# xiyichen/morphablediffusion

Measured on AMD Instinct MI355X. Metric: multi-view denoising steps/sec (N=16 views, 256x256, CFG 2.0, DDIM-50 step), higher is better.
Workload: dtype f16; 1 GPU; synthetic sample (FaceScape-FLAME-sized mesh, 5023 vertices before voxel de-duplication): N=16 target views, 256x256 (latent 32x32), perspective cameras, full-width UNet (916.9M params, random init), CFG 2.0, one denoise_apply per step; views_per_gpu=16, batch_view_num=16, parallelism=single GPU

## Files before the change

include/mvd.h:

```cpp
#ifndef MVD_H
#define MVD_H
#include <stddef.h>
#include <stdint.h>

#ifdef __cplusplus
extern "C" {
#endif

typedef struct mvd_ctx mvd_ctx;

typedef struct {
  int image_size;
  int in_channels;
  int out_channels;
  int model_channels;
  int num_res_blocks;
  int channel_mult[4];
  int num_heads;
  int context_dim;
  int volume_dims[4];
  int attention_levels;
} mvd_unet_config;

typedef struct {
// ... 89 lines not shown
                      float* mse_per_sample, void* stream);
int mvd_op_image_metrics(const void* pred, int pred_dtype, int pred_layout, const void* target, int target_dtype, int target_layout,
                         const unsigned char* mask, int mask_mode, int V, int H, int W, double* out, void* stream);
int mvd_op_mesh_project(const float* verts, const float* K, const float* RT, int N, int Nv, float z_near, int32_t* xy, int32_t* key,
                        void* stream);
int mvd_op_mesh_raster(const int32_t* xy, const int32_t* key, const int32_t* faces, int N, int Nv, int Nf, int H, int W, int32_t* face_id,
                       int32_t* pix_key, int32_t* bad_faces, void* stream);
int mvd_op_mesh_vertex_colors(const void* images, int dtype, int layout, const int32_t* xy, const int32_t* key, const int32_t* faces,
                              const int32_t* face_id, const int32_t* pix_key, const float* verts, const float* normals,
                              const float* centres, int N, int Nv, int Nf, int H, int W, float power, int bias, int two_sided,
                              float fill_r, float fill_g, float fill_b, float* color, float* weight_sum, int32_t* n_seen, float* spread,
                              unsigned char* visible, void* stream);
int mvd_op_morph_pose(const float* betas, const float* pose, const float* j_template, const float* j_dirs, const int32_t* parents, int F,
                      int NB, int J, float* j_rest, float* rot, float* pose_feature, float* joints, float* A, void* stream);
int mvd_op_morph_skin(const float* basis, const float* v_template, const float* coef, const float* weights, const float* A,
                      const float* post, int F, int V, int L, int NB, int J, float* verts, void* stream);
int mvd_op_morph_landmarks(const float* verts, const int32_t* faces, const int32_t* lmk_face, const float* lmk_bary, int F, int V, int Nf,
                           int M, float* out, void* stream);
int mvd_train_conditioner_backward(mvd_ctx* ctx, const float* x_noisy, int64_t timestep, const float* v_embed, int n_views,
                                   int target_index, const float* dsrc0, const float* dsrc1, const float* dsrc2, const float* dsrc3,
                                   float* dbg_dvolume, float* dbg_dfused, float* dbg_dfeats, float* dbg_dtembed, void* stream);
int mvd_train_conditioner_backward_batch(mvd_ctx* ctx, int B, const int* slots, const float* x_noisy, const int64_t* timesteps,
                                         const float* v_embed, int n_views, const int* target_index, const float* dsrc0,
                                         const float* dsrc1, const float* dsrc2, const float* dsrc3, float* dbg_dvolume,
                                         float* dbg_dfused, float* dbg_dfeats, float* dbg_dtembed, void* stream);
int mvd_train_set_deterministic(mvd_ctx* ctx, int on);
int mvd_op_frustum_adjoint(mvd_ctx* ctx, const float* d_out, const int32_t* view_idx, int TN, int D, int S, int deterministic,
                           float* d_vol, void* stream);
int mvd_op_latent_adjoint(mvd_ctx* ctx, const float* d_vol, int deterministic, float* d_rows, int32_t* n_rows_out, void* stream);
int mvd_op_vertex_adjoint(mvd_ctx* ctx, const float* d_vf, const int32_t* view_idx, int n_views, int deterministic, float* d_feats,
                          void* stream);
int mvd_probe_adjoint_calls(mvd_ctx* ctx, int64_t* out);
int mvd_op_vertex_gather(mvd_ctx* ctx, const float* feats, const int32_t* view_idx, int n_views, float* vf_out, void* stream);
int mvd_op_latent_gather(mvd_ctx* ctx, const float* rows, float* vol_out, void* stream);
int mvd_op_frustum_gather(mvd_ctx* ctx, const float* vol, const int32_t* view_idx, int TN, int D, int S, float* out, void* stream);
int mvd_train_cond_backward(mvd_ctx* ctx, int cond_index, const float* x, const float* context, const float* d_out, int B, int H,
                            int W, int depth0, float* dx, float* dcontext, void* stream);
int mvd_train_get_grad(mvd_ctx* ctx, const char* name, float* out, size_t numel, void* stream);
int mvd_train_get_tensor(mvd_ctx* ctx, const char* name, float* out, size_t numel, void* stream);
int64_t mvd_train_bn_calls(mvd_ctx* ctx);
int mvd_train_adamw_step(mvd_ctx* ctx, float lr, float lr_aux, float beta1, float beta2, float eps, float weight_decay, int step,
                         float inv_scale, int finetune_unet, int* skipped_out, void* stream);
int mvd_train_grad_norm(mvd_ctx* ctx, float inv_scale, int finetune_unet, float* norm_out, void* stream);
int mvd_train_adamw_step_ex(mvd_ctx* ctx, float lr, float lr_aux, float beta1, float beta2, float eps, float weight_decay, int step,
                            float inv_scale, int finetune_unet, int* skipped_out, float max_grad_norm, float ema_decay,
                            float* grad_norm_out, void* stream);
int mvd_train_last_grad_norm(mvd_ctx* ctx, float* norm_out, void* stream);
int mvd_train_ema_swap(mvd_ctx* ctx, void* stream);
int mvd_train_repack(mvd_ctx* ctx);
int mvd_train_repack_async(mvd_ctx* ctx, void* stream);
int mvd_lora_attach(mvd_ctx* ctx, const char* const* keys, int n, int rank, float alpha);
int mvd_lora_arena_size(mvd_ctx* ctx, int64_t* numel);
int mvd_lora_target_count(mvd_ctx* ctx);
int mvd_lora_info(mvd_ctx* ctx, int i, char* name, size_t cap, int64_t* a_off, int64_t* b_off, int64_t* out, int64_t* in);
int mvd_lora_adopt_arena(mvd_ctx* ctx, int which, float* ptr, int64_t numel);
int mvd_lora_project(mvd_ctx* ctx, void* stream);
int mvd_lora_step(mvd_ctx* ctx, float lr, float beta1, float beta2, float eps, float weight_decay, int step, float inv_scale,
                  float max_grad_norm, int* skipped_out, float* grad_norm_out, void* stream);
int mvd_lora_set_scale(mvd_ctx* ctx, float scale, void* stream);
int mvd_lora_detach(mvd_ctx* ctx, int keep_merged);
int mvd_train_grad_bucket_count(mvd_ctx* ctx);
int mvd_train_grad_bucket(mvd_ctx* ctx, int k, int max_ranges, int64_t* offs, int64_t* lens, int* n_ranges);
int mvd_train_grad_bucket_wait(mvd_ctx* ctx, int k, void* stream);
int mvd_train_set_bucket_snapshot(mvd_ctx* ctx, float* arena);
int mvd_train_sync_gradients(mvd_ctx* ctx, int phase, void* comm_stream, void* stream);
int mvd_set_volume(mvd_ctx* ctx, const float* volume, void* stream);

int mvd_frustum_volumes(mvd_ctx* ctx, const float* t_embed, const float* v_embed, const int32_t* view_idx, int TN,
                        float* out0, float* out1, float* out2, float* out3, void* stream);
int mvd_frustum_volumes_batch(mvd_ctx* ctx, int B, const int* slots, const float* volumes, const float* t_embed, const float* v_rows,
                              const int32_t* view_idx, float* out0, float* out1, float* out2, float* out3, void* stream);

int mvd_denoise_views(mvd_ctx* ctx, const float* x_noisy, const float* x_input, const float* clip, int64_t timestep,
                      const float* t_embed, const float* v_embed, const int32_t* view_idx, int TN, float cfg_scale,
                      const float* noise, float sqrt_one_minus_at, float sqrt_at, float sqrt_aprev, float dir_coef,
                      float sigma, float* eps_out, float* x_prev, void* stream);
int mvd_denoise_views_batch(mvd_ctx* ctx, int B, const int* slots, const float* x_noisy, const float* x_input, const float* clip,
                            const int64_t* timesteps, const float* t_embed, const float* v_embed, const int32_t* view_idx, int TN,
                            float cfg_scale, const float* noise, float sqrt_one_minus_at, float sqrt_at, float sqrt_aprev,
                            float dir_coef, float sigma, float* eps_out, float* x_prev, void* stream);

int mvd_denoise_views_ms(mvd_ctx* ctx, int B, const int* slots, const float* x_noisy, const float* x_input, const float* clip,
                         const int64_t* timesteps, const float* t_embed, const float* v_embed, const int32_t* view_idx, int TN,
                         float cfg_scale, const float* noise, float s1m, float sqrt_at, float c_x, float c_d, float c_c, float c_n,
                         float* x0_hist, int first, float* eps_out, float* x_next, void* stream);

int mvd_op_cfg_ms(const float* eps_c, const float* eps_u, float scale, const float* x, const float* noise, float s1m, float sqrt_at,
                  float c_x, float c_d, float c_c, float c_n, float* x0_hist, int first, float* eps_out, float* x_next, size_t n,
                  void* stream);
int mvd_op_adamw_ex(float* p, const float* g, float* m, float* v, float* e, size_t n, float lr, float beta1, float beta2, float eps,
                    float wd, int step, float inv_scale, float max_grad_norm, float ema_decay, float* norm_out, void* stream);
int mvd_op_lora_project(const float* dW, const float* A, const float* B, int out, int in, int r, float scale, float* gA, float* gB,
                        void* stream);
int mvd_op_lora_merge(const float* W0, const float* A, const float* B, int out, int in, int r, float scale, float* W, void* stream);
int mvd_op_lora_project_grouped(const float* dW, const float* A, const float* B, int n, const int64_t* w_off, const int64_t* out,
                                const int64_t* in, const int64_t* a_off, const int64_t* b_off, int r, float scale, float* gA, float* gB,
                                void* stream);
int mvd_op_lora_merge_grouped(const float* W0, const float* A, const float* B, int n, const int64_t* w_off, const int64_t* w0_off,
                              const int64_t* out, const int64_t* in, const int64_t* a_off, const int64_t* b_off, int r, float scale,
                              float* W, void* stream);
int mvd_op_sparse_conv(const float* in, const int32_t* nbr, int n_out, int Cin, int Cout, const float* w, int layout, const float* scale,
                       const float* shift, int form, float* out, void* stream);
int mvd_op_bn_rows_relu(const float* x, int n, int C, const float* gamma, const float* beta, float eps, float momentum, float* y,
                        float* stats_out, float* rmean, float* rvar, void* stream);
int mvd_op_bn_rows_relu_bwd(const float* xraw, float* dy, int n, int C, const float* gamma, const float* beta, const float* stats,
                            int poison, float* dgamma, float* dbeta, void* stream);
int mvd_op_sparse_conv_bwd(const float* in, const int32_t* nbr, float* d_out, int n_in, int n_out, int Cin, int Cout, int strided,
                           int level0_subm, int deterministic, int form, const float* w, int layout, int poison, float* d_in, float* gw,
                           void* stream);
int mvd_op_conv(mvd_ctx* ctx, const float* x_nchw, int B, int Cin, int H, int W, const float* w, const float* bias,
                int Cout, int ksize, int stride, int upsample, const float* resid_nchw, float* out_nchw, int force_splitk,
                void* stream);
int mvd_op_linear(mvd_ctx* ctx, const float* a, int M, int K, const float* w, const float* bias, int N, int geglu,
                  const float* resid, int a_half, int force_splitk, float* out, void* stream);
int mvd_op_group_norm(mvd_ctx* ctx, const float* x_nchw, int B, int C, int HW, int groups, const float* gamma,
                      const float* beta, float eps, int act, float* out_nchw, void* stream);
int mvd_op_depth_attn(mvd_ctx* ctx, const float* qk, const float* context, const float* fill_row, int n_cond, int HW, int D, int Cc,
                      int heads, int ldx, int split, int nfill, int check_only, float* out, float* hi_out, void* stream);
int mvd_op_conv3d(mvd_ctx* ctx, const float* x_ncdhw, int B, int Cin, int D, int H, int W, const float* w,
                  const float* bias, int Cout, int stride, int transposed, const float* resid, float* out, void* stream);
int mvd_op_group_norm_bwd(mvd_ctx* ctx, const float* x, const float* dy, int B, int rows, int C, int groups, const float* gamma,
                          const float* beta, float eps, int act, float* dx, float* dgamma, float* dbeta, void* stream);
int mvd_op_layer_norm_bwd(mvd_ctx* ctx, const float* x, const float* dy, int rows, int C, const float* gamma, float* dx,
                          float* dgamma, float* dbeta, void* stream);
int mvd_op_conv_bwd(mvd_ctx* ctx, int kind, int ksize, int B, int Cin, int H, int W, int Cout, const float* x, int x_f16,
                    const float* w, const float* dy, int xp, int accum, int need_din, int poison, float* dx, float* dw, float* db,
                    void* stream);
int mvd_op_linear_bwd(mvd_ctx* ctx, int B, int rows, int K, int N, const float* x, int x_f16, const float* w, const float* bias,
                      const float* dy, int geglu, int dx_f16, int staged, int xp, int accum, int poison, float* dx, float* dw,
                      float* db, void* stream);
int mvd_op_conv3d_bwd(mvd_ctx* ctx, int kind, int B, int Cin, int D, int H, int W, int Cout, const float* x, int x_f16,
                      const float* w, const float* dy, int accum, int poison, float* dx, float* dw, float* db, void* stream);
int mvd_op_tgemm(mvd_ctx* ctx, int M, int N, int K, const float* a, int a_f16, int a_trans, long lda, const float* b, int b_f16,
                 int b_trans, long ldb, float* out, int ldc, int accum, int xp, int poison, void* stream);
int mvd_op_st_tail(mvd_ctx* ctx, int C, int rows, int T, const float* ao, const float* xin, const float* rowbias,
                   const float* w_ao, const float* b_ao, const float* ln_g, const float* ln_b, const float* w1, const float* b1,
                   const float* w2, const float* b2, const float* w_po, const float* b_po, const float* resid, float* out,
                   int flags, int iters, float* ms_out, void* stream);
int mvd_op_st_head(mvd_ctx* ctx, int rows, int xp, const float* n0, const float* w_pi, const float* b_pi, const float* ln_g,
                   const float* ln_b, const float* w_q, const float* w_k, const float* w_v, float* t0_out, float* qkv_out,
                   int iters, float* ms_out, void* stream);
int mvd_op_linear_ex(mvd_ctx* ctx, const float* a, int B, int rows, int K, const float* w, const float* bias, int N,
                     const float* rowbias, int rb_ld, float alpha, int act, int use_bias, int out_f16, int out_split, int ldc,
                     const float* resid, int resid_f16, int ldr, int a_half, int force_splitk, int xp, float* slabs,
                     size_t slabs_cap, int defer_epilogue, int* sk_used, int poison, void* out, void* stream);
int mvd_op_conv_ex(mvd_ctx* ctx, const float* x, int B, int H, int W, int Cin, const float* w, const float* bias, int Cout, int ksize,
                   int stride, int upsample, int up_fold, int tap_shift, const float* rowbias, int rb_ld, float alpha, int act,
                   int use_bias, int out_f16, int out_split, int ldc, const float* resid, int resid_f16, int ldr, int a_half,
                   int force_splitk, int xp, int conv3x_stream, float* slabs, size_t slabs_cap, int defer_epilogue, int* sk_used,
                   int poison, void* out, void* stream);
int mvd_op_conv3d_ex(mvd_ctx* ctx, const float* x, int B, int D, int H, int W, int Cin, const float* w, const float* bias, int Cout,
                     int stride, int transposed, int use_bias, const float* resid, int ldr, int in_place, int out_f16, int ldc,
                     int a_half, int force_splitk, int poison, void* out, void* stream);
int mvd_op_group_norm_ex(mvd_ctx* ctx, const float* x, int B, int rows, int C, int ld, int groups, const float* gamma,
                         const float* beta, float eps, int act, int form, const float* preadd, int pld, int split, int nslab,
                         size_t slab_stride, const float* bias2, const float* resid, int ldr, float* mat, int ldm, int ldo,
                         int poison, void* out, void* stream);
int mvd_op_layer_norm_slabs(mvd_ctx* ctx, const float* slabs, int nslab, size_t slab_stride, int rows, int C, const float* bias,
                            const float* rowbias, int rb_ld, int T, const float* resid, int ldr, const float* gamma,
                            const float* beta, float eps, int plain, int ld_raw, int poison, float* mat, void* raw, void* out,
                            void* stream);
int mvd_op_folded_group_norm(mvd_ctx* ctx, const float* x, int B, int rps, int K, const float* w, int N, int cpg,
                             const float* gamma, const float* beta, float eps, int poison, float* partials, float* scale,
                             float* shift, void* out, void* stream);
int mvd_op_softmax_rows(mvd_ctx* ctx, const float* scores, int rows, int cols, int out_f32, void* out, void* stream);
int mvd_op_rows_split(mvd_ctx* ctx, const float* x, int lda, int rows, int C, void* out, void* stream);
int mvd_op_attention_ex(mvd_ctx* ctx, const float* q, const float* k, const float* v, int B, int T, int heads, int d, int Tstride,
                        int ld_pad, int xcd, float* out, void* stream);
int mvd_op_attention_bwd_ex(mvd_ctx* ctx, const float* q, const float* k, const float* v, const float* d_out, int B, int T,
                            int heads, int d, float* dq, float* dk, float* dv, float* lse, float* delta, float* o, void* stream);
int mvd_op_train_depth_attn(const float* q, const float* k, const float* v, int R, int HW, int D, int hn, int hd, float* attn,
                            float* z, void* stream);
int mvd_op_train_depth_attn_bwd(const float* q, const float* k, const float* v, const float* attn, const float* dz, int R, int HW,
                                int D, int hn, int hd, float* dq, float* dk, float* dv, void* stream);
int mvd_op_train_im2col3(const float* x, int B, int H, int W, int C, float* col, void* stream);
int mvd_op_train_col2im3(const float* dcol, int B, int H, int W, int C, float* dx, void* stream);
int mvd_op_train_perm_w3(const float* src, int N, int C, int to_mat, float* dst, void* stream);
int mvd_bench_conv(mvd_ctx* ctx, int B, int C, int H, int W, int Cout, int iters, float* ms_out, void* stream);
int mvd_vae_decode(mvd_ctx* ctx, const float* z, int B, int h, int w, float* out, void* stream);
int mvd_vae_encode(mvd_ctx* ctx, const float* x, int B, int H, int W, float* moments, void* stream);
int mvd_clip_encode(mvd_ctx* ctx, const float* x, int B, int H, int W, float* out, void* stream);
int mvd_clip_embed_dim(mvd_ctx* ctx);
int mvd_probe_config(mvd_ctx* ctx, int mode, const char* family, int stride);
int mvd_probe_report(mvd_ctx* ctx, char* buf, size_t cap);
int mvd_bench_linear(mvd_ctx* ctx, int M, int K, int N, int flags, int iters, float* ms_out, void* stream);
int mvd_bench_group_norm(mvd_ctx* ctx, int B, int C, int HW, int groups, int flags, int iters, float* ms_out, void* stream);

#ifdef __cplusplus
}
#endif
#endif
```

morphablediffusion_amd/csrc/c_api_hooks.hip:

```cpp
#include <math.h>
#include <string.h>

#include <algorithm>
#include <string>
#include <vector>

#include "hooks.h"
#include "rowchain.h"

namespace {

__global__ void split_rows_to_f32_kernel(const half_t* in, int rows, int C, float* out) {
  for (size_t i = (size_t)blockIdx.x * blockDim.x + threadIdx.x; i < (size_t)rows * C; i += (size_t)gridDim.x * blockDim.x) {
    const size_t r = i / C, c = i % C;
    const half_t hi = in[r * 3 * C + c], lo = in[r * 3 * C + C + c], h2 = in[r * 3 * C + 2 * C + c];
    out[i] = (float)hi == (float)h2 ? (float)hi + (float)lo : __builtin_nanf("");
  }
}
__global__ void rows_f32_to_f16_ld_kernel(const float* in, size_t rows, int C, half_t* out, int ldo) {
  for (size_t i = (size_t)blockIdx.x * blockDim.x + threadIdx.x; i < rows * C; i += (size_t)gridDim.x * blockDim.x)
    out[(i / C) * ldo + i % C] = (half_t)in[i];
}
__global__ void rows_f32_ld_to_f16_ld_kernel(const float* in, int ldi, size_t rows, int C, half_t* out, int ldo) {
  for (size_t i = (size_t)blockIdx.x * blockDim.x + threadIdx.x; i < rows * C; i += (size_t)gridDim.x * blockDim.x)
// ... 484 lines not shown
  half_t* stream_w = ws_alloc<half_t>(c, rowhead_stream_halfs(xp));
  float* tmp = ws_alloc<float>(c, (size_t)3 * C);
  half_t* n0h = ws_alloc<half_t>(c, n * (xp ? 3 : 1));
  half_t* qkvh = ws_alloc<half_t>(c, 3 * n);
  WS_CHECK(stream_w && tmp && n0h && qkvh);
  RhWeights w;
  w.w_pi = w_pi; w.ln_g = ln_g; w.ln_b = ln_b; w.w_q = w_q; w.w_k = w_k; w.w_v = w_v;
  RET_IF(rowhead_pack(w, xp, tmp, stream_w, s));
  if (xp) RET_IF(launch_rows_f32_to_f16_split(n0, C, rows, C, n0h, s));
  else RET_IF(launch_f32_to_f16(n0, n0h, n, s));
  RowHead p;
  p.stream = stream_w; p.rows = rows; p.n0 = n0h; p.ld_n0 = xp ? 3 * C : C; p.b_pi = b_pi; p.t0 = t0_out; p.ld_t0 = C; p.qkv = qkvh; p.ld_qkv = 3 * C;
  RET_IF(launch_rowhead(p, xp, s));
  if (iters > 0) {
    float ms = 0.f;
    RET_IF(hook_time(s, iters, [&] { return launch_rowhead(p, xp, s); }, &ms));
    if (ms_out) *ms_out = ms;
  }
  hook_f16_to_f32(qkvh, qkv_out, 3 * n, s);
  HIP_CHECK_RET(hipGetLastError());
  return 0;
}

namespace {
struct ExEpi {
  const float *bias, *rowbias, *resid;
  int rb_ld, act, use_bias, out_f16, out_split, ldc, resid_f16, ldr, force_splitk;
  float alpha;
  float* slabs;
  size_t slabs_cap;
  int defer_epilogue;
  int* sk_used;
  void* out;
};
int ex_epi_check(const char* who, const ExEpi& e, int N, bool rb_unaligned_ok = false) {
  const std::string w(who);
  if (!e.out) return mvd_fail((w + ": null result").c_str());
  if (N <= 0 || (N & 3)) return mvd_fail((w + ": N must be a positive multiple of 4").c_str());
  if (e.act != ACT_NONE && e.act != ACT_SILU) return mvd_fail((w + ": act is 0 (none) or 1 (SiLU)").c_str());
  if (!(e.alpha == e.alpha) || e.alpha - e.alpha != 0.0f) return mvd_fail((w + ": alpha must be finite").c_str());
  if (e.use_bias && !e.bias) return mvd_fail((w + ": use_bias without a bias").c_str());
  if (e.rowbias && (e.rb_ld < N || (!rb_unaligned_ok && (e.rb_ld & 3)))) return mvd_fail((w + ": rb_ld must be a multiple of 4, >= N").c_str());
  if (e.resid && (e.ldr < N || (e.ldr & 3))) return mvd_fail((w + ": ldr must be a multiple of 4, >= N").c_str());
  if (e.out_split && !e.out_f16) return mvd_fail((w + ": out_split is a form of the fp16 result").c_str());
  if ((e.ldc & 3) || e.ldc < (e.out_split ? 3 : 1) * N) return mvd_fail((w + ": ldc must be a multiple of 4, >= N (3 N with out_split)").c_str());
  if (e.force_splitk < 0) return mvd_fail((w + ": force_splitk >= 0").c_str());
  if (e.slabs && !e.sk_used) return mvd_fail((w + ": a slab buffer needs sk_used").c_str());
  if (e.slabs && ((uintptr_t)e.slabs & 15)) return mvd_fail((w + ": the slab buffer must be 16-byte aligned").c_str());
  if ((uintptr_t)e.out & 15) return mvd_fail((w + ": the result must be 16-byte aligned").c_str());
  return 0;
}
int ex_epi_fill(mvd_ctx* c, const ExEpi& e, size_t out_rows, int N, GemmArgs& g, hipStream_t s) {
  g.out = e.out; g.out_f32 = e.out_f16 ? 0 : 1; g.ldc = e.ldc; g.out_split = e.out_split ? N : 0;
  g.rowbias = e.rowbias; g.rb_ld = e.rb_ld; g.alpha = e.alpha; g.act = e.act; g.use_bias = e.use_bias != 0;
  g.force_splitk = e.force_splitk;
  if (e.resid) {
    g.resid = e.resid; g.resid_f32 = 1; g.ldr = e.ldr;
    if (e.resid_f16) {
      const half_t* rh;
      RET_IF(hook_f16(c, e.resid, out_rows * e.ldr, &rh, s));
      g.resid = rh; g.resid_f32 = 0;
    }
  }
  if (e.slabs) {
    g.slabs = e.slabs; g.slabs_cap = e.slabs_cap; g.sk_used = e.sk_used; g.defer_epilogue = e.defer_epilogue != 0;
  }
  return 0;
}
}

int mvd_op_linear_ex(mvd_ctx* c, const float* a, int B, int rows, int K, const float* w, const float* bias, int N, const float* rowbias,
                     int rb_ld, float alpha, int act, int use_bias, int out_f16, int out_split, int ldc, const float* resid,
                     int resid_f16, int ldr, int a_half, int force_splitk, int xp, float* slabs, size_t slabs_cap, int defer_epilogue,
                     int* sk_used, int poison, void* out, void* stream) {
  RET_IF(hook_begin(c));
  if (!a || !w) return mvd_fail("op_linear_ex: null operand");
  if (B <= 0 || rows <= 0 || rows % B || K <= 0 || (K & 7)) return mvd_fail("op_linear_ex: rows % B == 0 and K % 8 == 0 expected");
  const ExEpi e{bias, rowbias, resid, rb_ld, act, use_bias, out_f16, out_split, ldc, resid_f16, ldr, force_splitk, alpha,
                slabs, slabs_cap, defer_epilogue, sk_used, out};
  RET_IF(ex_epi_check("op_linear_ex", e, N, true));
  hipStream_t s = S(stream);
  WsScope ws_scope(c);
  const int Kp = xp ? 3 * K : K;
  ConvW cw;
  RET_IF(hook_pack_fwd(c, w, N, K, 1, 0, 0, xp, &cw, s));
  cw.bias = const_cast<float*>(bias);
  GemmArgs g;
  g.a = a; g.a_f32 = 1; g.lda = K; g.w = &cw;
  if (xp || a_half) {
    half_t* ah = ws_alloc<half_t>(c, (size_t)rows * Kp);
    WS_CHECK(ah);
    if (xp) RET_IF(launch_rows_f32_to_f16_split(a, K, rows, K, ah, s));
    else RET_IF(launch_f32_to_f16(a, ah, (size_t)rows * K, s));
    g.a = ah; g.a_f32 = 0; g.lda = Kp;
  }
  RET_IF(ex_epi_fill(c, e, (size_t)rows, N, g, s));
  if (sk_used) *sk_used = 1;
  if (poison) RET_IF(hook_poison(c, s));
  return hook_sync("op_linear_ex", s, run_linear(c, g, B, rows, s));
}

int mvd_op_conv_ex(mvd_ctx* c, const float* x, int B, int H, int W, int Cin, const float* w, const float* bias, int Cout, int ksize,
                   int stride, int upsample, int up_fold, int tap_shift, const float* rowbias, int rb_ld, float alpha, int act,
                   int use_bias, int out_f16, int out_split, int ldc, const float* resid, int resid_f16, int ldr, int a_half,
                   int force_splitk, int xp, int conv3x_stream, float* slabs, size_t slabs_cap, int defer_epilogue, int* sk_used,
                   int poison, void* out, void* stream) {
  RET_IF(hook_begin(c));
  if (!x || !w) return mvd_fail("op_conv_ex: null operand");
  if (B <= 0 || H <= 0 || W <= 0 || Cin <= 0 || (Cin & 7)) return mvd_fail("op_conv_ex: Cin % 8 == 0 expected");
  if ((ksize != 1 && ksize != 3) || (stride != 1 && stride != 2) || (upsample != 0 && upsample != 1))
    return mvd_fail("op_conv_ex: 1x1 or 3x3, stride 1 or 2, upsample 0 or 1");
  if (tap_shift != 0 && (tap_shift != 1 || ksize != 3 || stride != 2 || upsample || (H & 1) || (W & 1)))
    return mvd_fail("op_conv_ex: tap_shift = 1 is the 3x3 stride-2 Downsample of even H and W");
  if (up_fold && (!upsample || ksize != 3 || stride != 1 || xp || slabs))
    return mvd_fail("op_conv_ex: the parity-folded form is a 3x3 stride-1 upsample conv without xp or a slab buffer");
  const ExEpi e{bias, rowbias, resid, rb_ld, act, use_bias, out_f16, out_split, ldc, resid_f16, ldr, force_splitk, alpha,
                slabs, slabs_cap, defer_epilogue, sk_used, out};
  RET_IF(ex_epi_check("op_conv_ex", e, Cout));
  hipStream_t s = S(stream);
  WsScope ws_scope(c);
  const int taps = ksize * ksize, Cp = xp ? 3 * Cin : Cin;
  const int Ho = ((H << upsample) - 1) / stride + 1, Wo = ((W << upsample) - 1) / stride + 1;
  const size_t rows_in = (size_t)B * H * W, rows_out = (size_t)B * Ho * Wo;
  ConvW cw;
  RET_IF(hook_pack_fwd(c, w, Cout, Cin, taps, 0, 0, xp, &cw, s));
  cw.bias = const_cast<float*>(bias);
  GemmArgs g;
  g.a = x; g.a_f32 = 1; g.lda = Cin; g.w = &cw; g.tap_shift = tap_shift;
  if (xp || a_half) {
    half_t* xh = ws_alloc<half_t>(c, rows_in * Cp);
    WS_CHECK(xh);
    if (xp) RET_IF(launch_rows_f32_to_f16_split(x, Cin, (long)rows_in, Cin, xh, s));
    else RET_IF(launch_f32_to_f16(x, xh, rows_in * Cin, s));
    g.a = xh; g.a_f32 = 0; g.lda = Cp;
  }
  const int bnx = Cout % 160 == 0 ? 160 : (Cout % 128 == 0 ? 128 : 0);
  if (conv3x_stream && taps == 9 && bnx && Cp % 64 == 0 && !g.a_f32) {
    cw.wx = ws_alloc<half_t>(c, conv3x_stream_halfs(Cout, Cp, bnx));
    WS_CHECK(cw.wx);
    RET_IF(conv3x_pack(cw.w, Cout, Cp, bnx, cw.wx, s));
    cw.wx_bn = bnx;
  }
  if (up_fold) {
    cw.w_up = ws_alloc<half_t>(c, (size_t)16 * Cout * Cin);
    WS_CHECK(cw.w_up);
    RET_IF(launch_pack_upconv_weight(w, Cout, Cin, cw.w_up, s));
  }
  RET_IF(ex_epi_fill(c, e, rows_out, Cout, g, s));
  if (sk_used) *sk_used = 1;
  if (poison) RET_IF(hook_poison(c, s));
  return hook_sync("op_conv_ex", s, up_fold ? run_upconv2d(c, g, B, H, W, s) : run_conv2d(c, g, B, H, W, stride, upsample, s));
}

int mvd_op_conv3d_ex(mvd_ctx* c, const float* x, int B, int D, int H, int W, int Cin, const float* w, const float* bias, int Cout,
                     int stride, int transposed, int use_bias, const float* resid, int ldr, int in_place, int out_f16, int ldc,
                     int a_half, int force_splitk, int poison, void* out, void* stream) {
  RET_IF(hook_begin(c));
  if (!x || !w || !out) return mvd_fail("op_conv3d_ex: null operand");
  if (B <= 0 || D <= 0 || H <= 0 || W <= 0 || Cin <= 0 || (Cin & 7)) return mvd_fail("op_conv3d_ex: Cin % 8 == 0 expected");
  if (Cout <= 0 || (Cout & 3)) return mvd_fail("op_conv3d_ex: Cout must be a positive multiple of 4");
  if ((transposed != 0 && transposed != 1) || (stride != 1 && stride != 2) || (transposed && stride != 1))
    return mvd_fail("op_conv3d_ex: stride 1 or 2, or transposed (with stride 1)");
  if (use_bias && !bias) return mvd_fail("op_conv3d_ex: use_bias without a bias");
  if (resid && (ldr < Cout || (ldr & 3))) return mvd_fail("op_conv3d_ex: ldr must be a multiple of 4, >= Cout");
  if (in_place && !resid) return mvd_fail("op_conv3d_ex: in_place needs a residual");
  if ((ldc & 3) || ldc < Cout) return mvd_fail("op_conv3d_ex: ldc must be a multiple of 4, >= Cout");
  if (force_splitk < 0) return mvd_fail("op_conv3d_ex: force_splitk >= 0");
  if ((uintptr_t)out & 15) return mvd_fail("op_conv3d_ex: the result must be 16-byte aligned");
  const int Do = transposed ? 2 * D : (D - 1) / stride + 1, Ho = transposed ? 2 * H : (H - 1) / stride + 1,
            Wo = transposed ? 2 * W : (W - 1) / stride + 1;
  const size_t rows_in = (size_t)B * D * H * W, rows_out = (size_t)B * Do * Ho * Wo;
  if (rows_out > (size_t)1 << 24 || rows_out * (size_t)ldc > (size_t)1 << 30 || rows_in * (size_t)Cin > (size_t)1 << 30)
    return mvd_fail("op_conv3d_ex: at most 2^24 output rows and 2^30 elements per image");
  hipStream_t s = S(stream);
  WsScope ws_scope(c);
  ConvW cw;
  RET_IF(hook_pack_fwd(c, w, Cout, Cin, 27, transposed, 0, 0, &cw, s));
  cw.bias = const_cast<float*>(bias);
  GemmArgs g;
  g.a = x; g.a_f32 = 1; g.lda = Cin; g.w = &cw; g.out = out; g.out_f32 = out_f16 ? 0 : 1; g.ldc = ldc;
  g.use_bias = use_bias != 0; g.force_splitk = force_splitk;
  if (a_half) {
    const half_t* xh;
    RET_IF(hook_f16(c, x, rows_in * Cin, &xh, s));
    g.a = xh; g.a_f32 = 0;
  }
  if (resid) {
    g.resid = resid; g.resid_f32 = 1; g.ldr = ldr;
    if (in_place) {
      if (out_f16) {
        hipLaunchKernelGGL(rows_f32_ld_to_f16_ld_kernel, dim3(hook_blocks(rows_out * Cout)), dim3(256), 0, s, resid, ldr, rows_out, Cout,
                           (half_t*)out, ldc);
        HIP_CHECK_RET(hipGetLastError());
      } else {
        HIP_CHECK_RET(hipMemcpy2DAsync(out, (size_t)ldc * 4, resid, (size_t)ldr * 4, (size_t)Cout * 4, rows_out, hipMemcpyDeviceToDevice, s));
      }
      g.resid = out; g.resid_f32 = out_f16 ? 0 : 1; g.ldr = ldc;
    }
  }
  if (poison) RET_IF(hook_poison(c, s));
  return hook_sync("op_conv3d_ex", s, transposed ? run_convT3d(c, g, B, D, H, W, s) : run_conv3d(c, g, B, D, H, W, stride, s));
}

int mvd_op_group_norm_ex(mvd_ctx* c, const float* x, int B, int rows, int C, int ld, int groups, const float* gamma, const float* beta,
                         float eps, int act, int form, const float* preadd, int pld, int split, int nslab, size_t slab_stride,
                         const float* bias2, const float* resid, int ldr, float* mat, int ldm, int ldo, int poison, void* out,
                         void* stream) {
  RET_IF(hook_begin(c));
  if (!x || !gamma || !beta || !out) return mvd_fail("op_group_norm_ex: null operand");
  if (B <= 0 || rows <= 0 || C <= 0 || groups <= 0 || C % groups || ld < C) return mvd_fail("op_group_norm_ex: C % groups == 0 and ld >= C expected");
  if (act < ACT_NONE || act > ACT_RELU || (form != 0 && form != 1) || split < 0 || split > 2) return mvd_fail("op_group_norm_ex: act 0..2, form 0..1, split 0..2");
  if (ldo < (split == 1 ? 3 : (split == 2 ? 2 : 1)) * C) return mvd_fail("op_group_norm_ex: ldo >= C halfs (3 C with split = 1, 2 C with split = 2)");
  if (nslab < 1 || (nslab > 1 && slab_stride < (size_t)B * rows * ld)) return mvd_fail("op_group_norm_ex: slabs overlap");
  if (preadd && pld < C) return mvd_fail("op_group_norm_ex: pld >= C expected");
  if ((resid && ldr < C) || (mat && ldm < C)) return mvd_fail("op_group_norm_ex: ldr, ldm >= C expected");
  const bool one_pass = !mvd_env().gn_two_pass && gn_group_eligible(ld, rows, C, groups, preadd ? pld : 0, ldo);
  if ((form == 1 || !one_pass) && (nslab > 1 || bias2 || resid || mat || split == 2))
    return mvd_fail("op_group_norm_ex: slabs, bias2, resid, mat and the fp32 result need the single-pass form");
  hipStream_t s = S(stream);
  WsScope ws_scope(c);
  NormW n;
  n.g = const_cast<float*>(gamma); n.b = const_cast<float*>(beta); n.C = C;
  half_t* o = (half_t*)out;
  if (form == 0) {
    if (poison) RET_IF(hook_poison(c, s));
    return hook_sync("op_group_norm_ex", s,
                   run_group_norm(c, x, ld, B, rows, n, groups, eps, act, preadd, o, ldo, s, pld, split, nslab, slab_stride, bias2, resid,
                                  ldr, mat, ldm));
  }
  if (C > 2560 || groups > 32 || (C & 3) || (ld & 3) || (ldo & 3) || (preadd && (pld & 3)))
    return mvd_fail("op_group_norm_ex: the two-pass form takes C <= 2560, groups <= 32 and C, ld, ldo, pld % 4 == 0");
  float* partial = ws_alloc<float>(c, (size_t)B * gn_max_slabs() * groups * 2);
  WS_CHECK(partial);
  if (poison) RET_IF(hook_poison(c, s));
  int nsl = 0;
  int rc = launch_gn_stats(x, ld, B, rows, C, groups, preadd, pld, partial, &nsl, s);
  if (!rc) rc = launch_gn_apply(x, ld, B, rows, C, groups, preadd, pld, partial, nsl, gamma, beta, eps, act, o, ldo, s, split);
  return hook_sync("op_group_norm_ex", s, rc);
}

int mvd_op_layer_norm_slabs(mvd_ctx* c, const float* slabs, int nslab, size_t slab_stride, int rows, int C, const float* bias,
                            const float* rowbias, int rb_ld, int T, const float* resid, int ldr, const float* gamma, const float* beta,
                            float eps, int plain, int ld_raw, int poison, float* mat, void* raw, void* out, void* stream) {
  RET_IF(hook_begin(c));
  if (!slabs || !gamma || !beta || !out) return mvd_fail("op_layer_norm_slabs: null operand");
  if (rows <= 0 || C <= 0 || nslab < 1 || T < 1) return mvd_fail("op_layer_norm_slabs: bad argument");
  if (raw && ld_raw < C) return mvd_fail("op_layer_norm_slabs: ld_raw >= C expected");
  hipStream_t s = S(stream);
  if (plain) {
    if (nslab != 1 || bias || rowbias || resid || mat) return mvd_fail("op_layer_norm_slabs: the plain LayerNorm takes one slab and writes no mat");
    if (poison) RET_IF(hook_poison(c, s));
    return hook_sync("op_layer_norm_slabs", s, launch_layernorm(slabs, rows, C, gamma, beta, eps, (half_t*)out, s, (half_t*)raw, ld_raw));
  }
  if (!mat) return mvd_fail("op_layer_norm_slabs: mat is required");
  if (nslab > 1 && slab_stride < (size_t)rows * C) return mvd_fail("op_layer_norm_slabs: slabs overlap");
  if ((rowbias && rb_ld < C) || (resid && ldr < C)) return mvd_fail("op_layer_norm_slabs: rb_ld, ldr >= C expected");
  if (poison) RET_IF(hook_poison(c, s));
  return hook_sync("op_layer_norm_slabs", s,
                 launch_layernorm_slabs(slabs, nslab, slab_stride, rows, C, bias, rowbias, rb_ld, T, resid, ldr, mat, gamma, beta, eps,
                                        (half_t*)out, s, (half_t*)raw, ld_raw));
}

int mvd_op_folded_group_norm(mvd_ctx* c, const float* x, int B, int rps, int K, const float* w, int N, int cpg, const float* gamma,
                             const float* beta, float eps, int poison, float* partials, float* scale, float* shift, void* out,
                             void* stream) {
  RET_IF(hook_begin(c));
  if (!x || !w || !gamma || !beta || !partials || !scale || !shift || !out) return mvd_fail("op_folded_group_norm: null operand");
  if (B <= 0 || rps <= 0 || K <= 0 || (K & 7) || N <= 0 || (N & 3)) return mvd_fail("op_folded_group_norm: K % 8 == 0 and N % 4 == 0 expected");
  if (rps % 256 || (cpg != 8 && cpg != 16 && cpg != 32) || (long)B * rps < 512)
    return mvd_fail("op_folded_group_norm: rps % 256 == 0, 8 / 16 / 32 channels per group and at least 512 rows expected");
  if (N % cpg || N / cpg > 32) return mvd_fail("op_folded_group_norm: at most 32 whole groups expected");
  hipStream_t s = S(stream);
  WsScope ws_scope(c);
  const int rows = B * rps, G = N / cpg, ntile = rps / 256;
  ConvW cw;
  RET_IF(hook_pack_fwd(c, w, N, K, 1, 0, 0, 0, &cw, s));
  const half_t* xh;
  RET_IF(hook_f16(c, x, (size_t)rows * K, &xh, s));
  if (poison) RET_IF(hook_poison(c, s));
  GemmArgs g;
  g.a = xh; g.lda = K; g.w = &cw; g.use_bias = false; g.gn_partial = partials; g.gn_cpg = cpg; g.force_splitk = 1;
  int rc = run_linear(c, g, B, rows, s);
  if (!rc) rc = launch_gn_finalize(partials, B, ntile, rps, N, G, gamma, beta, eps, scale, shift, N, s);
  if (!rc) {
    g = GemmArgs();
    g.a = xh; g.lda = K; g.w = &cw; g.use_bias = false; g.out = out; g.out_f32 = 0; g.ldc = N;
    g.rowscale = scale; g.rs_ld = N; g.rowbias = shift; g.rb_ld = N; g.act = ACT_RELU; g.force_splitk = 1;
    rc = run_linear(c, g, B, rows, s);
  }
  return hook_sync("op_folded_group_norm", s, rc);
}

int mvd_op_softmax_rows(mvd_ctx* c, const float* scores, int rows, int cols, int out_f32, void* out, void* stream) {
  RET_IF(hook_begin(c));
  if (!scores || !out || rows <= 0 || cols <= 0) return mvd_fail("op_softmax_rows: bad argument");
  hipStream_t s = S(stream);
  return hook_sync("op_softmax_rows", s,
                 out_f32 ? launch_softmax_rows_f32(scores, rows, cols, (float*)out, s) : launch_softmax_rows(scores, rows, cols, (half_t*)out, s));
}

int mvd_op_rows_split(mvd_ctx* c, const float* x, int lda, int rows, int C, void* out, void* stream) {
  RET_IF(hook_begin(c));
  if (!x || !out || rows <= 0 || C <= 0 || lda < C) return mvd_fail("op_rows_split: bad argument");
  hipStream_t s = S(stream);
  return hook_sync("op_rows_split", s, launch_rows_f32_to_f16_split(x, lda, rows, C, (half_t*)out, s));
}


namespace {
int attn_ex_check(const char* who, const void* q, const void* k, const void* v, int B, int T, int heads, int d) {
  const std::string w(who);
  if (!q || !k || !v) return mvd_fail((w + ": null operand").c_str());
  if (B < 1 || T < 1 || heads < 1) return mvd_fail((w + ": B, T, heads >= 1 expected").c_str());
  if (d != 8 && d != 16 && d != 32 && d != 40 && d != 64 && d != 80 && d != 160) return mvd_fail((w + ": unsupported head dim").c_str());
  return 0;
}
hipError_t hook_unpack_qkv(const float* dqkv, size_t rows, int C, float* dq, float* dk, float* dv, hipStream_t s) {
  float* outs[3] = {dq, dk, dv};
  for (int i = 0; i < 3; ++i) {
    const hipError_t e = hipMemcpy2DAsync(outs[i], (size_t)C * 4, dqkv + (size_t)i * C, (size_t)3 * C * 4, (size_t)C * 4, rows, hipMemcpyDeviceToDevice, s);
    if (e != hipSuccess) return e;
  }
  return hipSuccess;
}
}

int mvd_op_attention_ex(mvd_ctx* c, const float* q, const float* k, const float* v, int B, int T, int heads, int d, int Tstride,
                        int ld_pad, int xcd, float* out, void* stream) {
  RET_IF(hook_begin(c));
  RET_IF(attn_ex_check("op_attention_ex", q, k, v, B, T, heads, d));
  if (!out) return mvd_fail("op_attention_ex: null operand");
  if (Tstride < 0 || (Tstride != 0 && Tstride < T)) return mvd_fail("op_attention_ex: Tstride >= T (or 0) expected");
  if (ld_pad < 0 || ld_pad % 8) return mvd_fail("op_attention_ex: ld_pad must be a multiple of 8");
  if (xcd < -1 || xcd > 1) return mvd_fail("op_attention_ex: xcd is -1, 0 or 1");
  hipStream_t s = S(stream);
  WsScope ws_scope(c);
  const int C = heads * d, ld = 3 * C + ld_pad, Ts = Tstride ? Tstride : T;
  const size_t rows = (size_t)B * Ts + 1;
  half_t* qkv = ws_alloc<half_t>(c, rows * ld);
  half_t* o = ws_alloc<half_t>(c, rows * C);
  WS_CHECK(qkv && o);
  HIP_CHECK_RET(hipMemsetAsync(qkv, 0xFF, rows * ld * sizeof(half_t), s));
  HIP_CHECK_RET(hipMemsetAsync(o, 0xFF, rows * C * sizeof(half_t), s));
  hipLaunchKernelGGL(pack_qkv_image_kernel, dim3(hook_blocks((size_t)B * T * C)), dim3(256), 0, s, q, k, v, B, T, C, Ts, ld, qkv);
  int rc = launch_attention(qkv, ld, qkv + 2 * C, ld, o, C, B, T, heads, d, s, Ts, xcd);
  if (!rc) {
    hook_f16_to_f32(o, out, rows * C, s);
    if (hipGetLastError() != hipSuccess) rc = mvd_fail("op_attention_ex: launch failed");
  }
  return hook_sync("op_attention_ex", s, rc);
}

int mvd_op_attention_bwd_ex(mvd_ctx* c, const float* q, const float* k, const float* v, const float* d_out, int B, int T, int heads,
                            int d, float* dq, float* dk, float* dv, float* lse, float* delta, float* o_out, void* stream) {
// ... 74 lines not shown
```

morphablediffusion_amd/csrc/common.h:

```cpp
#pragma once
#include <hip/hip_runtime.h>
#include <hip/hip_fp16.h>
#include <stdint.h>

#include "env.h"

#ifdef MVD_BF16
typedef __bf16 half_t;
#define MVD_MFMA_32x32x16 __builtin_amdgcn_mfma_f32_32x32x16_bf16
#define MVD_MFMA_16x16x32 __builtin_amdgcn_mfma_f32_16x16x32_bf16
#define MVD_DTYPE_NAME "bf16"
#else
typedef _Float16 half_t;
#define MVD_MFMA_32x32x16 __builtin_amdgcn_mfma_f32_32x32x16_f16
#define MVD_MFMA_16x16x32 __builtin_amdgcn_mfma_f32_16x16x32_f16
#define MVD_DTYPE_NAME "f16"
#endif
typedef half_t h8 __attribute__((ext_vector_type(8)));
typedef half_t h4 __attribute__((ext_vector_type(4)));
typedef half_t h2 __attribute__((ext_vector_type(2)));
typedef float f32x16 __attribute__((ext_vector_type(16)));
typedef float f32x4 __attribute__((ext_vector_type(4)));

#define MVD_MAX_TAPS 27

enum { ACT_NONE = 0, ACT_SILU = 1, ACT_RELU = 2 };

inline bool xcd_prefers_cols(int tiles_m, int groups_n, double a_bytes, double w_bytes) {
  const int nwg = tiles_m * groups_n, q = (nwg + 7) / 8;
  if (nwg < 16) return false;
  auto span = [](int q_, int inner, int outer) {
    const double n = q_ % inner == 0 ? q_ / inner : (q_ - 1) / (double)inner + 1.0;
    return n < outer ? n : (double)outer;
  };
  const double at = a_bytes / tiles_m, wt = w_bytes / groups_n;
  const double row = at * span(q, groups_n, tiles_m) + wt * (q < groups_n ? q : groups_n);
  const double col = wt * span(q, tiles_m, groups_n) + at * (q < tiles_m ? q : tiles_m);
  return col < 0.8 * row;
}

struct IGemm {
  const void* a;
  int a_f32;
  int lda;
  int Cin;
  int cin_alg;
  int B, Z, Y, X;
  int IZ, IY, IX;
  int sz, sy, sx;
  int ups;
  int PZ, PY, PX;
  int ntaps;
  int tap[MVD_MAX_TAPS];
  const half_t* w;
  int N;
  void* out;
  int out_f32;
  int ldc;
  int out_linear;
  int OZ, OY, OX, ozm, ozo, oym, oyo, oxm, oxo;
  const float* bias;
  const float* rowbias;
  int rb_ld;
  const float* rowscale;
  int rs_ld;
  float* gn_partial;
  int gn_cpg;
  const void* resid;
  int resid_f32;
  int ldr;
  int out_split;
  int geglu;
  float alpha;
  int act;
  int nch;
  int xcd_cols;
  int npar;
  int par_ntaps[8];
  int par_tap[8][8];
  int par_oz[8], par_oy[8], par_ox[8];
  int par_walk;
  const half_t* wx;
  int wx_bn;
  int bn;
  int bm;
  int splitk;
  float* partial;
};

struct MvdStream {
  hipStream_t s;
};

#define HIP_CHECK_RET(expr)                                        \
  do {                                                             \
    hipError_t _e = (expr);                                        \
    if (_e != hipSuccess) return mvd_fail(hipGetErrorString(_e));  \
  } while (0)

int mvd_fail(const char* msg);
const char* mvd_error_text();

#define MVD_MAX_DEVICES 64
static inline int mvd_current_device() {
  int d = 0;
  if (hipGetDevice(&d) != hipSuccess || d < 0 || d >= MVD_MAX_DEVICES) d = 0;
  return d;
}
static inline int cdiv(int a, int b) { return (a + b - 1) / b; }
static inline int igemm_tap(int dz, int dy, int dx, int slab) { return (dz + 1) | ((dy + 1) << 2) | ((dx + 1) << 4) | (slab << 8); }

int launch_igemm(const IGemm& g, hipStream_t s);
int igemm_pick_bn(int N, int geglu);
int launch_splitk_reduce(const IGemm& g, hipStream_t s);
bool conv3_halo_eligible(const IGemm& g);
int conv3_halo_tiles(const IGemm& g, int bn);
int launch_conv3_halo(const IGemm& g, hipStream_t s);
int igemm_pick_splitk(int M, int N, int ksteps, int bn);
bool conv3x_eligible(const IGemm& g, int bn);
size_t conv3x_stream_halfs(int N, int Cin, int bn);
int conv3x_pack(const half_t* w, int N, int Cin, int bn, half_t* stream, hipStream_t s);
int launch_conv3x(const IGemm& g, const half_t* stream, int bn, hipStream_t s);
bool gemm_dma_eligible(const IGemm& g);
bool gemm_dma_is_plain(const IGemm& g);
void gemm_dma_plan(int M, int N, int ksteps, int bn, int geglu, int* nch_out, int* splitk_out);
int launch_target_encoder(const float* x, const float* pre, int n_views, const half_t* const* w, const float* const* bias,
                          const int* cin, const float* const* gamma, const float* const* beta, float* feats, hipStream_t s);
void gemm_dma_plan_us(int M, int N, int ksteps, int geglu, int out_b, int res_b, int* bn_io, int* nch_out, int* splitk_out,
                      int* bm_out = nullptr);
int launch_gemm_dma(const IGemm& g, hipStream_t s);

int launch_gn_stats(const float* x, int ld, int B, int rows_per_sample, int C, int G, const float* preadd, int pld,
                    float* partial, int* nslabs_out, hipStream_t s);
int launch_gn_apply(const float* x, int ld, int B, int rows_per_sample, int C, int G, const float* preadd, int pld,
                    const float* partial, int nslabs, const float* gamma, const float* beta, float eps, int act,
                    half_t* out, int ldo, hipStream_t s, int split = 0);
int gn_max_slabs();
int launch_gn_finalize(const float* partial, int B, int nslabs, int rows_per_sample, int C, int G, const float* gamma,
                       const float* beta, float eps, float* scale, float* shift, int ld, hipStream_t s);
bool gn_group_eligible(int ld, int rows, int C, int G, int pld, int ldo);
int launch_gn_group(const float* x, int ld, int B, int rows, int C, int G, const float* preadd, int pld, const float* gamma,
                    const float* beta, float eps, int act, half_t* out, int ldo, hipStream_t s, int split = 0,
                    int nslab = 1, size_t slab_stride = 0, const float* bias2 = nullptr, const float* resid = nullptr, int ldr = 0,
                    float* mat = nullptr, int ldm = 0);
int launch_layernorm(const float* x, int rows, int C, const float* gamma, const float* beta, float eps,
                     half_t* out, hipStream_t s, half_t* raw = nullptr, int ld_raw = 0);
bool layernorm_slabs_takes(int C);
int launch_layernorm_slabs(const float* slabs, int nslab, size_t slab_stride, int rows, int C, const float* bias, const float* rowbias,
                           int rb_ld, int T, const float* resid, int ldr, float* mat, const float* gamma, const float* beta, float eps,
                           half_t* out, hipStream_t s, half_t* raw = nullptr, int ld_raw = 0);
int launch_layernorm_f32(const float* x, long ldx, int rows, int C, const float* gamma, const float* beta, float eps,
                         float* out, hipStream_t s);
int launch_attention(const half_t* qk, int ldqk, const half_t* v, int ldv, half_t* out, int ldo, int B, int T, int heads,
                     int d, hipStream_t s, int Tstride = 0, int xcd = -1);
int launch_clip_patches(const float* img, int B, int H, int W, int S, int P, int Kp, half_t* out, hipStream_t s);
int launch_clip_tokens(const float* pe, const float* cls, const float* pos, int B, int T, int Tp, int C, float* x,
                       hipStream_t s);
int launch_scale_copy(const float* src, size_t n, float k, float* dst, hipStream_t s);
int launch_softmax_rows(const float* s, long rows, int cols, half_t* p, hipStream_t st);
int launch_softmax_rows_f32(const float* s, long rows, int cols, float* p, hipStream_t st);
int launch_depth_attn(const float* qk, const half_t* ctxn, half_t* z, int n_cond, int HW, int D, int Cc, int heads,
                      hipStream_t s, int split = 0, int nfill = 0, const half_t* fill_row = nullptr, int ldx = 0);
int depth_attn_check(int D, int Cc, int heads, int ldx, int nfill);
int launch_small_linear(const float* a, int lda, int rows, int K, const half_t* w, const float* bias, int N,
                        int act_in, float* out, int ldo, int accumulate, hipStream_t s);
int launch_timestep_embedding(const int64_t* t, int B, int dim, float* out, hipStream_t s);
int launch_nchw_to_nhwc(const float* in, int B, int C, int HW, float* out, int ldo, int cpad, hipStream_t s);
int launch_nhwc_to_nchw(const float* in, int ld, int B, int C, int HW, float* out, hipStream_t s);
int launch_pack_weight(const float* src, int N, int Cin, int taps, int transposed, int geglu, half_t* dst,
                       hipStream_t s, int cin_src = -1, int xp = 0);
int launch_rows_f32_to_f16_split(const float* in, int lda, long rows, int C, half_t* out, hipStream_t s);
int launch_permute_geglu_bias(const float* src, int N, float* dst, hipStream_t s);
int launch_f32_to_f16(const float* in, half_t* out, size_t n, hipStream_t s);
int launch_rows_f32_to_f16(const float* in, int lda, long rows, int C, half_t* out, hipStream_t s);
int launch_pack_upconv_weight(const float* src, int N, int Cin, half_t* dst, hipStream_t s);
int launch_fill_rows_f16(half_t* out, int ld, int rows, const half_t* vec, int n, hipStream_t s);
int launch_fold_qk(const float* wq, const float* wk, int heads, int hd, int Cc, int I, float scale, half_t* out,
                   hipStream_t s, float* out32 = nullptr);
int launch_fold_ov(const float* wo, const float* wv, int heads, int hd, int Cc, int I, half_t* out, hipStream_t s,
                   float* out32 = nullptr);
int launch_fold_mm(const float* a, int lda, const float* b, int ldb, int M, int N, int K, half_t* out16, int ldc, float* out32,
                   hipStream_t s);
int launch_relu_beta_tile(const float* beta, int Cc, int heads, half_t* out, hipStream_t s, int split = 0);
int launch_cfg_ddim(const float* eps_c, const float* eps_u, float scale, const float* x, const float* noise,
                    float sqrt_one_minus_at, float sqrt_at, float sqrt_aprev, float dir_coef, float sigma,
                    float* eps_out, float* x_prev, size_t n, hipStream_t s);
struct DpmCoef {
  float s1m, sqrt_at, c_x, c_d, c_c, c_n;
};
int launch_cfg_dpm(const float* eps_c, const float* eps_u, float scale, const float* x, const float* noise, DpmCoef k,
                   float* x0_hist, int use_hist, float* eps_out, float* x_next, size_t n, hipStream_t s);
struct ViewCam {
  float P[12];
  float Pinv[12];
  float Kinv[9];
  float near_, far_;
};
int launch_vertex_gather(const float* feats, const ViewCam* cams, const int* view_idx, int n_views, const float* verts, int Nv, int V,
                         float vol_len, int fsize, int persp, float* out, hipStream_t s);
int launch_unproject_views(const float* feats, const ViewCam* cams, int N, int V, float vol_len, int S, int persp, half_t* out,
                           hipStream_t s);
int launch_rows_f16_to_nchw(const half_t* in, long rows, int C, float* out, hipStream_t s);
int launch_accumulate_f32(float* dst, const float* src, size_t n, hipStream_t s);
int launch_fuse_views(const float* vf, int n_views, int Nv, int total_views, const float* w, const float* b,
                      float* out, int accumulate, hipStream_t s);
int launch_sparse_conv(const float* in, const int* nbr, int n_out, int Cin, int Cout, const float* w, const float* wp,
                       const float* scale, const float* shift, float* out, hipStream_t s, int mask_nonrep = 0);
bool sparse_mfma_takes(int Cin, int Cout);
int launch_sparse_w_frag(const float* w, int Cl_in, int Cl_out, int transposed, int flip, float* dst, hipStream_t s);
int launch_sparse_w_pack(const float* src, int Cin, int Cout, int layout, float* dst, hipStream_t s);
int launch_bn_fold(const float* gamma, const float* beta, const float* mean, const float* var, float eps, int C, float* scale,
                   float* shift, hipStream_t s);
int launch_bn_rows_relu(const float* x, float* y, int n, int C, const float* gamma, const float* beta, float eps, float* stats_out,
                        hipStream_t s, float* rmean = nullptr, float* rvar = nullptr, float momentum = 0.f);
int launch_mse(const float* a, const float* b, size_t n, float* out, hipStream_t s);
size_t train_loss_scratch_bytes(int B, int HW);
int train_loss_check(const char* who, int B, int HW, int C, int loss_type, float huber_delta);
int launch_train_loss(const float* pred, const float* target, int B, int HW, int C, const float* w, const float* m, int loss_type,
                      float huber_delta, float loss_scale, float* dpred, float* loss_out, float* loss_ps, float* mse_ps, void* scratch,
                      hipStream_t s);
size_t image_metrics_scratch_bytes(int V, int H, int W);
int image_metrics_check(const char* who, const void* pred, int pred_dtype, int pred_layout, const void* target, int target_dtype,
                        int target_layout, const unsigned char* mask, int mask_mode, int V, int H, int W, const double* out);
int launch_image_metrics(const void* pred, int pred_dtype, int pred_layout, const void* target, int target_dtype, int target_layout,
                         const unsigned char* mask, int mask_mode, int V, int H, int W, double* out, void* scratch, hipStream_t s);
int mesh_project_check(const char* who, const float* verts, const float* K, const float* RT, int N, int Nv, float z_near, const int* xy,
                       const int* key);
int launch_mesh_project(const float* verts, const float* K, const float* RT, int N, int Nv, float z_near, int* xy, int* key, hipStream_t s);
int mesh_raster_check(const char* who, const int* xy, const int* key, const int* faces, int N, int Nv, int Nf, int H, int W,
                      const int* face_id, const int* pix_key, const int* bad_faces);
size_t mesh_raster_scratch_bytes(int N, int H, int W);
int launch_mesh_raster(const int* xy, const int* key, const int* faces, int N, int Nv, int Nf, int H, int W, int* face_id, int* pix_key,
                       int* bad_faces, void* scratch, hipStream_t s);
int mesh_vertex_colors_check(const char* who, const void* images, int dtype, int layout, const int* xy, const int* key, const int* faces,
                             const int* face_id, const int* pix_key, const float* verts, const float* normals, const float* centres, int N,
                             int Nv, int Nf, int H, int W, float power, const float* color, const float* weight_sum, const int* n_seen,
                             const float* spread);
int launch_mesh_vertex_colors(const void* images, int dtype, int layout, const int* xy, const int* key, const int* faces, const int* face_id,
                              const int* pix_key, const float* verts, const float* normals, const float* centres, int N, int Nv, int Nf,
                              int H, int W, float power, int bias, int two_sided, float fill_r, float fill_g, float fill_b, float* color,
                              float* weight_sum, int* n_seen, float* spread, unsigned char* visible, hipStream_t s);
constexpr int MORPH_MAX_JOINTS = 64;
int morph_pose_check(const char* who, const float* betas, const float* pose, const float* j_template, const float* j_dirs,
                     const int* parents, int F, int NB, int J, const float* j_rest, const float* rot, const float* pose_feature,
                     const float* joints, const float* A);
int launch_morph_pose(const float* betas, const float* pose, const float* j_template, const float* j_dirs, const int* parents, int F,
                      int NB, int J, float* j_rest, float* rot, float* pose_feature, float* joints, float* A, hipStream_t s);
int morph_skin_check(const char* who, const float* basis, const float* v_template, const float* coef, const float* weights,
                     const float* A, int F, int V, int L, int NB, int J, const float* verts);
int launch_morph_skin(const float* basis, const float* v_template, const float* coef, const float* weights, const float* A,
                      const float* post, int F, int V, int L, int J, float* verts, hipStream_t s);
int morph_landmarks_check(const char* who, const float* verts, const int* faces, const int* lmk_face, const float* lmk_bary, int F, int V,
                          int Nf, int M, const float* out);
int launch_morph_landmarks(const float* verts, const int* faces, const int* lmk_face, const float* lmk_bary, int F, int V, int Nf, int M,
                           float* out, hipStream_t s);
int launch_latent_gather(const float* feats, const int* grid, int gd, int gh, int gw, const float* min_xyz,
                         const int* out_sh, float voxel, int V, float vol_len, float* out, hipStream_t s);
int launch_sparse_densify(const float* feats, const int* grid, long nvox, int C, float* out, hipStream_t s);
int launch_frustum_gather(const float* vol, const ViewCam* cams, const int* view_idx, int TN, int D, int S, int V,
                          float vol_len, int persp, half_t* out, hipStream_t s);
int launch_bits_checksum(const void* p, size_t bytes, unsigned long long* out, hipStream_t s);
int launch_add_rows(float* dst, const float* a, const float* b, size_t n, hipStream_t s);
int launch_add_image_rows(const float* in, int ldi, const float* img, int C, int nb, int HW, float* out, int ldo, hipStream_t s);
int launch_upsample2_f16(const float* in, int ldi, int B, int H, int W, int C, half_t* out, hipStream_t s);
int launch_conv_in_f32(const float* x, int ldx, const float* w, int cin_src, const float* bias, int N, int B, int H, int W, float* out,
                       int ldo, hipStream_t s);
int launch_out_conv_f32(const float* a, int C, const float* w, const float* bias, int N, int B, int H, int W, float* out, int ldo,
                        hipStream_t s);
int launch_probe_null(hipStream_t s);
int bwd_tcast(const void* src, int src_f32, long ld, int R, int C, half_t* dst, int Rp, hipStream_t s, int split = 0, half_t* rows16 = nullptr,
              int Cp = 0);
int bwd_im2colT(const void* src, int src_f32, long ld, int B, int H, int W, int C, int stride, int ups, half_t* dst, int Rp, hipStream_t s);
int bwd_cast_rows(const float* src, long ld, long rows, int C, int Cp, half_t* dst, hipStream_t s, int split = 0);
int bwd_pack_dgrad(const half_t* w, int taps, int N, int ldw, int Cl, int Np, half_t* wT, hipStream_t s, int flip = 1);
int bwd_group_norm(const float* x, long ld, const float* pre, int pld, const float* dy, long ldy, int B, int rows, int C, int G,
// ... 97 lines not shown
```

morphablediffusion_amd/csrc/engine.h:

```cpp
#pragma once
#include <functional>
#include <map>
#include <string>
#include <vector>

#include "../../include/mvd.h"
#include "common.h"
#include "rowchain.h"

struct RawTensor {
  float* d = nullptr;
  std::vector<int64_t> shape;
  size_t numel = 0;
};

struct ConvW {
  int xp = 0;
  int cin_l = 0;
  half_t* w = nullptr;
  half_t* wx = nullptr;
  int wx_bn = 0;
  half_t* w_up = nullptr;
  int res_out = 0;
  float* w32 = nullptr;
// ... 385 lines not shown
  int Bv, n_ctx, depth0;
  const float* emb_all;
  const float* context;
  const float* a2_all;
  const Ctx5* src;
  const half_t* src16[4];
  const half_t* cn_pre[16] = {nullptr};
  int cn_ld[16] = {0};
  bool ctx_side = false;
  bool train = false;
};
struct Carry;
int unet_embeddings(mvd_ctx* c, const int64_t* t, const float* context, int Bv, hipStream_t s, float** e0_out, float** e1_out,
                    float** e2_out, float** ea_out, float** a2_out);
int engine_unet_block(mvd_ctx* c, const char* path, const float* x_nhwc, int B, int C, int H, int W, const int64_t* t,
                      const float* context, const float* vol_ndhwc, int D, int n_ctx, float* out_nhwc, int* Cout, int* Hout,
                      hipStream_t s);
int unet_do_res(Fwd& f, const ResW& r, View in, View out, int H, int W, ResSaved* sv = nullptr, Carry* in_carry = nullptr,
                Carry* out_carry = nullptr);
int unet_do_st(Fwd& f, const STW& t, View in, View out, int H, int W, STSaved* sv = nullptr, Carry* in_carry = nullptr,
               Carry* out_carry = nullptr);
int unet_do_cond(Fwd& f, const CondW& d, View in, View out, int H, int W, int level, int cond_idx = -1);
int unet_do_op(Fwd& f, const UOp& op, View in, View out, int& H, int& W, StageRec* rec = nullptr, Carry* in_carry = nullptr,
               Carry* out_carry = nullptr);
int engine_repack(mvd_ctx* c, hipStream_t after = nullptr, bool have_stream = false);
int engine_train_setup(mvd_ctx* c);
void engine_build_rotate(mvd_ctx* c);
int engine_build_join(mvd_ctx* c);
bool engine_hot_key(const std::string& k);
int engine_build_dgrad(mvd_ctx* c);
int engine_build_dgrad_cond(mvd_ctx* c);
float* engine_grad(mvd_ctx* c, const std::string& key);
const float* engine_master(mvd_ctx* c, const std::string& key);
int engine_dmalloc(mvd_ctx* c, void** p, size_t bytes);
int engine_train_conditioner_backward(mvd_ctx* c, const float* x_noisy_nchw, int64_t timestep, const float* v_embed, int n_views,
                                      int target_idx, float* const dsrc[4], float* dbg_dvolume, float* dbg_dfused, float* dbg_dfeats,
                                      float* dbg_dtembed, hipStream_t s);
int engine_train_conditioner_backward_batch(mvd_ctx* c, int B, const int* slots, const float* x_noisy_all, const int64_t* timesteps,
                                            const float* v_embed_all, int n_views, const int* target_idx, float* const dsrc[4],
                                            float* dbg_dvolume, float* dbg_dfused, float* dbg_dfeats, float* dbg_dtembed, hipStream_t s);
struct TrainLossOpts {
  const float* sample_w;
  const float* pixel_w;
  int loss_type;
  float huber_delta;
  float* loss_per_sample;
  float* mse_per_sample;
};
int engine_train_cond_backward(mvd_ctx* c, int cond_idx, const float* x, const float* ctx_vol, const float* dout, int B, int H, int W,
                               int level, int depth0, float* dx, float* dctx, hipStream_t s);
int engine_train_step(mvd_ctx* c, const float* x_nhwc, int x_ld, const int64_t* t, const float* context, int B, int depth0,
                      const Ctx5 src[4], const float* target_nhwc, float loss_scale, int recompute, float* pred_nhwc, float* loss_out,
                      float* const dsrc[4], hipStream_t s, const TrainLossOpts* lo = nullptr);
int engine_set_cameras(mvd_ctx* c, const float* K, const float* RT, int N, hipStream_t s);
int engine_set_mesh(mvd_ctx* c, const float* vertices, const int32_t* coord, const int32_t* out_sh, const float* bounds,
                    int Nv, hipStream_t s);
int engine_select_sample(mvd_ctx* c, int slot);
int engine_set_samples(mvd_ctx* c, int B, const int* slots, const float* const* vertices, const int32_t* const* coord,
                       const int32_t* const* out_sh, const float* const* bounds, const int* Nv, const float* const* K,
                       const float* const* RT, int N, hipStream_t s);
int engine_rulebook_build(const int32_t* coord, const int32_t* out_sh, int Nv, int force_hash, int32_t* n_sites, int64_t* lens);
int engine_rulebook_table(int which, int32_t* out);
void mesh_free(MeshTables& m);
int engine_vertex_features(mvd_ctx* c, const float* x_noisy, const float* t_embed, const float* v_embed,
                           const int32_t* view_idx_dev, int n_local, int add_bias, float* fused_out, hipStream_t s,
                           float* vf_out = nullptr);
int engine_target_encoder(mvd_ctx* c, const float* x_noisy, const float* t_embed, const float* v_embed, int n_local, float* feats,
                          hipStream_t s, float* pre_own = nullptr);
bool engine_encoder_is_fused(const mvd_ctx* c);
struct EncBufs {
  float *cur[4], *r1[3];
  half_t *a1[3], *a2[3], *af;
};
int engine_encoder_layers(mvd_ctx* c, const ConvW* const w[8], bool xp, const void* x0, int n, const float* pre, const EncBufs& b,
                          float* feats, hipStream_t s);
struct SparseSaved {
  const float* in[9];
  float *raw[9], *post[9], *stats[9];
  const int* nbr[9];
  int n_out[9], n_in[9];
};
int engine_sparse_net(mvd_ctx* c, const float* fused, hipStream_t s, bool bn_batch_stats, const float** rows_out,
                      SparseSaved* sv = nullptr);
struct FrustumGeom {
  int D[4], S[4];
  size_t vox[4];
};
FrustumGeom frustum_geom(const mvd_ctx* c);
struct FrustumBufs {
  float *xd[4], *xf[4];
  float* tmp[3];
  half_t *a1[3], *a2[3], *au[3];
  half_t* x0h = nullptr;
};
int engine_frustum_layers(mvd_ctx* c, int TN, const half_t* gath, const float* pre, const FrustumBufs& b, hipStream_t s,
                          const std::function<int()>* film = nullptr);
int engine_fuse_vertex_features(mvd_ctx* c, const float* vf_all, int n_views, float* fused_out, hipStream_t s);
int engine_volume_from_fused(mvd_ctx* c, const float* fused, hipStream_t s, bool bn_batch_stats = false);
struct FrustumOut {
  half_t* lvl0_half = nullptr;
  float* lvl[4];
};
int engine_frustum(mvd_ctx* c, const float* t_embed, const float* v_embed, const int32_t* view_idx_dev, int TN,
                   FrustumOut* out, hipStream_t s, bool half0 = false);
int engine_frustum_multi(mvd_ctx* c, int B, const int* slots, const float* t_embed, const float* v_embed,
                         const int32_t* view_idx_dev, int TN, FrustumOut* out, hipStream_t s, bool half0);
int engine_frustum_batch(mvd_ctx* c, int B, const int* slots, const float* volumes, const float* t_embed, const float* v_rows,
                         const int32_t* view_idx_dev, FrustumOut* out, hipStream_t s);
int engine_spatial_time_volume(mvd_ctx* c, const float* x_noisy, const float* t_embed, const float* v_embed, int n_views,
                               float* volume_out, hipStream_t s);
int engine_stage_unproject(mvd_ctx* c, const float* feats_nchw, int n_views, float* out, hipStream_t s);
size_t engine_spatial_arena_bytes(const mvd_ctx* c);

struct GemmArgs {
  const void* a = nullptr;
  int a_f32 = 0, lda = 0;
  const ConvW* w = nullptr;
  void* out = nullptr;
  int out_f32 = 1, ldc = 0;
  const float* rowbias = nullptr;
  int rb_ld = 0;
  float alpha = 1.0f;
  int tap_shift = 0;
  const float* rowscale = nullptr;
  int rs_ld = 0;
  float* gn_partial = nullptr;
  int gn_cpg = 0;
  const void* resid = nullptr;
  int resid_f32 = 1, ldr = 0;
  int geglu = 0;
  int act = 0;
  bool use_bias = true;
  int force_splitk = 0;
  int out_split = 0;
  float* slabs = nullptr;
  size_t slabs_cap = 0;
  int* sk_used = nullptr;
  bool defer_epilogue = false;
};
struct Carry {
  float* slabs = nullptr;
  size_t cap = 0;
  float* aux = nullptr;
  size_t aux_cap = 0;
  int sk = 1;
  size_t stride = 0;
  const float* bias = nullptr;
  const float* resid = nullptr;
  int ldr = 0;
};
int run_linear(mvd_ctx* c, const GemmArgs& ga, int B, int rows, hipStream_t s);
int run_conv2d(mvd_ctx* c, const GemmArgs& ga, int B, int H, int W, int stride, int ups, hipStream_t s);
int run_upconv2d(mvd_ctx* c, const GemmArgs& ga, int B, int H, int W, hipStream_t s);
int run_conv3d(mvd_ctx* c, const GemmArgs& ga, int B, int D, int H, int W, int stride, hipStream_t s);
int run_convT3d(mvd_ctx* c, const GemmArgs& ga, int B, int D, int H, int W, hipStream_t s);
int run_group_norm(mvd_ctx* c, const float* x, int ld, int B, int rows_per_sample, const NormW& n, int groups, float eps,
                   int act, const float* preadd, half_t* out, int ldo, hipStream_t s, int preadd_ld = 0, int split = 0,
                   int nslab = 1, size_t slab_stride = 0, const float* bias2 = nullptr, const float* resid = nullptr, int ldr = 0,
                   float* mat = nullptr, int ldm = 0);
enum { WS_CHAIN = 0, WS_BLOCK = 1, WS_TEMP = 2 };
struct WsScope {
  Workspace& w;
  const size_t mark;
  const int kind;
  explicit WsScope(mvd_ctx* c, int kind_ = WS_CHAIN) : w(c->ws), mark(c->ws.off), kind(kind_) {}
  ~WsScope() {
    if (!w.hold || (kind == WS_TEMP && w.hold >= 2) || (kind == WS_BLOCK && w.hold == 3)) w.off = mark;
  }
  WsScope(const WsScope&) = delete;
  WsScope& operator=(const WsScope&) = delete;
};
struct SideJoin {
  hipStream_t main;
  hipStream_t side = nullptr;
  hipEvent_t ev = nullptr;
  explicit SideJoin(hipStream_t m) : main(m) {}
  ~SideJoin() {
    if (!side) return;
    hipEventRecord(ev, side);
    hipStreamWaitEvent(main, ev, 0);
  }
};
struct ProbeScope {
  mvd_ctx* c;
  hipStream_t s;
  size_t slot = (size_t)-1;
  ProbeScope(mvd_ctx* c_, hipStream_t s_, const char* family, double flops, double bytes) : c(c_), s(s_) {
    if (!c->probe_mode) return;
    if (c->probe_mode == 2 && c->probe_only != family) return;
    mvd_ctx::ProbeFam& f = c->probe_fam[family];
    ++f.launches;
    f.flops += flops;
    f.bytes += bytes;
    if (c->probe_mode == 2 && c->probe_stride > 1) {
      unsigned h = ++c->probe_counter * 2654435761u;
      h ^= h >> 15;
      if (h % (unsigned)c->probe_stride) return;
    }
    if (c->probe_used + 2 > c->probe_ev.size())
      for (int i = 0; i < 2; ++i) {
        hipEvent_t ev;
        if (hipEventCreate(&ev) != hipSuccess) return;
        c->probe_ev.push_back(ev);
      }
    slot = c->probe_used;
    c->probe_used += 2;
    ++f.sampled;
    f.s_flops += flops;
    f.s_bytes += bytes;
    f.ev.push_back(slot);
    hipEventRecord(c->probe_ev[slot], s);
  }
  ~ProbeScope() {
    if (slot == (size_t)-1) return;
    hipEventRecord(c->probe_ev[slot + 1], s);
    if (c->probe_mode == 1 && (slot & 14) == 0) {
      if (c->probe_used + 2 > c->probe_ev.size())
        for (int i = 0; i < 2; ++i) {
          hipEvent_t ev;
          if (hipEventCreate(&ev) != hipSuccess) return;
          c->probe_ev.push_back(ev);
        }
      const size_t e = c->probe_used;
      c->probe_used += 2;
      c->probe_empty.push_back(e);
      hipEventRecord(c->probe_ev[e], s);
      hipEventRecord(c->probe_ev[e + 1], s);
    }
    if (c->probe_mode == 1 && (slot & 14) == 8) {
      if (c->probe_used + 2 > c->probe_ev.size())
        for (int i = 0; i < 2; ++i) {
          hipEvent_t ev;
          if (hipEventCreate(&ev) != hipSuccess) return;
          c->probe_ev.push_back(ev);
        }
      const size_t e = c->probe_used;
      c->probe_used += 2;
      c->probe_null.push_back(e);
      hipEventRecord(c->probe_ev[e], s);
      launch_probe_null(s);
      hipEventRecord(c->probe_ev[e + 1], s);
    }
  }
  ProbeScope(const ProbeScope&) = delete;
  ProbeScope& operator=(const ProbeScope&) = delete;
};
int engine_side_init(mvd_ctx* c);
template <typename T>
inline T* ws_alloc(mvd_ctx* c, size_t n) {
  return (T*)c->ws.alloc(n * sizeof(T));
}
#define WS_CHECK(p) \
  if (!(p)) return mvd_fail("workspace exhausted: create the context with a larger workspace_bytes")
#define RET_IF(x)          \
  do {                     \
    int _r = (x);          \
    if (_r) return _r;     \
  } while (0)
```

morphablediffusion_amd/csrc/engine_unet.hip:

```cpp
#include <string.h>

#include <algorithm>

#include "engine.h"

namespace {

void igemm_init(IGemm& g) {
  memset(&g, 0, sizeof(g));
  g.alpha = 1.0f;
  g.sz = g.sy = g.sx = 1;
  g.out_linear = 1;
  g.Z = g.Y = g.X = g.B = 1;
  g.IZ = g.IY = g.IX = 1;
  g.PZ = g.PY = g.PX = 1;
  for (int i = 0; i < MVD_MAX_TAPS; ++i) g.tap[i] = igemm_tap(0, 0, 0, i);
}

void igemm_fill(IGemm& g, const GemmArgs& ga) {
  g.a = ga.a;
  g.a_f32 = ga.a_f32;
  g.lda = ga.lda;
  g.Cin = ga.w->Cin;
  g.cin_alg = ga.w->xp ? ga.w->cin_l : ga.w->Cin;
  g.w = ga.w->w;
  g.wx = ga.w->wx;
  g.wx_bn = ga.w->wx_bn;
  g.N = ga.w->N;
  g.out = ga.out;
  g.out_f32 = ga.out_f32;
  g.ldc = ga.ldc;
  g.bias = ga.use_bias ? ga.w->bias : nullptr;
  g.rowbias = ga.rowbias;
  g.rb_ld = ga.rb_ld;
  g.alpha = ga.alpha;
  g.rowscale = ga.rowscale;
  g.rs_ld = ga.rs_ld;
  g.gn_partial = ga.gn_partial;
  g.gn_cpg = ga.gn_cpg;
  g.resid = ga.resid;
  g.resid_f32 = ga.resid_f32;
  g.ldr = ga.ldr;
  g.geglu = ga.geglu;
  g.act = ga.act;
  g.out_split = ga.out_split;
}

int pick_chunk_split(int tiles, int ncc, double step_us, int M, int N, double* us) {
  int sk = 1;
  *us = 1e30;
  for (int s2 = 1; s2 <= 8 && s2 <= ncc; ++s2) {
    const int rounds = cdiv(tiles * s2, 256), steps = cdiv(ncc, s2) * 9;
    double t = rounds * (steps * step_us + 8.0);
    if (s2 > 1) t += 3.0 + (s2 + 1) * (double)M * N * 4.0 / 3.5e6;
    if (t < *us) {
      *us = t;
      sk = s2;
    }
  }
  return sk;
}

bool place_partials(mvd_ctx* c, IGemm& g, int M, int sk, const GemmArgs* defer, bool form_ok) {
  g.splitk = sk;
  g.partial = nullptr;
  bool deferred = false;
  if (sk > 1) {
    if (defer && defer->slabs && defer->sk_used && sk <= mvd_env().defer_max && (size_t)sk * M * g.N <= defer->slabs_cap &&
        (!g.resid || (defer->defer_epilogue && g.resid_f32)) && form_ok) {
      g.partial = defer->slabs;
      deferred = true;
    } else {
      g.partial = ws_alloc<float>(c, (size_t)sk * M * g.N);
      if (!g.partial) g.splitk = 1;
    }
  }
  if (defer && defer->sk_used) *defer->sk_used = deferred ? sk : 1;
  return deferred;
}

int reduce_partials(mvd_ctx* c, IGemm& g, int M, hipStream_t s) {
  ProbeScope ps(c, s, "splitk_reduce_kernel", 0.0, (double)M * g.N * 4.0 * (g.splitk + 1));
  return launch_splitk_reduce(g, s);
}

int go_conv3x(mvd_ctx* c, IGemm& g, int M, int force_splitk, hipStream_t s, const GemmArgs* defer) {
  const int ncc = g.Cin / 64;
  const int tiles = (g.X == 8 ? cdiv(g.B, 4) : g.B * (g.Y / 16) * (g.X / 16)) * (g.N / g.wx_bn);
  double us;
  int sk = pick_chunk_split(tiles, ncc, g.wx_bn == 160 ? 0.75 : 0.62, M, g.N, &us);
  if (force_splitk > 0) sk = force_splitk < ncc ? force_splitk : ncc;
  if (sk > 1) sk = cdiv(ncc, cdiv(ncc, sk));
  g.bn = g.wx_bn;
  WsScope ws_scope(c, WS_TEMP);
  const bool deferred = place_partials(c, g, M, sk, defer, true);
  const double kalg = (double)(g.cin_alg ? g.cin_alg : g.Cin);
  const double flops = 2.0 * M * g.N * kalg * 9.0;
  double bytes = (double)M * kalg * 2 + 9.0 * g.N * kalg * 2 + (g.splitk > 1 ? 0.0 : (double)M * g.N * 4);
  if (g.resid && g.splitk <= 1) bytes += (double)M * g.N * 4;
  int r;
  {
    ProbeScope ps(c, s, g.wx_bn == 160 ? "conv3x_kernel<5>" : "conv3x_kernel<4>", flops, bytes);
    r = launch_conv3x(g, g.wx, g.wx_bn, s);
  }
  if (!r && g.splitk > 1 && !deferred) r = reduce_partials(c, g, M, s);
  return r;
}

int go_parity_batch(mvd_ctx* c, IGemm& g, int M, hipStream_t s) {
  if (!gemm_dma_eligible(g)) return mvd_fail("igemm_go: parity batch needs the LDS-DMA kernel");
  int kmax = 0;
  for (int p = 0; p < g.npar; ++p) kmax = g.par_ntaps[p] > kmax ? g.par_ntaps[p] : kmax;
  int nch = 1, sk2 = 1;
  gemm_dma_plan(M * g.npar, g.N, kmax * cdiv(g.Cin, 64), g.bn, 1, &nch, &sk2);
  g.nch = nch;
  g.splitk = 1;
  g.partial = nullptr;
  const int pwalk_min = mvd_env().par_walk_min;
  if (pwalk_min > 0 && cdiv(M, 256) * cdiv(g.N, g.bn) >= pwalk_min) {
    g.par_walk = 1;
    g.nch = 1;
  }
  double fl = 0.0;
  for (int p = 0; p < g.npar; ++p) fl += 2.0 * M * g.N * (double)(g.cin_alg ? g.cin_alg : g.Cin) * g.par_ntaps[p];
  const double by = (double)g.B * g.PZ * g.PY * g.PX * g.Cin * 2 + (double)g.npar * kmax * g.N * g.Cin * 2 +
                    (double)M * g.npar * g.N * (g.out_f32 ? 4 : 2) + (g.resid ? (double)M * g.npar * g.N * (g.resid_f32 ? 4 : 2) : 0.0);
  char fam[64];
  snprintf(fam, sizeof fam, "gemm_dma_kernel<%d,0>", g.bn);
  ProbeScope ps(c, s, fam, fl, by);
  return launch_gemm_dma(g, s);
}

int plan_halo(IGemm& g, int M, int force_splitk) {
  const MvdEnv& env = mvd_env();
  const int ncc = g.Cin / 64;
  double best = 1e30;
  int best_bn = 128, best_sk = 1;
  for (int bn = 128; bn <= 160; bn += 32) {
    double us;
    const int s2 = pick_chunk_split(conv3_halo_tiles(g, bn), ncc, bn == 160 ? 1.3 : 1.0, M, g.N, &us);
    if (us < best) {
      best = us;
      best_bn = bn;
      best_sk = s2;
    }
  }
  g.bn = best_bn;
  int sk = force_splitk > 0 ? (force_splitk < ncc ? force_splitk : ncc) : best_sk;
  if (env.halo_bn) g.bn = env.halo_bn;
  if (env.halo_sk) sk = env.halo_sk;
  if (sk > ncc) sk = ncc;
  if (sk > 1) sk = cdiv(ncc, cdiv(ncc, sk));
  return sk;
}

int plan_dense(IGemm& g, int M, int force_splitk) {
  const MvdEnv& env = mvd_env();
  int nch = 1, sk2 = 1;
  const int ksteps = g.ntaps * cdiv(g.Cin, 64);
  const bool plain_gemm = !g.gn_partial && !g.rowscale && g.ntaps == 1;
  if (plain_gemm && !env.old_plan) {
    int bn = 0, bm = 256;
    gemm_dma_plan_us(M, g.N, ksteps, g.geglu, g.out_f32 ? 4 : (g.out_split ? 6 : 2), g.resid ? (g.resid_f32 ? 4 : 2) : 0, &bn,
                     &nch, &sk2, gemm_dma_is_plain(g) ? &bm : nullptr);
    g.bn = bn;
    g.bm = bm;
  } else {
    gemm_dma_plan(M, g.N, ksteps, g.bn, g.geglu, &nch, &sk2);
  }
  if (g.gn_partial || g.rowscale) {
    if (g.bn == 160) g.bn = 128;
    const int tiles = cdiv(M, 256) * cdiv(g.N, g.bn);
    nch = cdiv(tiles, 256);
    if (nch > 64) nch = 64;
    force_splitk = 1;
  }
  int sk = g.geglu ? 1 : (force_splitk > 0 ? force_splitk : sk2);
  if (env.dense_bn && !g.geglu && !g.gn_partial && !g.rowscale) {
    g.bn = env.dense_bn;
    g.bm = (env.dense_bm == 128 && gemm_dma_is_plain(g)) ? 128 : 256;
    gemm_dma_plan(M, g.N, ksteps, g.bn, g.geglu, &nch, &sk2);
    if (g.bm == 128) {
      nch = 1;
      sk2 = 1;
    }
    if (force_splitk <= 0) sk = sk2;
  }
  if (env.dense_sk && !g.geglu && force_splitk <= 0) sk = env.dense_sk;
  if (sk > ksteps) sk = ksteps;
  if (sk > 1) sk = cdiv(ksteps, cdiv(ksteps, sk));
  g.nch = sk > 1 ? 1 : nch;
  if (env.plan_debug) fprintf(stderr, "[plan] M=%d N=%d ksteps=%d -> bm=%d bn=%d nch=%d sk=%d\n", M, g.N, ksteps, g.bm ? g.bm : 256, g.bn, g.nch, sk);
  return sk;
}

int plan_gather(IGemm& g, int M, int force_splitk) {
  const int ksteps = g.ntaps * cdiv(g.Cin, 64);
  int sk = force_splitk > 0 ? force_splitk : igemm_pick_splitk(M, g.N, ksteps, g.bn);
  if (sk > ksteps) sk = ksteps;
  if (sk > 1) sk = cdiv(ksteps, cdiv(ksteps, sk));
  return sk;
}

enum IGemmKernel { K_GATHER = 0, K_HALO = 1, K_DENSE = 2 };

int launch_planned(mvd_ctx* c, IGemm& g, int M, int sk, IGemmKernel kernel, hipStream_t s, const GemmArgs* defer) {
  WsScope ws_scope(c, WS_TEMP);
  const bool deferred =
      place_partials(c, g, M, sk, defer, !g.geglu && g.act == 0 && g.alpha == 1.0f && g.out_linear && g.out_f32 && !g.out_split);
  const bool timing = mvd_env().layer_timing;
  static hipEvent_t ev0 = nullptr, ev1 = nullptr;
  if (timing) {
    if (!ev0) {
      hipEventCreate(&ev0);
      hipEventCreate(&ev1);
    }
    hipEventRecord(ev0, s);
  }
  int r;
  const double flops = 2.0 * M * g.N * (double)(g.cin_alg ? g.cin_alg : g.Cin) * g.ntaps;
  const double in_rows = (double)g.B * g.PZ * g.PY * g.PX;
  const double out_cols = g.geglu ? g.N / 2 : g.N;
  const double kalg = (double)(g.cin_alg ? g.cin_alg : g.Cin);
  double bytes = in_rows * kalg * (g.a_f32 ? 4 : 2) + (double)g.ntaps * g.N * kalg * 2 +
                 (g.gn_partial ? 0.0 : (double)M * out_cols * (g.out_f32 ? 4 : 2));
  if (g.resid) bytes += (double)M * g.N * (g.resid_f32 ? 4 : 2);
  char fam[64];
  if (kernel == K_HALO) {
    snprintf(fam, sizeof fam, "conv3_dma_kernel<%d,%d,%d>", g.bn == 160 ? 160 : 128, g.X % 16 == 0 ? 16 : 8, g.X % 16 == 0 ? 16 : 8);
    ProbeScope ps(c, s, fam, flops, g.splitk > 1 ? bytes - (double)M * out_cols * (g.out_f32 ? 4 : 2) : bytes);
    r = launch_conv3_halo(g, s);
  } else if (kernel == K_DENSE) {
    if (g.bm == 128) snprintf(fam, sizeof fam, "gemm_dma_kernel<128x%d>", g.bn);
    else snprintf(fam, sizeof fam, "gemm_dma_kernel<%d,%d>", g.bn, g.gn_partial ? 1 : (g.rowscale ? 2 : 0));
    ProbeScope ps(c, s, fam, flops, bytes);
    r = launch_gemm_dma(g, s);
  } else {
    const int bn = g.bn ? g.bn : igemm_pick_bn(g.N, g.geglu);
    snprintf(fam, sizeof fam, "igemm_kernel<%d,%d>", g.a_f32, bn);
    ProbeScope ps(c, s, fam, flops, bytes);
    r = launch_igemm(g, s);
  }
  if (!r && g.splitk > 1 && !deferred) r = reduce_partials(c, g, M, s);
  if (timing) {
    hipEventRecord(ev1, s);
    hipEventSynchronize(ev1);
    float ms = 0.f;
    hipEventElapsedTime(&ms, ev0, ev1);
    const double fl = 2.0 * M * g.N * g.Cin * g.ntaps;
    fprintf(stderr, "[gemm] M=%d N=%d Cin=%d taps=%d f32=%d halo=%d bn=%d sk=%d geglu=%d  %.1f us  %.0f TF\n", M, g.N, g.Cin,
            g.ntaps, g.a_f32, (int)kernel, g.bn, g.splitk, g.geglu, ms * 1e3, fl / (ms * 1e-3) * 1e-12);
  }
  return r;
}

int igemm_go(mvd_ctx* c, IGemm& g, int force_splitk, hipStream_t s, const GemmArgs* defer = nullptr) {
  const MvdEnv& env = mvd_env();
  const int M = g.B * g.Z * g.Y * g.X;
  g.bn = igemm_pick_bn(g.N, g.geglu);
  if (g.a_f32 && g.bn == 160 && env.igemm_f32_bn128) g.bn = 128;
  if (env.conv3x && c->use_halo && g.wx && conv3x_eligible(g, g.wx_bn)) return go_conv3x(c, g, M, force_splitk, s, defer);
  if (g.npar > 0) return go_parity_batch(c, g, M, s);
  const bool halo = c->use_halo && conv3_halo_eligible(g);
  const bool dense = env.gemm_dma && !halo && M >= env.dense_min_m && (g.ntaps == 1 || M <= 16384) && gemm_dma_eligible(g);
  if (g.gn_partial && !dense) return mvd_fail("igemm_go: the statistics-only pass needs the LDS-DMA kernel");
  if (halo) return launch_planned(c, g, M, plan_halo(g, M, force_splitk), K_HALO, s, defer);
  if (dense) return launch_planned(c, g, M, plan_dense(g, M, force_splitk), K_DENSE, s, defer);
  return launch_planned(c, g, M, plan_gather(g, M, force_splitk), K_GATHER, s, defer);
}

}

int run_linear(mvd_ctx* c, const GemmArgs& ga, int B, int rows, hipStream_t s) {
  IGemm g;
  igemm_init(g);
  igemm_fill(g, ga);
  g.B = B;
  g.X = rows / B;
  g.IX = g.X;
  g.PX = g.X;
  g.ntaps = 1;
  return igemm_go(c, g, ga.force_splitk, s, &ga);
}

int run_conv2d(mvd_ctx* c, const GemmArgs& ga, int B, int H, int W, int stride, int ups, hipStream_t s) {
  IGemm g;
  igemm_init(g);
  igemm_fill(g, ga);
  g.B = B;
  g.PY = H;
  g.PX = W;
  g.ups = ups;
  g.IY = H << ups;
  g.IX = W << ups;
  g.sy = g.sx = stride;
  g.Y = (g.IY - 1) / stride + 1;
  g.X = (g.IX - 1) / stride + 1;
  if (ga.w->taps == 9) {
    g.ntaps = 9;
    for (int t = 0; t < 9; ++t) g.tap[t] = igemm_tap(0, t / 3 - 1 + ga.tap_shift, t % 3 - 1 + ga.tap_shift, t);
  } else if (ga.w->taps == 1) {
    g.ntaps = 1;
  } else {
    return mvd_fail("run_conv2d: kernel must be 1x1 or 3x3");
  }
  return igemm_go(c, g, ga.force_splitk, s, &ga);
}

int run_upconv2d(mvd_ctx* c, const GemmArgs& ga_in, int B, int H, int W, hipStream_t s) {
  if (!ga_in.w->w_up) return mvd_fail("run_upconv2d: weights were not folded");
  WsScope ws_scope(c, WS_TEMP);
  GemmArgs ga = ga_in;
  ConvW cw = *ga_in.w;
  cw.w = cw.w_up;
  cw.taps = 16;
  ga.w = &cw;
  if (ga.a_f32) {
    half_t* ah = ws_alloc<half_t>(c, (size_t)B * H * W * cw.Cin);
    WS_CHECK(ah);
    RET_IF(launch_rows_f32_to_f16((const float*)ga.a, ga.lda, (long)B * H * W, cw.Cin, ah, s));
    ga.a = ah;
    ga.a_f32 = 0;
    ga.lda = cw.Cin;
  }
  IGemm gb;
  igemm_init(gb);
  igemm_fill(gb, ga);
  gb.B = B;
  gb.Y = gb.PY = gb.IY = H;
  gb.X = gb.PX = gb.IX = W;
  gb.out_linear = 0;
  gb.OZ = 1;
  gb.OY = 2 * H;
  gb.OX = 2 * W;
  gb.ozm = 1;
  gb.oym = gb.oxm = 2;
  const bool batched = mvd_env().parity_batch && ga.force_splitk <= 1 && gemm_dma_eligible(gb);
  for (int par = 0; par < 4; ++par) {
    const int py = par >> 1, px = par & 1;
    int taps[4];
    for (int a = 0; a < 2; ++a)
      for (int b = 0; b < 2; ++b)
        taps[a * 2 + b] = igemm_tap(0, py == 0 ? a - 1 : a, px == 0 ? b - 1 : b, par * 4 + a * 2 + b);
    if (batched) {
      gb.par_ntaps[par] = 4;
      for (int i = 0; i < 4; ++i) gb.par_tap[par][i] = taps[i];
      gb.par_oz[par] = 0;
      gb.par_oy[par] = py;
      gb.par_ox[par] = px;
      continue;
    }
    IGemm g = gb;
    g.ntaps = 4;
    for (int i = 0; i < 4; ++i) g.tap[i] = taps[i];
    g.oyo = py;
    g.oxo = px;
    RET_IF(igemm_go(c, g, ga.force_splitk, s));
  }
  if (batched) {
    gb.npar = 4;
    gb.ntaps = 4;
    gb.bn = igemm_pick_bn(gb.N, 0);
    RET_IF(igemm_go(c, gb, 0, s));
  }
  return 0;
}

int run_conv3d(mvd_ctx* c, const GemmArgs& ga, int B, int D, int H, int W, int stride, hipStream_t s) {
  IGemm g;
  igemm_init(g);
  igemm_fill(g, ga);
  g.B = B;
  g.PZ = g.IZ = D;
  g.PY = g.IY = H;
  g.PX = g.IX = W;
  g.sz = g.sy = g.sx = stride;
  g.Z = (D - 1) / stride + 1;
  g.Y = (H - 1) / stride + 1;
  g.X = (W - 1) / stride + 1;
  if (ga.w->taps == 27) {
    g.ntaps = 27;
    for (int t = 0; t < 27; ++t) g.tap[t] = igemm_tap(t / 9 - 1, (t / 3) % 3 - 1, t % 3 - 1, t);
  } else if (ga.w->taps == 1) {
    g.ntaps = 1;
  } else {
    return mvd_fail("run_conv3d: kernel must be 1 or 27 taps");
  }
  return igemm_go(c, g, ga.force_splitk, s);
}

int run_convT3d(mvd_ctx* c, const GemmArgs& ga, int B, int D, int H, int W, hipStream_t s) {
  if (ga.w->taps != 27) return mvd_fail("run_convT3d: expects a 3x3x3 kernel");
  IGemm gb;
  igemm_init(gb);
  igemm_fill(gb, ga);
  gb.B = B;
  gb.Z = gb.PZ = gb.IZ = D;
  gb.Y = gb.PY = gb.IY = H;
  gb.X = gb.PX = gb.IX = W;
  gb.out_linear = 0;
  gb.OZ = 2 * D;
  gb.OY = 2 * H;
  gb.OX = 2 * W;
  gb.ozm = gb.oym = gb.oxm = 2;
  const bool batched = mvd_env().parity_batch && !ga.a_f32 && ga.force_splitk <= 1 && B * D * H * W >= 512 && gemm_dma_eligible(gb);
  for (int par = 0; par < 8; ++par) {
    const int pz = par >> 2, py = (par >> 1) & 1, px = par & 1;
    const int kz[2] = {pz ? 0 : 1, 2}, dzv[2] = {pz ? 1 : 0, 0}, nz = pz ? 2 : 1;
    const int ky[2] = {py ? 0 : 1, 2}, dyv[2] = {py ? 1 : 0, 0}, ny = py ? 2 : 1;
    const int kx[2] = {px ? 0 : 1, 2}, dxv[2] = {px ? 1 : 0, 0}, nx = px ? 2 : 1;
    int taps[8], t = 0;
    for (int a = 0; a < nz; ++a)
      for (int b = 0; b < ny; ++b)
        for (int e = 0; e < nx; ++e) taps[t++] = igemm_tap(dzv[a], dyv[b], dxv[e], (kz[a] * 3 + ky[b]) * 3 + kx[e]);
    if (batched) {
      gb.par_ntaps[par] = t;
      for (int i = 0; i < t; ++i) gb.par_tap[par][i] = taps[i];
      gb.par_oz[par] = pz;
      gb.par_oy[par] = py;
      gb.par_ox[par] = px;
      continue;
    }
    IGemm g = gb;
    for (int i = 0; i < t; ++i) g.tap[i] = taps[i];
    g.ntaps = t;
    g.ozo = pz;
    g.oyo = py;
    g.oxo = px;
    RET_IF(igemm_go(c, g, ga.force_splitk, s));
  }
  if (batched) {
    gb.npar = 8;
    gb.ntaps = 8;
    gb.bn = igemm_pick_bn(gb.N, 0);
    RET_IF(igemm_go(c, gb, 0, s));
  }
  return 0;
}

int run_group_norm(mvd_ctx* c, const float* x, int ld, int B, int rows_per_sample, const NormW& n, int groups, float eps,
                   int act, const float* preadd, half_t* out, int ldo, hipStream_t s, int preadd_ld, int split, int nslab,
                   size_t slab_stride, const float* bias2, const float* resid, int ldr, float* mat, int ldm) {
  ProbeScope ps(c, s, "group_norm", 0.0, (double)B * rows_per_sample * n.C * 6.0);
  if (!mvd_env().gn_two_pass && gn_group_eligible(ld, rows_per_sample, n.C, groups, preadd ? (preadd_ld ? preadd_ld : n.C) : 0, ldo))
    return launch_gn_group(x, ld, B, rows_per_sample, n.C, groups, preadd, preadd_ld ? preadd_ld : n.C, n.g, n.b, eps, act, out,
                           ldo, s, split, nslab, slab_stride, bias2, resid, ldr, mat, ldm);
  if (nslab > 1 || resid || mat) return mvd_fail("run_group_norm: slab input needs the single-pass form");
  WsScope ws_scope(c, WS_TEMP);
  float* partial = ws_alloc<float>(c, (size_t)B * gn_max_slabs() * groups * 2);
  WS_CHECK(partial);
  int nslabs = 0;
  RET_IF(launch_gn_stats(x, ld, B, rows_per_sample, n.C, groups, preadd, preadd_ld, partial, &nslabs, s));
  RET_IF(launch_gn_apply(x, ld, B, rows_per_sample, n.C, groups, preadd, preadd_ld, partial, nslabs, n.g, n.b, eps, act, out,
                         ldo, s, split));
  return 0;
}

namespace {

}

int unet_do_res(Fwd& f, const ResW& r, View in, View out, int H, int W, ResSaved* sv, Carry* in_carry, Carry* out_carry) {
  mvd_ctx* c = f.c;
  WsScope ws_scope(c, WS_BLOCK);
  const int rows = f.Bv * H * W;
  const int w1 = r.c1.xp ? 3 : 1, w2 = r.c2.xp ? 3 : 1;
  half_t* a1 = ws_alloc<half_t>(c, (size_t)rows * r.cin * w1);
  float* h1 = ws_alloc<float>(c, (size_t)rows * r.cout);
  half_t* a2 = ws_alloc<half_t>(c, (size_t)rows * r.cout * w2);
  WS_CHECK(a1 && h1 && a2);
  const bool skip_side = r.has_skip && mvd_env().skip_side && !f.train && !sv;
  const bool sk_in_carry = r.has_skip && out_carry && out_carry->aux && out_carry->aux_cap >= (size_t)rows * r.cout;
  float* skbuf = nullptr;
  auto launch_skip = [&](hipStream_t ss, bool no_split) -> int {
    GemmArgs gs;
    gs.a = in.p; gs.a_f32 = 1; gs.lda = in.ld; gs.w = &r.skip; gs.out = skbuf; gs.ldc = r.cout;
    if (no_split) gs.force_splitk = 1;
    if (r.skip.xp) {
      half_t* as = ws_alloc<half_t>(c, (size_t)rows * 3 * r.cin);
      WS_CHECK(as);
      RET_IF(launch_rows_f32_to_f16_split(in.p, in.ld, rows, r.cin, as, ss));
      gs.a = as; gs.a_f32 = 0; gs.lda = 3 * r.cin;
    }
    return run_linear(c, gs, f.Bv, rows, ss);
  };
  auto fork_skip = [&]() -> int {
    if (!c->side2) {
      HIP_CHECK_RET(hipStreamCreateWithFlags(&c->side2, hipStreamNonBlocking));
      HIP_CHECK_RET(hipEventCreateWithFlags(&c->ev_s2_fork, hipEventDisableTiming));
      HIP_CHECK_RET(hipEventCreateWithFlags(&c->ev_s2_join, hipEventDisableTiming));
    }
    HIP_CHECK_RET(hipEventRecord(c->ev_s2_fork, f.s));
    HIP_CHECK_RET(hipStreamWaitEvent(c->side2, c->ev_s2_fork, 0));
    RET_IF(launch_skip(c->side2, true));
    HIP_CHECK_RET(hipEventRecord(c->ev_s2_join, c->side2));
    return 0;
  };
  if (r.has_skip) {
    skbuf = sk_in_carry ? out_carry->aux : ws_alloc<float>(c, (size_t)rows * r.cout);
    WS_CHECK(skbuf);
  }
  const bool in_slabs = in_carry && in_carry->sk > 1;
  if (skip_side && !in_slabs) RET_IF(fork_skip());
  if (in_slabs)
    RET_IF(run_group_norm(c, in_carry->slabs, r.cin, f.Bv, H * W, r.n1, 32, 1e-5f, ACT_SILU, nullptr, a1, r.cin * w1, f.s, 0, r.c1.xp,
                          in_carry->sk, in_carry->stride, in_carry->bias, in_carry->resid, in_carry->ldr, in.p, in.ld));
  else
    RET_IF(run_group_norm(c, in.p, in.ld, f.Bv, H * W, r.n1, 32, 1e-5f, ACT_SILU, nullptr, a1, r.cin * w1, f.s, 0, r.c1.xp));
  if (skip_side && in_slabs) RET_IF(fork_skip());
  GemmArgs g1;
  g1.a = a1; g1.lda = r.cin * w1; g1.w = &r.c1; g1.out = h1; g1.ldc = r.cout;
  g1.rowbias = f.emb_all + r.emb_off; g1.rb_ld = c->emb_total;
  int sk1 = 1;
  const size_t slab_elems = (size_t)rows * r.cout;
  if (mvd_env().defer_reduce && !f.train && gn_group_eligible(r.cout, H * W, r.cout, 32, c->emb_total, r.cout * w2)) {
    const size_t nsl = rows > 8192 ? 4 : 16;
    g1.slabs = ws_alloc<float>(c, nsl * slab_elems);
    g1.slabs_cap = g1.slabs ? nsl * slab_elems : 0;
    g1.sk_used = &sk1;
  }
  RET_IF(run_conv2d(c, g1, f.Bv, H, W, 1, 0, f.s));
  if (sk1 > 1)
    RET_IF(run_group_norm(c, g1.slabs, r.cout, f.Bv, H * W, r.n2, 32, 1e-5f, ACT_SILU, g1.rowbias, a2, r.cout * w2, f.s, g1.rb_ld,
                          r.c2.xp, sk1, slab_elems, r.c1.bias));
  else
    RET_IF(run_group_norm(c, h1, r.cout, f.Bv, H * W, r.n2, 32, 1e-5f, ACT_SILU, nullptr, a2, r.cout * w2, f.s, 0, r.c2.xp));
  const float* resid = in.p;
  int ldr = in.ld;
  bool skip_outlives_scope = true;
  if (r.has_skip) {
    skip_outlives_scope = sk_in_carry;
    if (skip_side) HIP_CHECK_RET(hipStreamWaitEvent(f.s, c->ev_s2_join, 0));
    else RET_IF(launch_skip(f.s, false));
    resid = skbuf;
    ldr = r.cout;
  }
  GemmArgs g2;
  g2.a = a2; g2.lda = r.cout * w2; g2.w = &r.c2; g2.out = out.p; g2.ldc = out.ld; g2.resid = resid; g2.ldr = ldr;
  int sk2 = 1;
  if (out_carry && out_carry->slabs && skip_outlives_scope) {
    g2.slabs = out_carry->slabs; g2.slabs_cap = out_carry->cap; g2.sk_used = &sk2; g2.defer_epilogue = true;
// ... 848 lines not shown
```

morphablediffusion_amd/csrc/engine_weights.hip:

```cpp
#include <algorithm>
#include <math.h>
#include <string.h>

#include "engine.h"

int engine_dmalloc(mvd_ctx* c, void** p, size_t bytes) {
  if (bytes == 0) bytes = 16;
  if (c->repacking) {
    if (c->repack_cursor >= c->sec_end || c->owned_bytes[c->repack_cursor] != bytes)
      return mvd_fail("engine_repack: allocation sequence differs from the first build");
    *p = c->owned[c->repack_cursor++];
    return 0;
  }
  HIP_CHECK_RET(hipMalloc(p, bytes));
  c->owned.push_back(*p);
  c->owned_bytes.push_back(bytes);
  return 0;
}

void engine_build_rotate(mvd_ctx* c) {
  if (c->bs_multi) c->bs = c->bstreams[(c->bs_rr++) & 3];
}
int engine_build_join(mvd_ctx* c) {
  if (!c->bs_multi) return 0;
// ... 58 lines not shown
  o->cin_l = Cl;
  o->taps = taps;
  o->key = wkey;
  o->bkey = bkey;
  RET_IF(dmalloc(c, (void**)&o->w, (size_t)taps * N * Cin * sizeof(half_t)));
  RET_IF(launch_pack_weight(r->d, N, Cin, taps, transposed ? 1 : 0, geglu ? 1 : 0, o->w, c->bs, cin_src, xp ? 1 : 0));
  if (!bkey.empty()) {
    if (geglu) {
      RawTensor* b;
      RET_IF(get_raw(c, bkey, &b));
      RET_IF(dmalloc(c, (void**)&o->bias, (size_t)N * sizeof(float)));
      RET_IF(launch_permute_geglu_bias(b->d, N, o->bias, c->bs));
    } else {
      RET_IF(copy_f32(c, bkey, &o->bias));
    }
  }
  return 0;
}

int pack_lin(mvd_ctx* c, const std::string& wkey, const std::string& bkey, LinW* o) {
  engine_build_rotate(c);
  RawTensor* r;
  RET_IF(get_raw(c, wkey, &r));
  o->N = (int)r->shape[0];
  o->K = (int)(r->numel / r->shape[0]);
  o->key = wkey.size() > 7 ? wkey.substr(0, wkey.size() - 7) : wkey;
  RET_IF(dmalloc(c, (void**)&o->w, r->numel * sizeof(half_t)));
  RET_IF(launch_f32_to_f16(r->d, o->w, r->numel, c->bs));
  if (!bkey.empty()) RET_IF(copy_f32(c, bkey, &o->bias));
  return 0;
}

int build_res(mvd_ctx* c, const std::string& p, int cin, int cout, ResW* r) {
  r->key = p;
  r->cin = cin;
  r->cout = cout;
  RET_IF(load_norm(c, p + ".in_layers.0", &r->n1));
  RET_IF(pack_conv(c, p + ".in_layers.2.weight", p + ".in_layers.2.bias", false, false, &r->c1));
  RET_IF(load_norm(c, p + ".out_layers.0", &r->n2));
  RET_IF(pack_conv(c, p + ".out_layers.3.weight", p + ".out_layers.3.bias", false, false, &r->c2));
  r->has_skip = c->raw.count(p + ".skip_connection.weight") > 0;
  if (r->has_skip) RET_IF(pack_conv(c, p + ".skip_connection.weight", p + ".skip_connection.bias", false, false, &r->skip));
  else if (cin != cout) return mvd_fail("ResBlock changes width but has no skip_connection weight");
  return 0;
}

int build_st(mvd_ctx* c, const std::string& p, int C, STW* s) {
  s->key = p;
  s->C = C;
  s->heads = c->u.num_heads;
  const std::string t = p + ".transformer_blocks.0";
  RET_IF(load_norm(c, p + ".norm", &s->norm));
  RET_IF(pack_conv(c, p + ".proj_in.weight", p + ".proj_in.bias", false, false, &s->proj_in));
  RET_IF(pack_conv(c, p + ".proj_out.weight", p + ".proj_out.bias", false, false, &s->proj_out));
  RET_IF(load_norm(c, t + ".norm1", &s->ln1));
  RET_IF(load_norm(c, t + ".norm3", &s->ln3));
  RawTensor *q, *k, *v;
  RET_IF(get_raw(c, t + ".attn1.to_q.weight", &q));
  RET_IF(get_raw(c, t + ".attn1.to_k.weight", &k));
  RET_IF(get_raw(c, t + ".attn1.to_v.weight", &v));
  s->qkv.N = 3 * C;
  s->qkv.Cin = C;
  s->qkv.cin_l = C;
  s->qkv.taps = 1;
  RET_IF(dmalloc(c, (void**)&s->qkv.w, (size_t)3 * C * C * sizeof(half_t)));
  RET_IF(launch_f32_to_f16(q->d, s->qkv.w, (size_t)C * C, c->bs));
  RET_IF(launch_f32_to_f16(k->d, s->qkv.w + (size_t)C * C, (size_t)C * C, c->bs));
  RET_IF(launch_f32_to_f16(v->d, s->qkv.w + (size_t)2 * C * C, (size_t)C * C, c->bs));
  RET_IF(pack_conv(c, t + ".attn1.to_out.0.weight", t + ".attn1.to_out.0.bias", false, false, &s->attn_out));
  RET_IF(pack_conv(c, t + ".ff.net.0.proj.weight", t + ".ff.net.0.proj.bias", false, true, &s->ff1));
  RET_IF(pack_conv(c, t + ".ff.net.2.weight", t + ".ff.net.2.bias", false, false, &s->ff2));
  return 0;
}

int build_cond(mvd_ctx* c, const std::string& p, int dim, int Cc, CondW* d) {
  const int heads = 4, hd = Cc / 2, I = 2 * Cc;
  d->key = p;
  d->dim = dim;
  d->Cc = Cc;
  d->I = I;
  RET_IF(pack_conv(c, p + ".proj_in.0.weight", p + ".proj_in.0.bias", false, false, &d->proj_in));
  RET_IF(load_norm(c, p + ".proj_in.1", &d->gn_in));
  RET_IF(pack_conv(c, p + ".proj_context.0.weight", "", false, false, &d->proj_ctx));
  RET_IF(load_norm(c, p + ".proj_context.1", &d->gn_ctx));
  RawTensor *wq, *wk, *wv, *wo;
  RET_IF(get_raw(c, p + ".depth_attn.to_q.weight", &wq));
  RET_IF(get_raw(c, p + ".depth_attn.to_k.weight", &wk));
  RET_IF(get_raw(c, p + ".depth_attn.to_v.weight", &wv));
  RET_IF(get_raw(c, p + ".depth_attn.to_out.weight", &wo));
  d->wqk.N = heads * Cc;
  d->wqk.Cin = I;
  d->wqk.taps = 1;
  RET_IF(dmalloc(c, (void**)&d->wqk.w, (size_t)heads * Cc * I * sizeof(half_t)));
  RET_IF(launch_fold_qk(wq->d, wk->d, heads, hd, Cc, I, 1.0f / sqrtf((float)hd), d->wqk.w, c->bs));
  d->wov.N = I;
  d->wov.Cin = heads * Cc;
  d->wov.taps = 1;
  RET_IF(dmalloc(c, (void**)&d->wov.w, (size_t)heads * Cc * I * sizeof(half_t)));
  RET_IF(launch_fold_ov(wo->d, wv->d, heads, hd, Cc, I, d->wov.w, c->bs));
  RET_IF(load_norm(c, p + ".proj_out.0", &d->gn_o1));
  RET_IF(pack_conv(c, p + ".proj_out.2.weight", "", false, false, &d->conv1));
  RET_IF(load_norm(c, p + ".proj_out.3", &d->gn_o2));
  RET_IF(pack_conv(c, p + ".proj_out.5.weight", "", false, false, &d->conv2));
  RET_IF(dmalloc(c, (void**)&d->relu_beta, (size_t)heads * Cc * sizeof(half_t)));
  RET_IF(launch_relu_beta_tile(d->gn_ctx.b, Cc, heads, d->relu_beta, c->bs));
  return 0;
}

int build_sparse_layer(mvd_ctx* c, const std::string& p, const std::string& blk, int slot, bool strided, SparseLayerW* L) {
  RawTensor *w, *g, *b, *rm, *rv;
  const std::string wk = p + blk + "." + std::to_string(slot) + ".weight";
  const std::string bn = p + blk + "." + std::to_string(slot + 1);
  RET_IF(get_raw(c, wk, &w));
  RET_IF(get_raw(c, bn + ".weight", &g));
  RET_IF(get_raw(c, bn + ".bias", &b));
  RET_IF(get_raw(c, bn + ".running_mean", &rm));
  RET_IF(get_raw(c, bn + ".running_var", &rv));
  if (w->shape.size() != 5) return mvd_fail("sparse conv weight: rank 5 expected");
  const int64_t* sh5 = w->shape.data();
  int layout = -1, cout = 0, cin = 0;
  if (sh5[2] == 3 && sh5[3] == 3 && sh5[4] == 3 && sh5[0] != 3) { layout = 0; cout = (int)sh5[0]; cin = (int)sh5[1]; }
  else if (sh5[1] == 3 && sh5[2] == 3 && sh5[3] == 3 && sh5[0] != 3) { layout = 1; cout = (int)sh5[0]; cin = (int)sh5[4]; }
  else if (sh5[0] == 3 && sh5[1] == 3 && sh5[2] == 3) { layout = 2; cin = (int)sh5[3]; cout = (int)sh5[4]; }
  else return mvd_fail("sparse conv weight: not a 3x3x3 kernel in a known layout");
  if ((int)g->numel != cout) return mvd_fail("sparse conv weight: channel count does not match its BatchNorm");
  L->cin = cin;
  L->cout = cout;
  L->strided = strided;
  L->wkey = wk;
  L->bnkey = bn;
  L->layout = layout;
  RET_IF(dmalloc(c, (void**)&L->w, w->numel * 4));
  RET_IF(dmalloc(c, (void**)&L->scale, cout * 4));
  RET_IF(dmalloc(c, (void**)&L->shift, cout * 4));
  RET_IF(launch_sparse_w_pack(w->d, cin, cout, layout, L->w, c->bs));
  if (sparse_mfma_takes(cin, cout) && !mvd_env_call::sparse_valu()) {
    RET_IF(dmalloc(c, (void**)&L->wp, w->numel * 4));
    RET_IF(launch_sparse_w_frag(L->w, cin, cout, 0, 0, L->wp, c->bs));
    if (c->train_mode) {
      RET_IF(dmalloc(c, (void**)&L->wd, w->numel * 4));
      RET_IF(launch_sparse_w_frag(L->w, cout, cin, 1, strided ? 0 : 1, L->wd, c->bs));
    }
  }
  RET_IF(launch_bn_fold(g->d, b->d, rm->d, rv->d, 1e-3f, cout, L->scale, L->shift, c->bs));
  RET_IF(copy_f32(c, bn + ".weight", &L->gamma));
  RET_IF(copy_f32(c, bn + ".bias", &L->beta));
  if (c->train_mode) {
    L->rmean = rm->d;
    L->rvar = rv->d;
  }
  return 0;
}

int build_frustum_block(mvd_ctx* c, const std::string& p, const char* norm_name, bool transposed, int stride,
                        FrustumBlockW* f) {
  RET_IF(pack_lin(c, p + "t_conv.weight", p + "t_conv.bias", &f->t_conv));
  RET_IF(pack_lin(c, p + "v_conv.weight", p + "v_conv.bias", &f->v_conv));
  RET_IF(load_norm(c, p + norm_name, &f->gn));
  RET_IF(pack_conv(c, p + "conv.weight", p + "conv.bias", transposed, false, &f->conv));
  f->cin = f->conv.Cin;
  f->cout = f->conv.N;
  f->stride = stride;
  return 0;
}

}

int build_vae_res(mvd_ctx* c, const std::string& p, VaeResW* r) {
  RawTensor* w1;
  RET_IF(get_raw(c, p + ".conv1.weight", &w1));
  r->cout = (int)w1->shape[0];
  r->cin = (int)w1->shape[1];
  RET_IF(load_norm(c, p + ".norm1", &r->n1));
  RET_IF(pack_conv(c, p + ".conv1.weight", p + ".conv1.bias", false, false, &r->c1, 0, c->vae_exact));
  RET_IF(load_norm(c, p + ".norm2", &r->n2));
  RET_IF(pack_conv(c, p + ".conv2.weight", p + ".conv2.bias", false, false, &r->c2, 0, c->vae_exact));
  r->has_skip = c->raw.count(p + ".nin_shortcut.weight") > 0;
  if (r->has_skip) RET_IF(pack_conv(c, p + ".nin_shortcut.weight", p + ".nin_shortcut.bias", false, false, &r->skip, 0, c->vae_exact));
  else if (r->cin != r->cout) return mvd_fail("VAE ResnetBlock changes width but has no nin_shortcut (conv_shortcut is not used by the reference config)");
  return 0;
}

__global__ void vae_fold_v_bias_kernel(const float* __restrict__ wp, const float* __restrict__ bv, const float* __restrict__ bp,
                                       int C, float* __restrict__ out) {
  const int i = blockIdx.x * blockDim.x + threadIdx.x;
  if (i >= C) return;
  double acc = bp[i];
  for (int j = 0; j < C; ++j) acc += (double)wp[(long)i * C + j] * (double)bv[j];
  out[i] = (float)acc;
}

int build_vae_attn(mvd_ctx* c, const std::string& p, VaeAttnW* a) {
  RET_IF(load_norm(c, p + ".norm", &a->norm));
  RET_IF(pack_conv(c, p + ".q.weight", p + ".q.bias", false, false, &a->q, 0, c->vae_exact));
  RET_IF(pack_conv(c, p + ".k.weight", p + ".k.bias", false, false, &a->k, 0, c->vae_exact));
  RET_IF(pack_conv(c, p + ".v.weight", "", false, false, &a->v, 0, c->vae_exact));
  RET_IF(pack_conv(c, p + ".proj_out.weight", "", false, false, &a->proj, 0, c->vae_exact));
  RawTensor *wp, *bv, *bp;
  RET_IF(get_raw(c, p + ".proj_out.weight", &wp));
  RET_IF(get_raw(c, p + ".v.bias", &bv));
  RET_IF(get_raw(c, p + ".proj_out.bias", &bp));
  const int C = (int)bp->numel;
  RET_IF(dmalloc(c, (void**)&a->proj.bias, C * sizeof(float)));
  hipLaunchKernelGGL(vae_fold_v_bias_kernel, dim3(cdiv(C, 128)), dim3(128), 0, 0, wp->d, bv->d, bp->d, C, a->proj.bias);
  HIP_CHECK_RET(hipGetLastError());
  return 0;
}

int pack_rows(mvd_ctx* c, const float* src, int N, int Cin, int cin_src, ConvW* o) {
  engine_build_rotate(c);
  o->N = N;
  o->Cin = Cin;
  o->taps = 1;
  RET_IF(dmalloc(c, (void**)&o->w, (size_t)N * Cin * sizeof(half_t)));
  return launch_pack_weight(src, N, Cin, 1, 0, 0, o->w, c->bs, cin_src);
}

int build_clip(mvd_ctx* c) {
  const std::string P = "clip_image_encoder.model.visual.";
  ClipW& k = c->clip;
  RawTensor *c1, *pos, *pj;
  RET_IF(get_raw(c, P + "conv1.weight", &c1));
  RET_IF(get_raw(c, P + "positional_embedding", &pos));
  RET_IF(get_raw(c, P + "proj", &pj));
  if (c1->shape.size() != 4 || c1->shape[1] != 3 || c1->shape[2] != c1->shape[3] || pos->shape.size() != 2 ||
      pj->shape.size() != 2)
    return mvd_fail("CLIP: unexpected conv1 / positional_embedding / proj shapes");
  k.width = (int)c1->shape[0];
  k.patch = (int)c1->shape[2];
  k.T = (int)pos->shape[0];
  k.embed = (int)pj->shape[1];
  int grid = 1;
  while (grid * grid < k.T - 1) ++grid;
  if (grid * grid != k.T - 1 || (int)pos->shape[1] != k.width || (int)pj->shape[0] != k.width)
    return mvd_fail("CLIP: positional_embedding must hold 1 + grid^2 tokens of `width` channels");
  k.image = grid * k.patch;
  k.heads = k.width / 64;
  if (k.width % 64 || k.width > 1536) return mvd_fail("CLIP: width must be a multiple of 64, at most 1536");
  k.Tp = (k.T + 7) & ~7;
  const int K = 3 * k.patch * k.patch;
  k.Kp = (K + 7) & ~7;
  RET_IF(pack_rows(c, c1->d, k.width, k.Kp, K, &k.conv1));
  RET_IF(copy_f32(c, P + "class_embedding", &k.cls));
  RET_IF(copy_f32(c, P + "positional_embedding", &k.pos));
  RET_IF(load_norm(c, P + "ln_pre", &k.ln_pre));
  RET_IF(load_norm(c, P + "ln_post", &k.ln_post));
  {
    ConvW t;
    RET_IF(pack_conv(c, P + "proj", "", true, false, &t));
    k.proj.w = t.w;
    k.proj.N = k.embed;
    k.proj.K = k.width;
  }
  k.layers = 0;
  while (c->raw.count(P + "transformer.resblocks." + std::to_string(k.layers) + ".attn.in_proj_weight")) ++k.layers;
  if (k.layers < 1) return mvd_fail("CLIP: no transformer.resblocks uploaded");
  const int w = k.width;
  k.blk.assign(k.layers, ClipLayerW());
  for (int i = 0; i < k.layers; ++i) {
    const std::string L = P + "transformer.resblocks." + std::to_string(i);
    ClipLayerW& b = k.blk[i];
    RawTensor *iw, *ib, *ow, *ob, *fb;
    RET_IF(get_raw(c, L + ".attn.in_proj_weight", &iw));
    RET_IF(get_raw(c, L + ".attn.in_proj_bias", &ib));
    RET_IF(get_raw(c, L + ".attn.out_proj.weight", &ow));
    RET_IF(get_raw(c, L + ".attn.out_proj.bias", &ob));
    RET_IF(get_raw(c, L + ".mlp.c_fc.bias", &fb));
    if ((long)iw->numel != 3L * w * w || (long)ib->numel != 3L * w) return mvd_fail("CLIP: in_proj shape");
    RET_IF(load_norm(c, L + ".ln_1", &b.ln1));
    RET_IF(load_norm(c, L + ".ln_2", &b.ln2));
    RET_IF(pack_rows(c, iw->d, 3 * w, w, w, &b.qkv));
    RET_IF(dmalloc(c, (void**)&b.qkv.bias, (size_t)3 * w * sizeof(float)));
    HIP_CHECK_RET(hipMemcpyAsync(b.qkv.bias, ib->d, (size_t)2 * w * sizeof(float), hipMemcpyDeviceToDevice, 0));
    HIP_CHECK_RET(hipMemset(b.qkv.bias + 2 * w, 0, (size_t)w * sizeof(float)));
    RET_IF(pack_conv(c, L + ".attn.out_proj.weight", "", false, false, &b.out));
    RET_IF(dmalloc(c, (void**)&b.out.bias, (size_t)w * sizeof(float)));
    hipLaunchKernelGGL(vae_fold_v_bias_kernel, dim3(cdiv(w, 128)), dim3(128), 0, 0, ow->d, ib->d + 2 * w, ob->d, w, b.out.bias);
    HIP_CHECK_RET(hipGetLastError());
    RET_IF(pack_conv(c, L + ".mlp.c_fc.weight", "", false, false, &b.fc));
    RET_IF(dmalloc(c, (void**)&b.fc.bias, fb->numel * sizeof(float)));
    RET_IF(launch_scale_copy(fb->d, fb->numel, 1.702f, b.fc.bias, 0));
    RET_IF(pack_conv(c, L + ".mlp.c_proj.weight", L + ".mlp.c_proj.bias", false, false, &b.proj));
  }
  k.present = true;
  return 0;
}

int build_vae_encoder(mvd_ctx* c) {
  const std::string V = "first_stage_model.", E = V + "encoder.";
  VaeEncW& v = c->vae_enc;
  RawTensor *ci, *q;
  RET_IF(get_raw(c, E + "conv_in.weight", &ci));
  RET_IF(get_raw(c, V + "quant_conv.weight", &q));
  v.in_ch = (int)ci->shape[1];
  v.mom = (int)q->shape[0];
  if (v.in_ch > 8 || (v.mom & 3) || (q->shape[1] & 7)) return mvd_fail("VAE encoder: in_channels <= 8, moments % 4 == 0 expected");
  RET_IF(pack_conv(c, E + "conv_in.weight", E + "conv_in.bias", false, false, &v.conv_in, 8, c->vae_exact));
  v.nlev = 0;
  while (c->raw.count(E + "down." + std::to_string(v.nlev) + ".block.0.conv1.weight")) ++v.nlev;
  if (v.nlev < 1) return mvd_fail("VAE encoder: no down blocks uploaded");
  v.down.assign(v.nlev, {});
  v.down_conv.assign(v.nlev, ConvW());
  for (int l = 0; l < v.nlev; ++l) {
    const std::string L = E + "down." + std::to_string(l);
    for (int i = 0; c->raw.count(L + ".block." + std::to_string(i) + ".conv1.weight"); ++i) {
      VaeResW r;
      RET_IF(build_vae_res(c, L + ".block." + std::to_string(i), &r));
      v.down[l].push_back(r);
    }
    if (l < v.nlev - 1) RET_IF(pack_conv(c, L + ".downsample.conv.weight", L + ".downsample.conv.bias", false, false, &v.down_conv[l], 0, c->vae_exact));
  }
  RET_IF(build_vae_res(c, E + "mid.block_1", &v.mid1));
  RET_IF(build_vae_attn(c, E + "mid.attn_1", &v.attn));
  RET_IF(build_vae_res(c, E + "mid.block_2", &v.mid2));
  RET_IF(load_norm(c, E + "norm_out", &v.norm_out));
// ... 334 lines not shown
    }
    if (level != 3) {
      std::vector<UOp> ops;
      RET_IF(add_conv("input_blocks." + std::to_string(bi) + ".0.op", OP_DOWN, ch, ch, ops));
      c->in_blocks.push_back(ops);
      chans.push_back(ch);
      ++bi;
      ds *= 2;
    }
  }
  RET_IF(add_res("middle_block.0", ch, ch, c->mid_block));
  c->res.back().res = u.image_size / ds;
  RET_IF(add_st("middle_block.1", ch, c->mid_block));
  RET_IF(add_res("middle_block.2", ch, ch, c->mid_block));
  c->res.back().res = u.image_size / ds;
  bi = 0;
  for (int level = 3; level >= 0; --level) {
    const int mult = u.channel_mult[level];
    for (int i = 0; i <= u.num_res_blocks; ++i) {
      const int ich = chans.back();
      chans.pop_back();
      std::vector<UOp> ops;
      const std::string b = "output_blocks." + std::to_string(bi);
      RET_IF(add_res(b + ".0", ch + ich, mc * mult, ops));
      c->res.back().res = u.image_size / ds;
      ch = mc * mult;
      int j = 1;
      if (u.attention_levels & ds) {
        RET_IF(add_st(b + "." + std::to_string(j), ch, ops));
        ++j;
      }
      if (level && i == u.num_res_blocks) {
        RET_IF(add_conv(b + "." + std::to_string(j) + ".conv", OP_UP, ch, ch, ops));
        ds /= 2;
        c->convs.back().res_out = u.image_size / ds;
      }
      c->out_blocks.push_back(ops);
      ++bi;
    }
  }
  RET_IF(load_norm(c, U + "out.0", &c->out_norm));
  RET_IF(pack_conv(c, U + "out.2.weight", U + "out.2.bias", false, false, &c->out_conv));
  if (c->out_conv.taps == 9 && c->out_conv.N <= 4 && mc % 32 == 0 && mc <= 512) {
    RET_IF(copy_f32(c, U + "out.2.weight", &c->out_conv.w32));
    c->out_conv.cin_src = mc;
  }
  c->emb_all.N = c->emb_total;
  c->emb_all.K = temb;
  RET_IF(dmalloc(c, (void**)&c->emb_all.w, (size_t)c->emb_total * temb * sizeof(half_t)));
  RET_IF(dmalloc(c, (void**)&c->emb_all.bias, (size_t)c->emb_total * sizeof(float)));
  {
    int off = 0;
    for (auto& pz : emb_pieces) {
      RawTensor *w, *b;
      RET_IF(get_raw(c, pz.key + ".weight", &w));
      RET_IF(get_raw(c, pz.key + ".bias", &b));
      RET_IF(launch_f32_to_f16(w->d, c->emb_all.w + (size_t)off * temb, w->numel, c->bs));
      HIP_CHECK_RET(hipMemcpyAsync(c->emb_all.bias + off, b->d, pz.cout * sizeof(float), hipMemcpyDeviceToDevice, c->bs));
      off += pz.cout;
    }
  }
  c->a2_all.N = c->a2_total;
  c->a2_all.Cin = u.context_dim;
  c->a2_all.taps = 1;
  RET_IF(dmalloc(c, (void**)&c->a2_all.w, (size_t)c->a2_total * u.context_dim * sizeof(half_t)));
  RET_IF(dmalloc(c, (void**)&c->a2_all.bias, (size_t)c->a2_total * sizeof(float)));
  {
    size_t off = 0;
    for (auto& k : a2v_keys) {
      RawTensor *wv, *wo, *bo;
      RET_IF(get_raw(c, k + ".to_v.weight", &wv));
      RET_IF(get_raw(c, k + ".to_out.0.weight", &wo));
      RET_IF(get_raw(c, k + ".to_out.0.bias", &bo));
      const int C = (int)bo->numel;
      RET_IF(launch_fold_ov(wo->d, wv->d, 1, C, u.context_dim, C, c->a2_all.w + off * u.context_dim, c->bs));
      HIP_CHECK_RET(hipMemcpyAsync(c->a2_all.bias + off, bo->d, C * sizeof(float), hipMemcpyDeviceToDevice, c->bs));
      off += C;
    }
  }
  {
    const int c2 = mc * u.channel_mult[2], c1 = mc * u.channel_mult[1], c0 = mc * u.channel_mult[0];
    const int* d = u.volume_dims;
    const int dims[10] = {c2, c2, c2, c2, c1, c1, c1, c0, c0, c0};
    const int ccs[10] = {d[3], d[2], d[2], d[1], d[1], d[1], d[0], d[0], d[0], d[0]};
    const int lvl[10] = {3, 2, 2, 1, 1, 1, 0, 0, 0, 0};
    c->conds.resize(10);
    RET_IF(build_cond(c, U + "middle_conditions", dims[0], ccs[0], &c->conds[0]));
    for (int k = 0; k < 9; ++k)
      RET_IF(build_cond(c, U + "output_conditions." + std::to_string(k), dims[k + 1], ccs[k + 1], &c->conds[k + 1]));
    for (int k = 0; k < 10; ++k) c->conds[k].res = u.image_size >> lvl[k];
    RET_IF(engine_build_join(c));
    c->ctx_groups.clear();
    for (int L = 0; L < 4; ++L) {
      mvd_ctx::CtxGroup gp;
      gp.level = L;
      for (int k = 0; k < 10; ++k)
        if (lvl[k] == L && gp.nblk < 4 && !c->conds[k].proj_ctx.xp && (gp.nblk == 0 || c->conds[k].Cc == gp.Cc)) {
          gp.Cc = c->conds[k].Cc;
          gp.cond[gp.nblk++] = k;
        }
      if (gp.nblk < 2) continue;
      const int Cc = gp.Cc, N = gp.nblk * Cc;
      gp.w.N = N; gp.w.Cin = Cc; gp.w.taps = 1;
      gp.gn.C = N;
      RET_IF(dmalloc(c, (void**)&gp.w.w, (size_t)N * Cc * sizeof(half_t)));
      RET_IF(dmalloc(c, (void**)&gp.gn.g, (size_t)N * sizeof(float)));
      RET_IF(dmalloc(c, (void**)&gp.gn.b, (size_t)N * sizeof(float)));
      for (int j = 0; j < gp.nblk; ++j) {
        const CondW& d = c->conds[gp.cond[j]];
        if (d.proj_ctx.N != Cc || d.proj_ctx.Cin != Cc) return mvd_fail("build_unet_section: unexpected proj_context shape");
        HIP_CHECK_RET(hipMemcpyAsync(gp.w.w + (size_t)j * Cc * Cc, d.proj_ctx.w, (size_t)Cc * Cc * sizeof(half_t), hipMemcpyDeviceToDevice, c->bs));
        HIP_CHECK_RET(hipMemcpyAsync(gp.gn.g + (size_t)j * Cc, d.gn_ctx.g, (size_t)Cc * sizeof(float), hipMemcpyDeviceToDevice, c->bs));
        HIP_CHECK_RET(hipMemcpyAsync(gp.gn.b + (size_t)j * Cc, d.gn_ctx.b, (size_t)Cc * sizeof(float), hipMemcpyDeviceToDevice, c->bs));
      }
      c->ctx_groups.push_back(gp);
    }
  }
  return 0;
}

int build_step_section(mvd_ctx* c) {
  RET_IF(pack_lin(c, "time_embed.0.weight", "time_embed.0.bias", &c->step_te0));
  RET_IF(pack_lin(c, "time_embed.2.weight", "time_embed.2.bias", &c->step_te2));
  return 0;
}

int build_condnet_section(mvd_ctx* c) {
  const std::string S = "spatial_volume.";
  RET_IF(pack_conv(c, S + "target_encoder.init_conv.weight", S + "target_encoder.init_conv.bias", false, false,
                   &c->enc_init, 8));
  for (int i = 0; i < 3; ++i) {
    const std::string p = S + "target_encoder.out_conv" + std::to_string(i) + ".";
    EncBlockW& e = c->enc_blocks[i];
    RET_IF(pack_lin(c, p + "time_embed.weight", p + "time_embed.bias", &e.t));
    RET_IF(pack_lin(c, p + "view_embed.weight", p + "view_embed.bias", &e.v));
    RET_IF(load_norm(c, p + "conv.0", &e.n1));
    RET_IF(pack_conv(c, p + "conv.2.weight", p + "conv.2.bias", false, false, &e.c1));
    RET_IF(load_norm(c, p + "conv.3", &e.n2));
    RET_IF(pack_conv(c, p + "conv.5.weight", p + "conv.5.bias", false, false, &e.c2));
  }
  RET_IF(load_norm(c, S + "target_encoder.final_out.0", &c->enc_final_norm));
  RET_IF(pack_conv(c, S + "target_encoder.final_out.2.weight", S + "target_encoder.final_out.2.bias", false, false,
                   &c->enc_final));
  RET_IF(copy_f32(c, S + "smpl_feature_extractor.conv0.weight", &c->fuse_w));
  RET_IF(copy_f32(c, S + "smpl_feature_extractor.conv0.bias", &c->fuse_b));
  {
    const char* blk[9] = {"conv0", "conv0", "down0", "conv1", "conv1", "down1", "conv2", "conv2", "conv2"};
    const int slot[9] = {0, 3, 0, 0, 3, 0, 0, 3, 6};
    for (int i = 0; i < 9; ++i)
      RET_IF(build_sparse_layer(c, S + "xyzc_net.", blk[i], slot[i], blk[i][0] == 'd', &c->sparse[i]));
  }
  const std::string F = S + "frustum_volume_feats.";
  RET_IF(pack_conv(c, F + "conv0.weight", F + "conv0.bias", false, false, &c->fr_conv0));
  for (int i = 0; i < 6; ++i)
    RET_IF(build_frustum_block(c, F + "conv" + std::to_string(i + 1) + ".", "bn", false, (i % 2 == 0) ? 2 : 1,
                               &c->fr_blocks[i]));
  for (int i = 0; i < 3; ++i)
    RET_IF(build_frustum_block(c, F + "up" + std::to_string(i) + ".", "norm", true, 2, &c->fr_up[i]));
  {
    auto stack = [&](const std::vector<std::string>& prefixes, const char* wn, LinW* out, int K) -> int {
      int total = 0;
      std::vector<RawTensor*> ws, bs;
      for (auto& p : prefixes) {
        RawTensor *wt, *bt;
        RET_IF(get_raw(c, p + wn + ".weight", &wt));
        RET_IF(get_raw(c, p + wn + ".bias", &bt));
        ws.push_back(wt);
        bs.push_back(bt);
        total += (int)wt->shape[0];
      }
      out->N = total;
      out->K = K;
      RET_IF(dmalloc(c, (void**)&out->w, (size_t)total * K * sizeof(half_t)));
      RET_IF(dmalloc(c, (void**)&out->bias, (size_t)total * sizeof(float)));
      size_t off = 0;
      for (size_t i = 0; i < ws.size(); ++i) {
        RET_IF(launch_f32_to_f16(ws[i]->d, out->w + off * K, ws[i]->numel, c->bs));
        HIP_CHECK_RET(hipMemcpyAsync(out->bias + off, bs[i]->d, bs[i]->numel * sizeof(float), hipMemcpyDeviceToDevice, c->bs));
        off += ws[i]->shape[0];
      }
      return 0;
    };
    std::vector<std::string> fp, ep;
    int off = 0;
    for (int i = 0; i < 9; ++i) {
      fp.push_back(i < 6 ? F + "conv" + std::to_string(i + 1) + "." : F + "up" + std::to_string(i - 6) + ".");
      c->film_off[i] = off;
      off += i < 6 ? c->fr_blocks[i].cin : c->fr_up[i - 6].cin;
    }
    c->film_total = off;
    RET_IF(stack(fp, "t_conv", &c->film_t, c->v.time_dim));
    RET_IF(stack(fp, "v_conv", &c->film_v, c->v.view_dim));
    for (int i = 0; i < 3; ++i) ep.push_back(S + "target_encoder.out_conv" + std::to_string(i) + ".");
    RET_IF(stack(ep, "time_embed", &c->enc_t, c->v.time_dim));
    RET_IF(stack(ep, "view_embed", &c->enc_v, c->v.view_dim));
    c->has_spatial = false;
    if (c->use_spatial_volume) {
      const std::string T = S + "spatial_volume_feats.";
      RET_IF(pack_conv(c, T + "init_conv.weight", T + "init_conv.bias", false, false, &c->sp_init));
      if (c->sp_init.Cin != 16 * c->v.num_views || c->sp_init.N != c->spatial_dims[0])
        return mvd_fail("spatial_volume_feats.init_conv: expected [spatial_dims[0], 16 * num_views, 3, 3, 3]");
      const char* names[13] = {"conv0", "conv1", "conv2_0", "conv2_1", "conv3", "conv4_0", "conv4_1", "conv5", "conv6_0", "conv6_1",
                               "conv7", "conv8", "conv9"};
      std::vector<std::string> sp;
      int soff = 0;
      for (int i = 0; i < 13; ++i) {
        const std::string p = T + names[i] + ".";
        SpatialBlockW& b = i < 10 ? c->sp_blocks[i] : c->sp_up[i - 10];
        RET_IF(load_norm(c, p + (i < 10 ? "bn" : "norm"), &b.gn));
        RET_IF(pack_conv(c, p + "conv.weight", p + "conv.bias", i >= 10, false, &b.conv));
        b.cin = b.conv.Cin;
        b.cout = b.conv.N;
        if (b.conv.taps != 27 || b.gn.C != b.cin) return mvd_fail("spatial_volume_feats: a block's conv / norm has an unexpected shape");
        sp.push_back(p);
        c->sp_film_off[i] = soff;
        soff += b.cin;
      }
      c->sp_film_total = soff;
      RET_IF(stack(sp, "t_conv", &c->sp_film_t, c->v.time_dim));
      {
        const int* d = c->spatial_dims;
        const int want[13][2] = {{d[0], d[0]}, {d[0], d[1]}, {d[1], d[1]}, {d[1], d[1]}, {d[1], d[2]}, {d[2], d[2]}, {d[2], d[2]},
                                 {d[2], d[3]}, {d[3], d[3]}, {d[3], d[3]}, {d[3], d[2]}, {d[2], d[1]}, {d[1], d[0]}};
        for (int i = 0; i < 13; ++i) {
          const SpatialBlockW& b = i < 10 ? c->sp_blocks[i] : c->sp_up[i - 10];
          if (b.cin != want[i][0] || b.cout != want[i][1]) return mvd_fail("spatial_volume_feats: channel widths do not match spatial_dims");
        }
      }
      c->has_spatial = true;
    }
  }
  return 0;
}

int build_hot_sections(mvd_ctx* c) {
  if (c->has_unet) {
    RET_IF(build_unet_section(c));
    RET_IF(apply_xp_policy(c));
    RET_IF(engine_build_join(c));
    RET_IF(build_conv3x_streams(c));
    RET_IF(build_rowchain_streams(c));
    RET_IF(build_ffp(c));
    if (c->train_mode) RET_IF(engine_build_dgrad(c));
  }
  if (c->has_step) RET_IF(build_step_section(c));
  if (c->has_cond) {
    RET_IF(build_condnet_section(c));
    RET_IF(engine_build_join(c));
    if (c->train_mode) RET_IF(engine_build_dgrad_cond(c));
  }
  return 0;
}

}

int engine_finalize(mvd_ctx* c) {
  const std::string U = "model.diffusion_model.";
  HIP_CHECK_RET(hipSetDevice(c->device));
  const bool has_unet = c->raw.count(U + "time_embed.0.weight") > 0;
  const bool has_cond = c->raw.count("spatial_volume.target_encoder.init_conv.weight") > 0;
  const bool has_step = c->raw.count("time_embed.0.weight") > 0;
  const bool has_vae = c->raw.count("first_stage_model.decoder.conv_in.weight") > 0;
  const bool has_vae_enc = c->raw.count("first_stage_model.encoder.conv_in.weight") > 0;
  const bool has_clip = c->raw.count("clip_image_encoder.model.visual.conv1.weight") > 0;
  if (!has_unet && !has_cond && !has_vae && !has_vae_enc && !has_clip)
    return mvd_fail("finalize: no UNet, spatial_volume, first-stage or CLIP weights were uploaded");
  if (has_clip) RET_IF(build_clip(c));
  if (has_vae) RET_IF(build_vae(c));
  if (has_vae_enc) RET_IF(build_vae_encoder(c));
  c->has_unet = has_unet;
  c->has_step = has_step;
  c->has_cond = has_cond;
  if (c->train_mode) RET_IF(engine_train_setup(c));
  for (auto& cc : c->cond_const) cc.valid = false;
  c->sec_begin = c->owned.size();
  RET_IF(build_hot_sections(c));
  c->sec_end = c->owned.size();
  HIP_CHECK_RET(hipDeviceSynchronize());
  for (auto it = c->raw.begin(); it != c->raw.end();) {
    if (c->train_mode && engine_hot_key(it->first)) {
      ++it;
      continue;
    }
    hipFree(it->second.d);
    it = c->raw.erase(it);
  }
  if (c->has_unet) RET_IF(engine_side_init(c));
  if (c->has_spatial && !c->sp_ws.base) {
    const size_t bytes = engine_spatial_arena_bytes(c);
    if (hipMalloc((void**)&c->sp_ws.base, bytes) != hipSuccess) return mvd_fail("finalize: spatial-volume arena allocation failed");
    c->sp_ws.size = bytes;
  }
  c->finalized = true;
  return 0;
}

int engine_repack(mvd_ctx* c, hipStream_t after, bool have_stream) {
  if (!c->finalized || !c->train_mode) return mvd_fail("engine_repack: the context was not finalized in training mode");
  HIP_CHECK_RET(hipSetDevice(c->device));
  const bool one_stream = mvd_env().repack_one_stream;
  if (!c->bstreams[0])
    for (int i = 0; i < 4; ++i) {
      HIP_CHECK_RET(hipStreamCreateWithFlags(&c->bstreams[i], hipStreamNonBlocking));
      HIP_CHECK_RET(hipEventCreateWithFlags(&c->bevents[i], hipEventDisableTiming));
    }
  if (!c->bev_after) HIP_CHECK_RET(hipEventCreateWithFlags(&c->bev_after, hipEventDisableTiming));
  if (have_stream) {
    HIP_CHECK_RET(hipEventRecord(c->bev_after, after));
    for (int i = 0; i < 4; ++i) HIP_CHECK_RET(hipStreamWaitEvent(c->bstreams[i], c->bev_after, 0));
  } else {
    HIP_CHECK_RET(hipDeviceSynchronize());
  }
  c->bs_multi = !one_stream;
  c->bs_rr = 0;
  c->bs = c->bstreams[0];
  c->repacking = true;
  c->repack_cursor = c->sec_begin;
  const int r = build_hot_sections(c);
  const bool complete = c->repack_cursor == c->sec_end;
  c->repacking = false;
  c->bs_multi = false;
  c->bs = 0;
  if (have_stream) {
    for (int i = 0; i < 4; ++i) {
      hipEventRecord(c->bevents[i], c->bstreams[i]);
      hipStreamWaitEvent(after, c->bevents[i], 0);
    }
  } else {
    hipDeviceSynchronize();
  }
  RET_IF(r);
  if (!complete) return mvd_fail("engine_repack: allocation sequence shorter than the first build");
  return 0;
}
```

morphablediffusion_amd/csrc/k_conv3x.hip:

```cpp
#include "common.h"
#include "igemm_epilogue.h"

namespace {

template <int IW>
struct CxGeo {
  static constexpr int NI = 256 / (IW * IW);
  static constexpr int HW = IW + 2;
  static constexpr int ROWS = NI * HW * HW;
  static constexpr int GROUPS = (ROWS + 7) / 8;
  static constexpr int BYTES = GROUPS * 1024;
  static constexpr int HP = (GROUPS + 3) / 4;
};

template <int IW>
__device__ __forceinline__ int halo_key(int hy, int hx) {
  if constexpr (IW == 16) return (hx >> 1) & 7;
  else return ((hx >> 1) + 4 * (hy & 1)) & 7;
}

template <int NF, int IW>
__global__ __launch_bounds__(256) void conv3x_kernel(const IGemm g, const half_t* __restrict__ wstream) {
#if defined(__HIP_DEVICE_COMPILE__)
  using Geo = CxGeo<IW>;
  constexpr int CX_HALO_ROWS = Geo::ROWS, CX_HALO_GROUPS = Geo::GROUPS, CX_HALO_BYTES = Geo::BYTES, CX_HP = Geo::HP;
  constexpr int NI = Geo::NI, HWD = Geo::HW;
  constexpr int QF = 3 * NF;
  constexpr int PW = (QF + 3) / 4;
  constexpr int RING_BYTES = 4 * QF * 1024;
  constexpr int NSTEP = 36;
  constexpr int NQ = NSTEP / 3;
  constexpr int CHUNK_FRAGS = NSTEP * NF;
  extern __shared__ __attribute__((aligned(16))) char smem[];
  char* sHalo = smem;
  char* sRing = smem + 2 * CX_HALO_BYTES;
  typedef __attribute__((address_space(3))) void* lds_ptr;

  const int tid = threadIdx.x, lane = tid & 63, h = lane >> 5, pl = lane & 31;
  const int wave = __builtin_amdgcn_readfirstlane(tid >> 6);
  const int H = g.Y, W = g.X, N = g.N, Cin = g.Cin;
  const int bx_per = W / IW, by_per = H / IW, bpi = bx_per * by_per;
  const int nblocks = g.B * bpi;
  const int tiles_m = (nblocks + NI - 1) / NI, tiles_n = N / (32 * NF);
  int bid = blockIdx.x;
  {
    const int nwg = tiles_m * tiles_n;
    const int q = nwg >> 3, r = nwg & 7, xcd = bid & 7, slot = bid >> 3;
    bid = (xcd < r ? xcd * (q + 1) : r * (q + 1) + (xcd - r) * q) + slot;
  }
  int tm = bid / tiles_n, tn = bid - tm * tiles_n;
  if (g.xcd_cols) {
    tn = bid / tiles_m;
    tm = bid - tn * tiles_m;
  }
  const int n0 = tn * 32 * NF;
  auto block_pos = [&](int gb, int& b, int& y0, int& x0) {
    b = gb / bpi;
    const int brem = gb - b * bpi, by = brem / bx_per;
    y0 = by * IW;
    x0 = (brem - by * bx_per) * IW;
  };
  const int ncc = Cin / 64;
  int cc_beg = 0, cc_end = ncc;
  if (g.splitk > 1) {
    const int per = (ncc + g.splitk - 1) / g.splitk;
    cc_beg = blockIdx.y * per;
    cc_end = min(ncc, cc_beg + per);
  }
  const int nchunks = cc_end - cc_beg;

  const auto rsrcA = __builtin_amdgcn_make_buffer_rsrc(const_cast<void*>(g.a), (short)0, 0xFFFFFFFEu, 0x00020000);
  const auto rsrcW = __builtin_amdgcn_make_buffer_rsrc(const_cast<half_t*>(wstream) + (size_t)tn * ncc * CHUNK_FRAGS * 512, (short)0,
                                                       0xFFFFFFFEu, 0x00020000);

  unsigned h_off[CX_HP];
  int h_grp[CX_HP];
#pragma unroll
  for (int i = 0; i < CX_HP; ++i) {
    const int grp = min(wave + 4 * i, CX_HALO_GROUPS - 1);
    h_grp[i] = grp;
    const int hp = grp * 8 + (lane >> 3);
    const int hj = hp / (HWD * HWD), hr = hp - hj * (HWD * HWD);
    const int hy = hr / HWD, hx = hr - hy * HWD;
    const int chunk = (lane & 7) ^ halo_key<IW>(hy, hx);
    int b, y0, x0;
    block_pos(tm * NI + hj, b, y0, x0);
    const int y = y0 + hy - 1, x = x0 + hx - 1;
    const bool ok = hp < CX_HALO_ROWS && tm * NI + hj < nblocks && y >= 0 && y < H && x >= 0 && x < W;
    const unsigned pix = (unsigned)((b * H + y) * W + x);
    h_off[i] = ok ? (pix * (unsigned)g.lda + chunk * 8) * 2 : 0xFFFFFFFFu;
  }
  auto dma_halo_piece = [&](int i, int cc, int buf) {
    const unsigned off = h_off[i] == 0xFFFFFFFFu ? 0xFFFFFFFFu : h_off[i] + cc * 128;
    __builtin_amdgcn_raw_ptr_buffer_load_lds(rsrcA, (lds_ptr)(sHalo + buf * CX_HALO_BYTES + h_grp[i] * 1024), 16, off, 0, 0, 0);
  };
  const unsigned wvoff = (unsigned)(lane * 16);
  auto dma_w_piece = [&](int jq, int i) {
    const int fr = min(wave + 4 * i, QF - 1);
    __builtin_amdgcn_raw_ptr_buffer_load_lds(rsrcW, (lds_ptr)(sRing + (((jq & 3) * QF + fr) << 10)), 16, wvoff + (fr << 10),
                                             (cc_beg * NQ + jq) * (QF << 10), 0, 0);
  };

  int centre[2];
#pragma unroll
  for (int p = 0; p < 2; ++p) {
    if constexpr (IW == 16) centre[p] = (4 * wave + 2 * p + (pl >> 4) + 1) * HWD + (pl & 15) + 1;
    else centre[p] = wave * (HWD * HWD) + (4 * p + (pl >> 3) + 1) * HWD + (pl & 7) + 1;
  }
  const int cx = (IW == 16 ? (pl & 15) : (pl & 7)) + 1, cy_par = IW == 16 ? 0 : (((pl >> 3) + 1) & 1);

  f32x16 acc[2][NF];
#pragma unroll
  for (int p = 0; p < 2; ++p)
#pragma unroll
    for (int f = 0; f < NF; ++f)
#pragma unroll
      for (int r = 0; r < 16; ++r) acc[p][f][r] = 0.f;

  if (nchunks > 0) {
#pragma unroll
    for (int i = 0; i < CX_HP; ++i) dma_halo_piece(i, cc_beg, 0);
#pragma unroll
    for (int jq = 0; jq < 3; ++jq)
#pragma unroll
      for (int i = 0; i < PW; ++i) dma_w_piece(jq, i);
    asm volatile("s_waitcnt vmcnt(0)" ::: "memory");
    __builtin_amdgcn_s_barrier();

    auto rdw = [&](int slot) -> h8 { return *(const h8*)(sRing + (slot << 10) + lane * 16); };
    auto rdx = [&](int buf, int p, int step) -> h8 {
      const int tap = step >> 2, kk = step & 3;
      const int hrow = centre[p] + (tap / 3 - 1) * HWD + (tap % 3 - 1);
      const int key = halo_key<IW>(cy_par + (tap / 3 - 1) + 2, cx + (tap % 3 - 1));
      return *(const h8*)(sHalo + buf * CX_HALO_BYTES + hrow * 128 + (((2 * kk + h) ^ key) << 4));
    };
    h8 wq[4];
    h8 xf[2][2];
#pragma unroll
    for (int k = 0; k < 4; ++k) wq[k] = rdw(k);
    xf[0][0] = rdx(0, 0, 0);
    xf[0][1] = rdx(0, 1, 0);

#pragma unroll 1
    for (int c = 0; c < nchunks; ++c) {
      const int hbuf = c & 1;
      const int cc_next = min(cc_beg + c + 1, ncc - 1);
#pragma unroll
      for (int s = 0; s < NSTEP; ++s) {
        const int qd = s / 3;
        if (s % 3 == 0 && !(c == 0 && s == 0)) {
          const int prev = (qd + NQ - 1) % NQ;
          constexpr int NHQ = (CX_HP + 3) / 4, NH_LAST = CX_HP - 4 * (NHQ - 1);
          const int nh_prev = (prev >= 2 && prev < 2 + NHQ) ? (prev == 2 + NHQ - 1 ? NH_LAST : 4) : 0;
          if (nh_prev == 0) asm volatile("s_waitcnt vmcnt(%0)" ::"i"(PW) : "memory");
          else if (nh_prev == 4) asm volatile("s_waitcnt vmcnt(%0)" ::"i"(PW + 4) : "memory");
          else asm volatile("s_waitcnt vmcnt(%0)" ::"i"(PW + NH_LAST) : "memory");
          __builtin_amdgcn_s_barrier();
        }
#ifdef CX_EXP_NOLDSX
        if (c < 0)
#endif
        if (s + 1 < NSTEP) {
          xf[(s + 1) & 1][0] = rdx(hbuf, 0, s + 1);
          xf[(s + 1) & 1][1] = rdx(hbuf, 1, s + 1);
        } else {
          xf[(s + 1) & 1][0] = rdx(hbuf ^ 1, 0, 0);
          xf[(s + 1) & 1][1] = rdx(hbuf ^ 1, 1, 0);
        }
#pragma unroll
        for (int f = 0; f < NF; ++f) {
          const int i = s * NF + f;
          const int pos = (s % 3) * NF + f;
#ifdef CX_EXP_NODMA
          if (c < 0)
#endif
          if (pos < PW) dma_w_piece(c * NQ + qd + 3, pos);
#ifdef CX_EXP_NODMA
          if (c < 0)
#endif
          if (qd >= 2 && qd < 2 + (CX_HP + 3) / 4 && pos >= PW && pos < PW + 4) {
            const int hi = (qd - 2) * 4 + (pos - PW);
            if (hi < CX_HP) dma_halo_piece(hi, cc_next, hbuf ^ 1);
          }
          const h8 a = wq[i & 3];
#ifdef CX_EXP_NOLDSW
          if (c < 0)
#endif
          wq[i & 3] = rdw((i + 4) % (4 * QF));
          acc[0][f] = MVD_MFMA_32x32x16(a, xf[s & 1][0], acc[0][f], 0, 0, 0);
          acc[1][f] = MVD_MFMA_32x32x16(a, xf[s & 1][1], acc[1][f], 0, 0, 0);
#ifndef CX_NO_SCHEDBAR
          __builtin_amdgcn_sched_barrier(0);
#endif
        }
      }
    }
    asm volatile("s_waitcnt vmcnt(0)" ::: "memory");
    __builtin_amdgcn_s_barrier();
  }

  float* sc = (float*)(smem + wave * EPI_WAVE_BYTES);
  const int M = g.B * H * W;
  float* part = g.splitk > 1 ? g.partial + (long)blockIdx.y * M * N : nullptr;
  const int cq = (lane & 7) * 4;
  long row4[2][4];
  int b = 0;
  bool live = true;
  {
    int y0, x0;
    block_pos(tm * NI + (IW == 16 ? 0 : wave), b, y0, x0);
    live = tm * NI + (IW == 16 ? 0 : wave) < nblocks;
#pragma unroll
    for (int p = 0; p < 2; ++p)
#pragma unroll
      for (int i = 0; i < 4; ++i) {
        const int fr = (lane >> 3) + 8 * i;
        const int yy = IW == 16 ? 4 * wave + 2 * p + (fr >> 4) : 4 * p + (fr >> 3), xx = IW == 16 ? (fr & 15) : (fr & 7);
        row4[p][i] = (long)(b * H + y0 + yy) * W + x0 + xx;
      }
  }
#ifndef CX_NO_RESID_PREFETCH
  float4 rpre[2][NF][4];
  const bool has_res = g.resid && !part && live;
  if (has_res) {
#pragma unroll
    for (int p = 0; p < 2; ++p)
#pragma unroll
      for (int f = 0; f < NF; ++f)
#pragma unroll
        for (int i = 0; i < 4; ++i) rpre[p][f][i] = *(const float4*)((const float*)g.resid + row4[p][i] * g.ldr + n0 + 32 * f + cq);
  }
#endif
#pragma unroll
  for (int p = 0; p < 2; ++p) {
#pragma unroll
    for (int f = 0; f < NF; ++f) {
#pragma unroll
      for (int j = 0; j < 4; ++j)
        *(float4*)(sc + pl * EPI_LD + 8 * j + 4 * h) =
            make_float4(acc[p][f][4 * j], acc[p][f][4 * j + 1], acc[p][f][4 * j + 2], acc[p][f][4 * j + 3]);
      asm volatile("s_waitcnt lgkmcnt(0)" ::: "memory");
      const int n = n0 + 32 * f + cq;
      float4 bsum = make_float4(0.f, 0.f, 0.f, 0.f);
      if (!part) {
        if (g.bias) bsum = *(const float4*)(g.bias + n);
        if (g.rowbias && live) {
          const float4 r = *(const float4*)(g.rowbias + (long)b * g.rb_ld + n);
          bsum.x += r.x; bsum.y += r.y; bsum.z += r.z; bsum.w += r.w;
        }
      }
#pragma unroll
      for (int i = 0; i < 4; ++i) {
        const int fr = (lane >> 3) + 8 * i;
        float4 v = *(const float4*)(sc + fr * EPI_LD + cq);
        if (!live) continue;
        if (part) {
          *(float4*)(part + row4[p][i] * N + n) = v;
          continue;
        }
        v.x += bsum.x; v.y += bsum.y; v.z += bsum.z; v.w += bsum.w;
        if (g.resid) {
#ifndef CX_NO_RESID_PREFETCH
          const float4 r = rpre[p][f][i];
#else
          const float4 r = *(const float4*)((const float*)g.resid + row4[p][i] * g.ldr + n);
#endif
          v.x += r.x; v.y += r.y; v.z += r.z; v.w += r.w;
        }
        *(float4*)((float*)g.out + row4[p][i] * g.ldc + n) = v;
      }
      asm volatile("s_waitcnt lgkmcnt(0)" ::: "memory");
    }
  }
#endif
}

__global__ void conv3x_pack_kernel(const half_t* __restrict__ w, int N, int Cin, int NF, half_t* __restrict__ out, long nfrag) {
  const long gid = (long)blockIdx.x * blockDim.x + threadIdx.x;
  if (gid >= nfrag * 64) return;
  const long q = gid >> 6;
  const int l = (int)(gid & 63), h = l >> 5, r32 = l & 31;
  const int ncc = Cin / 64, per_tile = ncc * 36 * NF;
  const int tn = (int)(q / per_tile);
  int r = (int)(q - (long)tn * per_tile);
  const int cc = r / (36 * NF);
  r -= cc * 36 * NF;
  const int step = r / NF, f = r - step * NF;
  const int tap = step >> 2, kk = step & 3;
  const int n = tn * 32 * NF + 32 * f + r32;
  h8 o = *(const h8*)(w + ((long)tap * N + n) * Cin + 64 * cc + 16 * kk + 8 * h);
  *(h8*)(out + gid * 8) = o;
}

template <int NF, int IW>
int launch_cx(const IGemm& g, const half_t* stream, hipStream_t s) {
  constexpr int LDS = 2 * CxGeo<IW>::BYTES + 4 * 3 * NF * 1024;
  static_assert(LDS <= 160 * 1024 && 4 * EPI_WAVE_BYTES <= LDS, "LDS budget");
  static bool attr_done[MVD_MAX_DEVICES] = {false};
  bool& attr_set = attr_done[mvd_current_device()];
  if (!attr_set) {
    HIP_CHECK_RET(hipFuncSetAttribute((const void*)conv3x_kernel<NF, IW>, hipFuncAttributeMaxDynamicSharedMemorySize, LDS));
    attr_set = true;
  }
  constexpr int NI = CxGeo<IW>::NI;
  dim3 grid(cdiv(g.B * (g.Y / IW) * (g.X / IW), NI) * (g.N / (32 * NF)), g.splitk > 1 ? g.splitk : 1);
  IGemm gl = g;
  const int tiles_m = cdiv(g.B * (g.Y / IW) * (g.X / IW), NI);
  gl.xcd_cols = mvd_env().xcd_cols && xcd_prefers_cols(tiles_m, g.N / (32 * NF), (double)tiles_m * CxGeo<IW>::ROWS * g.Cin * 2, 9.0 * g.N * g.Cin * 2);
  hipLaunchKernelGGL((conv3x_kernel<NF, IW>), grid, dim3(256), LDS, s, gl, stream);
  HIP_CHECK_RET(hipGetLastError());
  return 0;
}

}

bool conv3x_eligible(const IGemm& g, int bn) {
  if (g.a_f32 || g.ntaps != 9 || g.sy != 1 || g.sx != 1 || g.ups || g.Z != 1 || g.geglu || !g.out_linear || g.npar > 0) return false;
  if (g.Cin % 64 || (bn != 160 && bn != 128) || g.N % bn) return false;
  if (g.Y != g.IY || g.X != g.IX) return false;
  if (!((g.Y % 16 == 0 && g.X % 16 == 0) || (g.Y == 8 && g.X == 8))) return false;
  if (!g.out_f32 || g.act != ACT_NONE || g.alpha != 1.0f || g.out_split || g.rowscale || g.gn_partial) return false;
  if ((g.lda & 7) || (g.ldc & 3) || (g.resid && (!g.resid_f32 || (g.ldr & 3))) || (g.rowbias && (g.rb_ld & 3))) return false;
  if ((long)g.B * g.Y * g.X * g.lda * 2 >= 0xFFFFFF00L) return false;
  return true;
}
size_t conv3x_stream_halfs(int N, int Cin, int bn) {
  const size_t nf = bn / 32;
  return ((size_t)(N / bn) * (Cin / 64) * 36 * nf + 4 * 3 * nf) * 512;
}
int conv3x_pack(const half_t* w, int N, int Cin, int bn, half_t* stream, hipStream_t s) {
  if (Cin % 64 || (bn != 160 && bn != 128) || N % bn) return mvd_fail("conv3x_pack: unsupported shape");
  const int nf = bn / 32;
  const long nfrag = (long)(N / bn) * (Cin / 64) * 36 * nf;
  HIP_CHECK_RET(hipMemsetAsync(stream + nfrag * 512, 0, (size_t)4 * 3 * nf * 1024, s));
  hipLaunchKernelGGL(conv3x_pack_kernel, dim3((unsigned)((nfrag * 64 + 255) / 256)), dim3(256), 0, s, w, N, Cin, nf, stream, nfrag);
  HIP_CHECK_RET(hipGetLastError());
  return 0;
}
int launch_conv3x(const IGemm& g, const half_t* stream, int bn, hipStream_t s) {
  if (!conv3x_eligible(g, bn)) return mvd_fail("conv3x: shape not supported");
  if (g.splitk > 1 && !g.partial) return mvd_fail("conv3x: split-K without a partial buffer");
  if ((long)(g.N / bn) * (g.Cin / 64) * 36 * (bn / 32) * 1024 >= 0xFFFFFF00L) return mvd_fail("conv3x: weight stream exceeds 4 GiB");
  if (g.X == 8) return bn == 160 ? launch_cx<5, 8>(g, stream, s) : launch_cx<4, 8>(g, stream, s);
  return bn == 160 ? launch_cx<5, 16>(g, stream, s) : launch_cx<4, 16>(g, stream, s);
}
```

morphablediffusion_amd/engine.py:

```python
import collections
import ctypes as C
import os
import types
from typing import Dict, Optional

import torch

from . import lib as L
from .spec import UNetConfig, VolumeConfig


def _stream():
    return torch.cuda.current_stream().cuda_stream


def _f32(t, device):
    return t.detach().to(device=device, dtype=torch.float32).contiguous()


LOSS_TYPES = ("l2", "huber")


def op_train_loss(pred, target, sample_weight=None, pixel_weight=None, loss_type="l2", huber_delta=1.0, loss_scale=1.0,
                  want_grad=False, device=None, lib=None):
# ... 1214 lines not shown
        sl = None if single else (C.c_int * B)(*slots)
        ts = (C.c_int64 * B)(*steps)
        L.check(self.lib.mvd_denoise_views_ms(
            self._ctx, B, sl, L.ptr(x), L.ptr(xi), L.ptr(cl), ts, L.ptr(te), L.ptr(ve), L.ptr(vi), TN, cfg_scale,
            L.ptr(nz), *coef, L.ptr(x0_hist), bool(first), L.ptr(eps), L.ptr(x_next), _stream()))
        if out is not None and x_next is not out:
            out.copy_(x_next)
        if want_eps and eps_out is not None and eps is not eps_out:
            eps_out.copy_(eps)
        return (x_next, eps) if want_eps else x_next

    def op_cfg_ms(self, eps_c, eps_u, scale, x, noise, coef, x0_hist, first, want_eps=False):
        dev = self.device
        ec, x = _f32(eps_c, dev), _f32(x, dev)
        eu = None if eps_u is None else _f32(eps_u, dev)
        nz = None if noise is None else _f32(noise, dev)
        assert x0_hist.is_contiguous() and x0_hist.dtype == torch.float32 and x0_hist.numel() == x.numel()
        x_next = torch.empty_like(x)
        eps = torch.empty_like(x) if want_eps else None
        L.check(self.lib.mvd_op_cfg_ms(L.ptr(ec), L.ptr(eu), scale, L.ptr(x), L.ptr(nz), *coef, L.ptr(x0_hist), bool(first),
                                       L.ptr(eps), L.ptr(x_next), x.numel(), _stream()))
        return (x_next, eps) if want_eps else x_next

    def op_conv(self, x, w, bias=None, stride=1, upsample=0, resid=None, force_splitk=0):
        dev = self.device
        x, w = _f32(x, dev), _f32(w, dev)
        B, Cin, H, W = x.shape
        Cout, k = w.shape[0], w.shape[2]
        Ho, Wo = ((H << upsample) - 1) // stride + 1, ((W << upsample) - 1) // stride + 1
        out = torch.empty(B, Cout, Ho, Wo, device=dev)
        b = None if bias is None else _f32(bias, dev)
        r = None if resid is None else _f32(resid, dev)
        L.check(self.lib.mvd_op_conv(self._ctx, L.ptr(x), B, Cin, H, W, L.ptr(w), L.ptr(b), Cout, k, stride, upsample,
                                     L.ptr(r), L.ptr(out), force_splitk, _stream()))
        return out

    def op_conv3d(self, x, w, bias=None, stride=1, transposed=False, resid=None):
        dev = self.device
        x, w = _f32(x, dev), _f32(w, dev)
        B, Cin, D, H, W = x.shape
        Cout = w.shape[1] if transposed else w.shape[0]
        if transposed:
            od = (2 * D, 2 * H, 2 * W)
        else:
            od = ((D - 1) // stride + 1, (H - 1) // stride + 1, (W - 1) // stride + 1)
        out = torch.empty(B, Cout, *od, device=dev)
        b = None if bias is None else _f32(bias, dev)
        r = None if resid is None else _f32(resid, dev)
        L.check(self.lib.mvd_op_conv3d(self._ctx, L.ptr(x), B, Cin, D, H, W, L.ptr(w), L.ptr(b), Cout, stride,
                                       bool(transposed), L.ptr(r), L.ptr(out), _stream()))
        return out

    def op_linear(self, a, w, bias=None, geglu=False, resid=None, a_half=False, force_splitk=0):
        dev = self.device
        a, w = _f32(a, dev), _f32(w, dev)
        M, K = a.shape
        N = w.shape[0]
        out = torch.empty(M, N // 2 if geglu else N, device=dev)
        b = None if bias is None else _f32(bias, dev)
        r = None if resid is None else _f32(resid, dev)
        L.check(self.lib.mvd_op_linear(self._ctx, L.ptr(a), M, K, L.ptr(w), L.ptr(b), N, bool(geglu), L.ptr(r),
                                       bool(a_half), force_splitk, L.ptr(out), _stream()))
        return out

    def _guarded(self, rows, ld, f32=True):
        return _nan_guarded(rows, ld, self.device, torch.float32 if f32 else (torch.float16 if L.DTYPE == "f16" else torch.bfloat16))

    @staticmethod
    def _guard_intact(t, rows, width, what):
        _nan_guard_intact(t, rows, what, width)

    def _epi_args(self, rows, N, B, bias, rowbias, rb_ld, resid, ldr, out_f16, out_split, ldc, defer_cap):
        dev = self.device
        if out_split and not out_f16:
            raise ValueError("out_split is a form of the 16-bit result")
        width = 3 * N if out_split else N
        ldc = ldc or width
        b = None if bias is None else _f32(bias, dev)
        rb = None
        if rowbias is not None:
            rb_ld = rb_ld or N
            rb = torch.full((B, rb_ld), float("nan"), device=dev)
            rb[:, :N] = _f32(rowbias, dev).reshape(B, N)
        r = None
        if resid is not None:
            ldr = ldr or N
            r = torch.full((rows, ldr), float("nan"), device=dev)
            r[:, :N] = _f32(resid, dev).reshape(rows, N)
        out = self._guarded(rows, ldc, f32=not out_f16)
        slabs = None
        if defer_cap:
            slabs = torch.empty(defer_cap + N, device=dev)
            slabs.view(torch.int32).fill_(-1)
        return b, rb, rb_ld or 0, r, ldr or 0, out, ldc, width, slabs

    def _epi_result(self, what, out, rows, N, width, out_split, slabs, defer_cap, sk_used):
        self._guard_intact(out, rows, width, what)
        res = types.SimpleNamespace(raw=out[:rows], sk_used=sk_used, slabs=None, hi=None, lo=None, third=None)
        bits = out.view(torch.int32 if out.dtype == torch.float32 else torch.int16)
        res.out_untouched = bool((bits == -1).all())
        if out_split:
            res.hi, res.lo, res.third = out[:rows, :N], out[:rows, N:2 * N], out[:rows, 2 * N:3 * N]
            res.out = res.hi.float() + res.lo.float()
        else:
            res.out = out[:rows, :N].float()
        if slabs is not None:
            used = sk_used * rows * N if sk_used > 1 else 0
            assert used <= defer_cap, f"{what}: sk_used = {sk_used} does not fit the offered slab capacity"
            assert bool((slabs.view(torch.int32)[used:] == -1).all()), f"{what}: the launch wrote behind the slabs it reported"
            if sk_used > 1:
                res.slabs = slabs[:used].reshape(sk_used, rows, N)
        return res

    def op_linear_ex(self, a, w, bias=None, B=1, rowbias=None, rb_ld=0, alpha=1.0, act=0, use_bias=True, out_f16=False,
                     out_split=False, ldc=0, resid=None, resid_f16=False, ldr=0, a_half=False, force_splitk=0, xp=False, defer_cap=0,
                     defer_epilogue=False, poison=True):
        dev = self.device
        a, w = _f32(a, dev), _f32(w, dev)
        rows, K = a.shape
        N = w.shape[0]
        b, rb, rb_ld, r, ldr, out, ldc, width, slabs = self._epi_args(rows, N, B, bias, rowbias, rb_ld, resid, ldr, out_f16, out_split,
                                                                      ldc, defer_cap)
        sk = C.c_int(-1)
        L.check(self.lib.mvd_op_linear_ex(self._ctx, L.ptr(a), B, rows, K, L.ptr(w), L.ptr(b), N, L.ptr(rb), rb_ld, alpha, act,
                                          bool(use_bias and b is not None), bool(out_f16), bool(out_split), ldc, L.ptr(r), bool(resid_f16),
                                          ldr, bool(a_half), force_splitk, bool(xp), L.ptr(slabs), defer_cap, bool(defer_epilogue),
                                          C.byref(sk), bool(poison), L.ptr(out), _stream()))
        return self._epi_result("op_linear_ex", out, rows, N, width, out_split, slabs, defer_cap, sk.value)

    def op_conv_ex(self, x, w, bias=None, stride=1, upsample=0, up_fold=False, tap_shift=0, rowbias=None, rb_ld=0, alpha=1.0, act=0,
                   use_bias=True, out_f16=False, out_split=False, ldc=0, resid=None, resid_f16=False, ldr=0, a_half=True, force_splitk=0,
                   xp=False, conv3x=True, defer_cap=0, defer_epilogue=False, poison=True):
        dev = self.device
        x, w = _f32(x, dev), _f32(w, dev)
        B, Cin, H, W = x.shape
        Cout, k = w.shape[0], w.shape[2]
        Ho, Wo = ((H << upsample) - 1) // stride + 1, ((W << upsample) - 1) // stride + 1
        rows = B * Ho * Wo
        xl = x.permute(0, 2, 3, 1).contiguous()
        rl = None if resid is None else _f32(resid, dev).permute(0, 2, 3, 1).reshape(rows, Cout)
        b, rb, rb_ld, r, ldr, out, ldc, width, slabs = self._epi_args(rows, Cout, B, bias, rowbias, rb_ld, rl, ldr, out_f16, out_split,
                                                                      ldc, defer_cap)
        sk = C.c_int(-1)
        L.check(self.lib.mvd_op_conv_ex(self._ctx, L.ptr(xl), B, H, W, Cin, L.ptr(w), L.ptr(b), Cout, k, stride, upsample, bool(up_fold),
                                        tap_shift, L.ptr(rb), rb_ld, alpha, act, bool(use_bias and b is not None), bool(out_f16),
                                        bool(out_split), ldc, L.ptr(r), bool(resid_f16), ldr, bool(a_half), force_splitk, bool(xp),
                                        bool(conv3x), L.ptr(slabs), defer_cap, bool(defer_epilogue), C.byref(sk), bool(poison), L.ptr(out),
                                        _stream()))
        res = self._epi_result("op_conv_ex", out, rows, Cout, width, out_split, slabs, defer_cap, sk.value)
        res.nchw = res.out.reshape(B, Ho, Wo, Cout).permute(0, 3, 1, 2).contiguous()
        return res

    def op_conv3d_ex(self, x, w, bias=None, stride=1, transposed=False, use_bias=True, resid=None, ldr=0, in_place=False,
                     out_f16=False, ldc=0, a_half=True, force_splitk=0, poison=True):
        dev = self.device
        x, w = _f32(x, dev), _f32(w, dev)
        B, Cin, D, H, W = x.shape
        Cout = w.shape[1] if transposed else w.shape[0]
        od = (2 * D, 2 * H, 2 * W) if transposed else tuple((n - 1) // stride + 1 for n in (D, H, W))
        rows = B * od[0] * od[1] * od[2]
        xl = x.permute(0, 2, 3, 4, 1).contiguous()
        b = None if bias is None else _f32(bias, dev)
        r = None
        if resid is not None:
            ldr = ldr or Cout
            r = torch.full((rows, ldr), float("nan"), device=dev)
            r[:, :Cout] = _f32(resid, dev).permute(0, 2, 3, 4, 1).reshape(rows, Cout)
        ldc = ldc or Cout
        out = self._guarded(rows, ldc, f32=not out_f16)
        L.check(self.lib.mvd_op_conv3d_ex(self._ctx, L.ptr(xl), B, D, H, W, Cin, L.ptr(w), L.ptr(b), Cout, stride, bool(transposed),
                                          bool(use_bias and b is not None), L.ptr(r), ldr or 0, bool(in_place), bool(out_f16), ldc,
                                          bool(a_half), force_splitk, bool(poison), L.ptr(out), _stream()))
        self._guard_intact(out, rows, Cout, "op_conv3d_ex")
        raw = out[:rows, :Cout]
        return types.SimpleNamespace(raw=raw, out=raw.float().reshape(B, *od, Cout).permute(0, 4, 1, 2, 3).contiguous())

    def op_group_norm_ex(self, x, groups, gamma, beta, eps=1e-5, act=0, form=0, ld=0, preadd=None, pld=0, split=0, bias2=None,
                         resid=None, ldr=0, mat=False, ldm=0, ldo=0, poison=True):
        dev = self.device
        x = _f32(x, dev)
        if x.dim() == 3:
            x = x[None]
        nslab, B, rows, Cc = x.shape
        ld = ld or Cc

        def padded(t, lead, ldt):
            p = torch.full((*lead, ldt), float("nan"), device=dev)
            p[..., :Cc] = _f32(t, dev).reshape(*lead, Cc)
            return p
        xs = padded(x, (nslab, B, rows), ld)
        pre = None if preadd is None else padded(preadd, (B,), pld or Cc)
        res = None if resid is None else padded(resid, (B, rows), ldr or Cc)
        b2 = None if bias2 is None else _f32(bias2, dev)
        g, bt = _f32(gamma, dev), _f32(beta, dev)
        wmul = 3 if split == 1 else 1
        ldo_h = ldo or ((2 if split == 2 else wmul) * Cc)
        if split == 2:
            out = self._guarded(B * rows, ldo_h // 2, f32=True)
        else:
            out = self._guarded(B * rows, ldo_h, f32=False)
        m = self._guarded(B * rows, ldm or Cc, f32=True) if mat else None
        L.check(self.lib.mvd_op_group_norm_ex(self._ctx, L.ptr(xs), B, rows, Cc, ld, groups, L.ptr(g), L.ptr(bt), eps, act, form,
                                              L.ptr(pre), (pld or Cc) if pre is not None else 0, split, nslab, B * rows * ld, L.ptr(b2),
                                              L.ptr(res), (ldr or Cc) if res is not None else 0, L.ptr(m), (ldm or Cc) if mat else 0,
                                              ldo_h, bool(poison), L.ptr(out), _stream()))
        self._guard_intact(out, B * rows, wmul * Cc, "op_group_norm_ex")
        if mat:
            self._guard_intact(m, B * rows, Cc, "op_group_norm_ex (mat)")
        if split == 1:
            hi, lo, third = out[:-1, :Cc], out[:-1, Cc:2 * Cc], out[:-1, 2 * Cc:3 * Cc]
            y = hi.float() + lo.float()
            y[hi.view(torch.int16) != third.view(torch.int16)] = float("nan")
        else:
            y = out[:-1, :Cc].float()
        return y.reshape(B, rows, Cc), (m[:-1, :Cc].reshape(B, rows, Cc).clone() if mat else None)

    def op_layer_norm_slabs(self, slabs, gamma, beta, bias=None, rowbias=None, rb_ld=0, T=None, resid=None, ldr=0, eps=1e-5,
                            plain=False, raw=False, ld_raw=0, poison=True):
        dev = self.device
        x = _f32(slabs, dev)
        if x.dim() == 2:
            x = x[None]
        nslab, rows, Cc = x.shape
        g, bt = _f32(gamma, dev), _f32(beta, dev)
        b = None if bias is None else _f32(bias, dev)
        rb = None
        if rowbias is not None:
            rb = torch.full((rowbias.shape[0], rb_ld or Cc), float("nan"), device=dev)
            rb[:, :Cc] = _f32(rowbias, dev)
        r = None
        if resid is not None:
            r = torch.full((rows, ldr or Cc), float("nan"), device=dev)
            r[:, :Cc] = _f32(resid, dev)
        out = self._guarded(rows, Cc, f32=False)
        m = None if plain else self._guarded(rows, Cc, f32=True)
        rw = self._guarded(rows, ld_raw or Cc, f32=False) if raw else None
        L.check(self.lib.mvd_op_layer_norm_slabs(self._ctx, L.ptr(x), nslab, rows * Cc, rows, Cc, L.ptr(b), L.ptr(rb),
                                                 (rb_ld or Cc) if rb is not None else 0, T or rows, L.ptr(r),
                                                 (ldr or Cc) if r is not None else 0, L.ptr(g), L.ptr(bt), eps, bool(plain),
                                                 (ld_raw or Cc) if raw else 0, bool(poison), L.ptr(m), L.ptr(rw), L.ptr(out), _stream()))
        self._guard_intact(out, rows, Cc, "op_layer_norm_slabs")
        if m is not None:
            self._guard_intact(m, rows, Cc, "op_layer_norm_slabs (mat)")
        if rw is not None:
            self._guard_intact(rw, rows, Cc, "op_layer_norm_slabs (raw)")
        return out[:rows].float(), (None if m is None else m[:rows].clone()), (None if rw is None else rw[:rows, :Cc].clone())

    def op_folded_group_norm(self, x, w, cpg, gamma, beta, B, eps=1e-5, poison=True):
        dev = self.device
        x, w, g, bt = _f32(x, dev), _f32(w, dev), _f32(gamma, dev), _f32(beta, dev)
        rows, K = x.shape
        N = w.shape[0]
        if B <= 0 or rows % B or cpg <= 0 or N % cpg:
            raise L.MvdError("op_folded_group_norm: rows % B == 0 and N % cpg == 0 expected")
        rps, G = rows // B, N // cpg
        ntile = max(rps // 256, 1)
        part = self._guarded(B * ntile, 2 * G)
        sc, sh = self._guarded(B, N), self._guarded(B, N)
        out = self._guarded(rows, N, f32=False)
        L.check(self.lib.mvd_op_folded_group_norm(self._ctx, L.ptr(x), B, rps, K, L.ptr(w), N, cpg, L.ptr(g), L.ptr(bt), eps,
                                                  bool(poison), L.ptr(part), L.ptr(sc), L.ptr(sh), L.ptr(out), _stream()))
        for t, n, name in ((part, B * ntile, "partials"), (sc, B, "scale"), (sh, B, "shift"), (out, rows, "out")):
            self._guard_intact(t, n, t.shape[1], f"op_folded_group_norm ({name})")
        return part[:-1].reshape(B, ntile, G, 2).clone(), sc[:B].clone(), sh[:B].clone(), out[:rows].float()

    def op_softmax_rows(self, scores, out_f32=False):
        s = _f32(scores, self.device)
        rows, cols = s.shape
        out = self._guarded(rows, cols, f32=bool(out_f32))
        L.check(self.lib.mvd_op_softmax_rows(self._ctx, L.ptr(s), rows, cols, bool(out_f32), L.ptr(out), _stream()))
        self._guard_intact(out, rows, cols, "op_softmax_rows")
        return out[:rows].clone()

    def op_rows_split(self, x, lda=0):
        dev = self.device
        x = _f32(x, dev)
        rows, Cc = x.shape
        lda = lda or Cc
        xp = torch.full((rows, lda), float("nan"), device=dev)
        xp[:, :Cc] = x
        out = self._guarded(rows, 3 * Cc, f32=False)
        L.check(self.lib.mvd_op_rows_split(self._ctx, L.ptr(xp), lda, rows, Cc, L.ptr(out), _stream()))
        self._guard_intact(out, rows, 3 * Cc, "op_rows_split")
        return out[:rows, :Cc].clone(), out[:rows, Cc:2 * Cc].clone(), out[:rows, 2 * Cc:].clone()

    def op_group_norm(self, x, groups, gamma, beta, eps, act=0):
        dev = self.device
        x = _f32(x, dev)
        B, Cc = x.shape[:2]
        HW = x[0, 0].numel()
        out = torch.empty_like(x)
        g, b = _f32(gamma, dev), _f32(beta, dev)
        L.check(self.lib.mvd_op_group_norm(self._ctx, L.ptr(x), B, Cc, HW, groups, L.ptr(g), L.ptr(b), eps,
                                           act, L.ptr(out), _stream()))
        return out

    def op_layer_norm(self, x, gamma, beta):
        return self.op_layer_norm_slabs(x, gamma, beta, eps=1e-5, plain=True)[0]

    def op_st_tail(self, xin, ln_g, ln_b, w1, b1, w2, b2, ao=None, w_ao=None, b_ao=None, rowbias=None, T=None, w_po=None, b_po=None,
                   resid=None, split=False, iters=0, xp_out=False):
        dev = self.device
        xin = _f32(xin, dev)
        rows, Cc = xin.shape
        keep = [_f32(t, dev) if t is not None else None for t in (ao, rowbias, w_ao, b_ao, ln_g, ln_b, w1, b1, w2, b2, w_po, b_po, resid)]
        ao_, rb_, wao_, bao_, g_, b_, w1_, b1_, w2_, b2_, wpo_, bpo_, res_ = keep
        flags = (1 if ao is not None else 0) | (2 if w_po is not None else 0) | (4 if split else 0) | (8 if xp_out else 0)
        out = torch.empty_like(xin)
        ms = C.c_float(0)
        L.check(self.lib.mvd_op_st_tail(self._ctx, Cc, rows, T or rows, L.ptr(ao_), L.ptr(xin), L.ptr(rb_), L.ptr(wao_), L.ptr(bao_),
                                        L.ptr(g_), L.ptr(b_), L.ptr(w1_), L.ptr(b1_), L.ptr(w2_), L.ptr(b2_), L.ptr(wpo_), L.ptr(bpo_),
                                        L.ptr(res_), L.ptr(out), flags, iters, C.byref(ms), _stream()))
        return (out, ms.value) if iters > 0 else out

    def op_st_head(self, n0, w_pi, b_pi, ln_g, ln_b, w_q, w_k, w_v, iters=0, xp=False):
        dev = self.device
        n0 = _f32(n0, dev)
        rows, Cc = n0.shape
        keep = [_f32(t, dev) for t in (w_pi, b_pi, ln_g, ln_b, w_q, w_k, w_v)]
        t0 = torch.empty(rows, Cc, device=dev)
        qkv = torch.empty(rows, 3 * Cc, device=dev)
        ms = C.c_float(0)
        L.check(self.lib.mvd_op_st_head(self._ctx, rows, bool(xp), L.ptr(n0), *[L.ptr(t) for t in keep], L.ptr(t0), L.ptr(qkv), iters,
                                        C.byref(ms), _stream()))
        return (t0, qkv, ms.value) if iters > 0 else (t0, qkv)

    def op_attention(self, q, k, v, heads):
        return self.op_attention_ex(q, k, v, heads)
# ... 202 lines not shown
```

Before: 78.15 steps/s.

## Route large stride-1 3x3x3 conv3d layers to a halo-streamed conv3z kernel

Extends the conv3x halo/weight-stream kernel with a Z-tap mode, so a 3x3x3 stride-1 conv3d runs as a single kernel. The kernel walks the three depth planes as extra K chunks, reusing the LDS-DMA halo loads and a prepacked weight stream, and can write f16 output. Weights for eligible frustum and spatial volume conv layers (64 or 128 output channels, Cin a multiple of 64) are packed at load time. When conv3x is enabled, layers with M above the dense-DMA limit are routed here instead of the generic implicit GEMM. This costs extra weight-stream memory and drops split-K for those layers.

Result: faster. 79.61 steps/s (median of 6 runs) (+1.9%).

```diff
diff --git a/include/mvd.h b/include/mvd.h
--- a/include/mvd.h
+++ b/include/mvd.h
@@ -265,6 +265,11 @@
 int mvd_op_conv3d_ex(mvd_ctx* ctx, const float* x, int B, int D, int H, int W, int Cin, const float* w, const float* bias, int Cout,
                      int stride, int transposed, int use_bias, const float* resid, int ldr, int in_place, int out_f16, int ldc,
                      int a_half, int force_splitk, int poison, void* out, void* stream);
+int mvd_op_conv3d_form(mvd_ctx* ctx, const float* x, int B, int D, int H, int W, int Cin, const float* w, const float* bias, int Cout,
+                       int stride, int transposed, int use_bias, const float* resid, int ldr, int in_place, int out_f16, int ldc,
+                       int a_half, int force_splitk, int form, int poison, void* out, void* stream);
+int mvd_conv3d_routed_form(int B, int D, int H, int W, int Cin, int Cout, int stride, int transposed, int a_half, int out_f16, int ldc,
+                           int has_resid, int resid_f16, int ldr, int force_splitk);
 int mvd_op_group_norm_ex(mvd_ctx* ctx, const float* x, int B, int rows, int C, int ld, int groups, const float* gamma,
                          const float* beta, float eps, int act, int form, const float* preadd, int pld, int split, int nslab,
                          size_t slab_stride, const float* bias2, const float* resid, int ldr, float* mat, int ldm, int ldo,
diff --git a/morphablediffusion_amd/csrc/c_api_hooks.hip b/morphablediffusion_amd/csrc/c_api_hooks.hip
--- a/morphablediffusion_amd/csrc/c_api_hooks.hip
+++ b/morphablediffusion_amd/csrc/c_api_hooks.hip
@@ -660,10 +660,12 @@
   return hook_sync("op_conv_ex", s, up_fold ? run_upconv2d(c, g, B, H, W, s) : run_conv2d(c, g, B, H, W, stride, upsample, s));
 }
 
-int mvd_op_conv3d_ex(mvd_ctx* c, const float* x, int B, int D, int H, int W, int Cin, const float* w, const float* bias, int Cout,
-                     int stride, int transposed, int use_bias, const float* resid, int ldr, int in_place, int out_f16, int ldc,
-                     int a_half, int force_splitk, int poison, void* out, void* stream) {
-  RET_IF(hook_begin(c));
+static int conv3d_hook(const char* who, mvd_ctx* c, const float* x, int B, int D, int H, int W, int Cin, const float* w, const float* bias,
+                       int Cout, int stride, int transposed, int use_bias, const float* resid, int ldr, int in_place, int out_f16, int ldc,
+                       int a_half, int force_splitk, int form, int poison, void* out, void* stream) {
+  RET_IF(hook_begin(c));
+  if (form != 0 && form != 1) return mvd_fail("op_conv3d_form: form must be 0 or 1");
+  if (form == 1 && (transposed || stride != 1)) return mvd_fail("op_conv3d_form: form 1 (conv3z) is a stride-1 convolution");
   if (!x || !w || !out) return mvd_fail("op_conv3d_ex: null operand");
   if (B <= 0 || D <= 0 || H <= 0 || W <= 0 || Cin <= 0 || (Cin & 7)) return mvd_fail("op_conv3d_ex: Cin % 8 == 0 expected");
   if (Cout <= 0 || (Cout & 3)) return mvd_fail("op_conv3d_ex: Cout must be a positive multiple of 4");
@@ -685,6 +687,13 @@
   ConvW cw;
   RET_IF(hook_pack_fwd(c, w, Cout, Cin, 27, transposed, 0, 0, &cw, s));
   cw.bias = const_cast<float*>(bias);
+  const int bnz = transposed || stride != 1 ? 0 : conv3z_stream_bn(27, Cout, Cin);
+  if (bnz && mvd_env_call::conv3x()) {
+    cw.wx = ws_alloc<half_t>(c, conv3z_stream_halfs(Cout, Cin, bnz));
+    WS_CHECK(cw.wx);
+    RET_IF(conv3z_pack(cw.w, Cout, Cin, bnz, cw.wx, s));
+    cw.wx_bn = bnz;
+  }
   GemmArgs g;
   g.a = x; g.a_f32 = 1; g.lda = Cin; g.w = &cw; g.out = out; g.out_f32 = out_f16 ? 0 : 1; g.ldc = ldc;
   g.use_bias = use_bias != 0; g.force_splitk = force_splitk;
@@ -707,7 +716,33 @@
     }
   }
   if (poison) RET_IF(hook_poison(c, s));
-  return hook_sync("op_conv3d_ex", s, transposed ? run_convT3d(c, g, B, D, H, W, s) : run_conv3d(c, g, B, D, H, W, stride, s));
+  return hook_sync(who, s, transposed ? run_convT3d(c, g, B, D, H, W, s) : run_conv3d(c, g, B, D, H, W, stride, s, form));
+}
+int mvd_op_conv3d_ex(mvd_ctx* c, const float* x, int B, int D, int H, int W, int Cin, const float* w, const float* bias, int Cout,
+                     int stride, int transposed, int use_bias, const float* resid, int ldr, int in_place, int out_f16, int ldc,
+                     int a_half, int force_splitk, int poison, void* out, void* stream) {
+  return conv3d_hook("op_conv3d_ex", c, x, B, D, H, W, Cin, w, bias, Cout, stride, transposed, use_bias, resid, ldr, in_place, out_f16, ldc,
+                     a_half, force_splitk, 0, poison, out, stream);
+}
+int mvd_op_conv3d_form(mvd_ctx* c, const float* x, int B, int D, int H, int W, int Cin, const float* w, const float* bias, int Cout,
+                       int stride, int transposed, int use_bias, const float* resid, int ldr, int in_place, int out_f16, int ldc,
+                       int a_half, int force_splitk, int form, int poison, void* out, void* stream) {
+  return conv3d_hook("op_conv3d_form", c, x, B, D, H, W, Cin, w, bias, Cout, stride, transposed, use_bias, resid, ldr, in_place, out_f16,
+                     ldc, a_half, force_splitk, form, poison, out, stream);
+}
+int mvd_conv3d_routed_form(int B, int D, int H, int W, int Cin, int Cout, int stride, int transposed, int a_half, int out_f16, int ldc,
+                           int has_resid, int resid_f16, int ldr, int force_splitk) {
+  if (B <= 0 || D <= 0 || H <= 0 || W <= 0 || Cin <= 0 || Cout <= 0 || (stride != 1 && stride != 2)) return mvd_fail("conv3d_routed_form: bad shape");
+  if (transposed) return 0;
+  static const half_t some = (half_t)0.f;
+  ConvW cw;
+  cw.N = Cout; cw.Cin = Cin; cw.taps = 27;
+  cw.wx_bn = stride == 1 ? conv3z_stream_bn(27, Cout, Cin) : 0;
+  cw.wx = cw.wx_bn ? const_cast<half_t*>(&some) : nullptr;
+  GemmArgs g;
+  g.a = &some; g.a_f32 = a_half ? 0 : 1; g.lda = Cin; g.w = &cw; g.out_f32 = out_f16 ? 0 : 1; g.ldc = ldc; g.force_splitk = force_splitk;
+  if (has_resid) { g.resid = &some; g.resid_f32 = resid_f16 ? 0 : 1; g.ldr = ldr; }
+  return conv3d_routed_form(g, B, D, H, W, stride);
 }
 
 int mvd_op_group_norm_ex(mvd_ctx* c, const float* x, int B, int rows, int C, int ld, int groups, const float* gamma, const float* beta,
diff --git a/morphablediffusion_amd/csrc/common.h b/morphablediffusion_amd/csrc/common.h
--- a/morphablediffusion_amd/csrc/common.h
+++ b/morphablediffusion_amd/csrc/common.h
@@ -121,6 +121,12 @@
 size_t conv3x_stream_halfs(int N, int Cin, int bn);
 int conv3x_pack(const half_t* w, int N, int Cin, int bn, half_t* stream, hipStream_t s);
 int launch_conv3x(const IGemm& g, const half_t* stream, int bn, hipStream_t s);
+constexpr int CONV3D_DMA_MAX_M = 16384;
+int conv3z_stream_bn(int taps, int N, int Cin);
+bool conv3z_eligible(const IGemm& g, int bn);
+size_t conv3z_stream_halfs(int N, int Cin, int bn);
+int conv3z_pack(const half_t* w, int N, int Cin, int bn, half_t* stream, hipStream_t s);
+int launch_conv3z(const IGemm& g, const half_t* stream, int bn, hipStream_t s);
 bool gemm_dma_eligible(const IGemm& g);
 bool gemm_dma_is_plain(const IGemm& g);
 void gemm_dma_plan(int M, int N, int ksteps, int bn, int geglu, int* nch_out, int* splitk_out);
diff --git a/morphablediffusion_amd/csrc/engine.h b/morphablediffusion_amd/csrc/engine.h
--- a/morphablediffusion_amd/csrc/engine.h
+++ b/morphablediffusion_amd/csrc/engine.h
@@ -561,7 +561,8 @@
 int run_linear(mvd_ctx* c, const GemmArgs& ga, int B, int rows, hipStream_t s);
 int run_conv2d(mvd_ctx* c, const GemmArgs& ga, int B, int H, int W, int stride, int ups, hipStream_t s);
 int run_upconv2d(mvd_ctx* c, const GemmArgs& ga, int B, int H, int W, hipStream_t s);
-int run_conv3d(mvd_ctx* c, const GemmArgs& ga, int B, int D, int H, int W, int stride, hipStream_t s);
+int run_conv3d(mvd_ctx* c, const GemmArgs& ga, int B, int D, int H, int W, int stride, hipStream_t s, int form = 0);
+int conv3d_routed_form(const GemmArgs& ga, int B, int D, int H, int W, int stride);
 int run_convT3d(mvd_ctx* c, const GemmArgs& ga, int B, int D, int H, int W, hipStream_t s);
 int run_group_norm(mvd_ctx* c, const float* x, int ld, int B, int rows_per_sample, const NormW& n, int groups, float eps,
                    int act, const float* preadd, half_t* out, int ldo, hipStream_t s, int preadd_ld = 0, int split = 0,
diff --git a/morphablediffusion_amd/csrc/engine_unet.hip b/morphablediffusion_amd/csrc/engine_unet.hip
--- a/morphablediffusion_amd/csrc/engine_unet.hip
+++ b/morphablediffusion_amd/csrc/engine_unet.hip
@@ -107,6 +107,20 @@
   return r;
 }
 
+int go_conv3z(mvd_ctx* c, IGemm& g, int M, hipStream_t s) {
+  g.bn = g.wx_bn;
+  g.splitk = 1;
+  g.partial = nullptr;
+  const double kalg = (double)(g.cin_alg ? g.cin_alg : g.Cin);
+  double bytes = (double)M * kalg * 2 + 27.0 * g.N * kalg * 2 + (double)M * g.N * (g.out_f32 ? 4 : 2);
+  if (g.resid) bytes += (double)M * g.N * 4;
+  ProbeScope ps(c, s, g.wx_bn == 64 ? "conv3z_kernel<2>" : "conv3z_kernel<4>", 2.0 * M * g.N * kalg * 27.0, bytes);
+  return launch_conv3z(g, g.wx, g.wx_bn, s);
+}
+bool conv3z_routed(const IGemm& g, int M, int force_splitk) {
+  return g.wx && g.ntaps == 27 && force_splitk <= 1 && M > CONV3D_DMA_MAX_M && conv3z_eligible(g, g.wx_bn);
+}
+
 int go_parity_batch(mvd_ctx* c, IGemm& g, int M, hipStream_t s) {
   if (!gemm_dma_eligible(g)) return mvd_fail("igemm_go: parity batch needs the LDS-DMA kernel");
   int kmax = 0;
@@ -260,9 +274,10 @@
   g.bn = igemm_pick_bn(g.N, g.geglu);
   if (g.a_f32 && g.bn == 160 && env.igemm_f32_bn128) g.bn = 128;
   if (env.conv3x && c->use_halo && g.wx && conv3x_eligible(g, g.wx_bn)) return go_conv3x(c, g, M, force_splitk, s, defer);
+  if (env.conv3x && c->use_halo && conv3z_routed(g, M, force_splitk)) return go_conv3z(c, g, M, s);
   if (g.npar > 0) return go_parity_batch(c, g, M, s);
   const bool halo = c->use_halo && conv3_halo_eligible(g);
-  const bool dense = env.gemm_dma && !halo && M >= env.dense_min_m && (g.ntaps == 1 || M <= 16384) && gemm_dma_eligible(g);
+  const bool dense = env.gemm_dma && !halo && M >= env.dense_min_m && (g.ntaps == 1 || M <= CONV3D_DMA_MAX_M) && gemm_dma_eligible(g);
   if (g.gn_partial && !dense) return mvd_fail("igemm_go: the statistics-only pass needs the LDS-DMA kernel");
   if (halo) return launch_planned(c, g, M, plan_halo(g, M, force_splitk), K_HALO, s, defer);
   if (dense) return launch_planned(c, g, M, plan_dense(g, M, force_splitk), K_DENSE, s, defer);
@@ -366,8 +381,9 @@
   return 0;
 }
 
-int run_conv3d(mvd_ctx* c, const GemmArgs& ga, int B, int D, int H, int W, int stride, hipStream_t s) {
-  IGemm g;
+namespace {
+
+int conv3d_desc(IGemm& g, const GemmArgs& ga, int B, int D, int H, int W, int stride) {
   igemm_init(g);
   igemm_fill(g, ga);
   g.B = B;
@@ -386,7 +402,27 @@
   } else {
     return mvd_fail("run_conv3d: kernel must be 1 or 27 taps");
   }
+  return 0;
+}
+
+}
+
+int run_conv3d(mvd_ctx* c, const GemmArgs& ga, int B, int D, int H, int W, int stride, hipStream_t s, int form) {
+  IGemm g;
+  RET_IF(conv3d_desc(g, ga, B, D, H, W, stride));
+  if (form == 1) {
+    if (!g.wx || !conv3z_eligible(g, g.wx_bn))
+      return mvd_fail("run_conv3d: form 1 (conv3z) takes 3x3x3 stride-1 layers of an fp16 source with Cin % 64 == 0, 64 or 128 output channels, H and W multiples of 16");
+    return go_conv3z(c, g, B * g.Z * g.Y * g.X, s);
+  }
+  if (form != 0) return mvd_fail("run_conv3d: form must be 0 or 1");
   return igemm_go(c, g, ga.force_splitk, s);
+}
+
+int conv3d_routed_form(const GemmArgs& ga, int B, int D, int H, int W, int stride) {
+  IGemm g;
+  if (conv3d_desc(g, ga, B, D, H, W, stride)) return -1;
+  return conv3z_routed(g, B * g.Z * g.Y * g.X, ga.force_splitk) ? 1 : 0;
 }
 
 int run_convT3d(mvd_ctx* c, const GemmArgs& ga, int B, int D, int H, int W, hipStream_t s) {
diff --git a/morphablediffusion_amd/csrc/engine_weights.hip b/morphablediffusion_amd/csrc/engine_weights.hip
--- a/morphablediffusion_amd/csrc/engine_weights.hip
+++ b/morphablediffusion_amd/csrc/engine_weights.hip
@@ -234,6 +234,15 @@
   return 0;
 }
 
+int pack_conv3z_stream(mvd_ctx* c, ConvW* w) {
+  const int bn = conv3z_stream_bn(w->taps, w->N, w->Cin);
+  if (!mvd_env().conv3x || !bn || w->xp || c->train_mode) return 0;
+  RET_IF(dmalloc(c, (void**)&w->wx, conv3z_stream_halfs(w->N, w->Cin, bn) * sizeof(half_t)));
+  RET_IF(conv3z_pack(w->w, w->N, w->Cin, bn, w->wx, c->bs));
+  w->wx_bn = bn;
+  return 0;
+}
+
 int build_frustum_block(mvd_ctx* c, const std::string& p, const char* norm_name, bool transposed, int stride,
                         FrustumBlockW* f) {
   RET_IF(pack_lin(c, p + "t_conv.weight", p + "t_conv.bias", &f->t_conv));
@@ -243,6 +252,7 @@
   f->cin = f->conv.Cin;
   f->cout = f->conv.N;
   f->stride = stride;
+  if (!transposed && stride == 1) RET_IF(pack_conv3z_stream(c, &f->conv));
   return 0;
 }
 
@@ -883,6 +893,7 @@
   }
   const std::string F = S + "frustum_volume_feats.";
   RET_IF(pack_conv(c, F + "conv0.weight", F + "conv0.bias", false, false, &c->fr_conv0));
+  RET_IF(pack_conv3z_stream(c, &c->fr_conv0));
   for (int i = 0; i < 6; ++i)
     RET_IF(build_frustum_block(c, F + "conv" + std::to_string(i + 1) + ".", "bn", false, (i % 2 == 0) ? 2 : 1,
                                &c->fr_blocks[i]));
@@ -940,6 +951,7 @@
         SpatialBlockW& b = i < 10 ? c->sp_blocks[i] : c->sp_up[i - 10];
         RET_IF(load_norm(c, p + (i < 10 ? "bn" : "norm"), &b.gn));
         RET_IF(pack_conv(c, p + "conv.weight", p + "conv.bias", i >= 10, false, &b.conv));
+        if (i < 10 && i % 3 != 1) RET_IF(pack_conv3z_stream(c, &b.conv));
         b.cin = b.conv.Cin;
         b.cout = b.conv.N;
         if (b.conv.taps != 27 || b.gn.C != b.cin) return mvd_fail("spatial_volume_feats: a block's conv / norm has an unexpected shape");
diff --git a/morphablediffusion_amd/csrc/k_conv3x.hip b/morphablediffusion_amd/csrc/k_conv3x.hip
--- a/morphablediffusion_amd/csrc/k_conv3x.hip
+++ b/morphablediffusion_amd/csrc/k_conv3x.hip
@@ -19,7 +19,7 @@
   else return ((hx >> 1) + 4 * (hy & 1)) & 7;
 }
 
-template <int NF, int IW>
+template <int NF, int IW, bool ZT = false>
 __global__ __launch_bounds__(256) void conv3x_kernel(const IGemm g, const half_t* __restrict__ wstream) {
 #if defined(__HIP_DEVICE_COMPILE__)
   using Geo = CxGeo<IW>;
@@ -40,7 +40,7 @@
   const int wave = __builtin_amdgcn_readfirstlane(tid >> 6);
   const int H = g.Y, W = g.X, N = g.N, Cin = g.Cin;
   const int bx_per = W / IW, by_per = H / IW, bpi = bx_per * by_per;
-  const int nblocks = g.B * bpi;
+  const int nblocks = (ZT ? g.B * g.Z : g.B) * bpi;
   const int tiles_m = (nblocks + NI - 1) / NI, tiles_n = N / (32 * NF);
   int bid = blockIdx.x;
   {
@@ -60,7 +60,7 @@
     y0 = by * IW;
     x0 = (brem - by * bx_per) * IW;
   };
-  const int ncc = Cin / 64;
+  const int ncc_in = Cin / 64, ncc = ZT ? 3 * ncc_in : ncc_in;
   int cc_beg = 0, cc_end = ncc;
   if (g.splitk > 1) {
     const int per = (ncc + g.splitk - 1) / g.splitk;
@@ -90,8 +90,19 @@
     const unsigned pix = (unsigned)((b * H + y) * W + x);
     h_off[i] = ok ? (pix * (unsigned)g.lda + chunk * 8) * 2 : 0xFFFFFFFFu;
   }
-  auto dma_halo_piece = [&](int i, int cc, int buf) {
-    const unsigned off = h_off[i] == 0xFFFFFFFFu ? 0xFFFFFFFFu : h_off[i] + cc * 128;
+  int zpl = 0;
+  if constexpr (ZT) zpl = (tm / bpi) % g.Z;
+  auto chunk_off = [&](int cc) -> unsigned {
+    if constexpr (ZT) {
+      const int kz = cc / ncc_in, ci = cc - kz * ncc_in;
+      if ((unsigned)(zpl + kz - 1) >= (unsigned)g.Z) return 0xFFFFFFFFu;
+      return (unsigned)(kz - 1) * (unsigned)(H * W * g.lda * 2) + (unsigned)ci * 128u;
+    } else {
+      return (unsigned)cc * 128u;
+    }
+  };
+  auto dma_halo_piece = [&](int i, unsigned coff, int buf) {
+    const unsigned off = (h_off[i] == 0xFFFFFFFFu || (ZT && coff == 0xFFFFFFFFu)) ? 0xFFFFFFFFu : h_off[i] + coff;
     __builtin_amdgcn_raw_ptr_buffer_load_lds(rsrcA, (lds_ptr)(sHalo + buf * CX_HALO_BYTES + h_grp[i] * 1024), 16, off, 0, 0, 0);
   };
   const unsigned wvoff = (unsigned)(lane * 16);
@@ -119,7 +130,7 @@
 
   if (nchunks > 0) {
 #pragma unroll
-    for (int i = 0; i < CX_HP; ++i) dma_halo_piece(i, cc_beg, 0);
+    for (int i = 0; i < CX_HP; ++i) dma_halo_piece(i, chunk_off(cc_beg), 0);
 #pragma unroll
     for (int jq = 0; jq < 3; ++jq)
 #pragma unroll
@@ -144,7 +155,7 @@
 #pragma unroll 1
     for (int c = 0; c < nchunks; ++c) {
       const int hbuf = c & 1;
-      const int cc_next = min(cc_beg + c + 1, ncc - 1);
+      const unsigned coff_next = chunk_off(min(cc_beg + c + 1, ncc - 1));
 #pragma unroll
       for (int s = 0; s < NSTEP; ++s) {
         const int qd = s / 3;
@@ -180,7 +191,7 @@
 #endif
           if (qd >= 2 && qd < 2 + (CX_HP + 3) / 4 && pos >= PW && pos < PW + 4) {
             const int hi = (qd - 2) * 4 + (pos - PW);
-            if (hi < CX_HP) dma_halo_piece(hi, cc_next, hbuf ^ 1);
+            if (hi < CX_HP) dma_halo_piece(hi, coff_next, hbuf ^ 1);
           }
           const h8 a = wq[i & 3];
 #ifdef CX_EXP_NOLDSW
@@ -267,6 +278,14 @@
 #endif
           v.x += r.x; v.y += r.y; v.z += r.z; v.w += r.w;
         }
+        if constexpr (ZT) {
+          if (!g.out_f32) {
+            h4 o;
+            o[0] = (half_t)v.x; o[1] = (half_t)v.y; o[2] = (half_t)v.z; o[3] = (half_t)v.w;
+            *(h4*)((half_t*)g.out + row4[p][i] * g.ldc + n) = o;
+            continue;
+          }
+        }
         *(float4*)((float*)g.out + row4[p][i] * g.ldc + n) = v;
       }
       asm volatile("s_waitcnt lgkmcnt(0)" ::: "memory");
@@ -275,18 +294,18 @@
 #endif
 }
 
-__global__ void conv3x_pack_kernel(const half_t* __restrict__ w, int N, int Cin, int NF, half_t* __restrict__ out, long nfrag) {
+__global__ void conv3x_pack_kernel(const half_t* __restrict__ w, int N, int Cin, int NF, int nz, half_t* __restrict__ out, long nfrag) {
   const long gid = (long)blockIdx.x * blockDim.x + threadIdx.x;
   if (gid >= nfrag * 64) return;
   const long q = gid >> 6;
   const int l = (int)(gid & 63), h = l >> 5, r32 = l & 31;
-  const int ncc = Cin / 64, per_tile = ncc * 36 * NF;
+  const int ncc = Cin / 64, per_tile = nz * ncc * 36 * NF;
   const int tn = (int)(q / per_tile);
   int r = (int)(q - (long)tn * per_tile);
-  const int cc = r / (36 * NF);
-  r -= cc * 36 * NF;
+  const int vc = r / (36 * NF), kz = vc / ncc, cc = vc - kz * ncc;
+  r -= vc * 36 * NF;
   const int step = r / NF, f = r - step * NF;
-  const int tap = step >> 2, kk = step & 3;
+  const int tap = kz * 9 + (step >> 2), kk = step & 3;
   const int n = tn * 32 * NF + 32 * f + r32;
   h8 o = *(const h8*)(w + ((long)tap * N + n) * Cin + 64 * cc + 16 * kk + 8 * h);
   *(h8*)(out + gid * 8) = o;
@@ -312,6 +331,24 @@
   return 0;
 }
 
+template <int NF>
+int launch_cz(const IGemm& g, const half_t* stream, hipStream_t s) {
+  constexpr int LDS = 2 * CxGeo<16>::BYTES + 4 * 3 * NF * 1024;
+  static_assert(LDS <= 160 * 1024 && 4 * EPI_WAVE_BYTES <= LDS, "LDS budget");
+  static bool attr_done[MVD_MAX_DEVICES] = {false};
+  bool& attr_set = attr_done[mvd_current_device()];
+  if (!attr_set) {
+    HIP_CHECK_RET(hipFuncSetAttribute((const void*)conv3x_kernel<NF, 16, true>, hipFuncAttributeMaxDynamicSharedMemorySize, LDS));
+    attr_set = true;
+  }
+  IGemm gl = g;
+  gl.xcd_cols = 0;
+  gl.splitk = 1;
+  hipLaunchKernelGGL((conv3x_kernel<NF, 16, true>), dim3(g.B * g.Z * (g.Y / 16) * (g.X / 16) * (g.N / (32 * NF))), dim3(256), LDS, s, gl, stream);
+  HIP_CHECK_RET(hipGetLastError());
+  return 0;
+}
+
 }
 
 bool conv3x_eligible(const IGemm& g, int bn) {
@@ -333,7 +370,7 @@
   const int nf = bn / 32;
   const long nfrag = (long)(N / bn) * (Cin / 64) * 36 * nf;
   HIP_CHECK_RET(hipMemsetAsync(stream + nfrag * 512, 0, (size_t)4 * 3 * nf * 1024, s));
-  hipLaunchKernelGGL(conv3x_pack_kernel, dim3((unsigned)((nfrag * 64 + 255) / 256)), dim3(256), 0, s, w, N, Cin, nf, stream, nfrag);
+  hipLaunchKernelGGL(conv3x_pack_kernel, dim3((unsigned)((nfrag * 64 + 255) / 256)), dim3(256), 0, s, w, N, Cin, nf, 1, stream, nfrag);
   HIP_CHECK_RET(hipGetLastError());
   return 0;
 }
@@ -344,3 +381,35 @@
   if (g.X == 8) return bn == 160 ? launch_cx<5, 8>(g, stream, s) : launch_cx<4, 8>(g, stream, s);
   return bn == 160 ? launch_cx<5, 16>(g, stream, s) : launch_cx<4, 16>(g, stream, s);
 }
+
+bool conv3z_eligible(const IGemm& g, int bn) {
+  if (g.a_f32 || g.ntaps != 27 || g.sz != 1 || g.sy != 1 || g.sx != 1 || g.ups || g.geglu || !g.out_linear || g.npar > 0) return false;
+  for (int t = 0; t < 27; ++t)
+    if (g.tap[t] != igemm_tap(t / 9 - 1, (t / 3) % 3 - 1, t % 3 - 1, t)) return false;
+  if (g.Cin % 64 || (bn != 64 && bn != 128) || (g.N != 64 && g.N != 128) || g.N % bn) return false;
+  if (g.Z != g.IZ || g.Y != g.IY || g.X != g.IX || g.Z != g.PZ || g.Y != g.PY || g.X != g.PX) return false;
+  if (g.Y % 16 || g.X % 16) return false;
+  if (g.act != ACT_NONE || g.alpha != 1.0f || g.out_split || g.rowscale || g.rowbias || g.gn_partial) return false;
+  if ((g.lda & 7) || (g.ldc & 3) || (g.resid && (!g.resid_f32 || (g.ldr & 3)))) return false;
+  if ((long)g.B * g.Z * g.Y * g.X * g.lda * 2 >= 0xFFFFFF00L) return false;
+  return true;
+}
+int conv3z_stream_bn(int taps, int N, int Cin) { return taps == 27 && Cin > 0 && Cin % 64 == 0 && (N == 64 || N == 128) ? N : 0; }
+size_t conv3z_stream_halfs(int N, int Cin, int bn) {
+  const size_t nf = bn / 32;
+  return ((size_t)(N / bn) * 3 * (Cin / 64) * 36 * nf + 4 * 3 * nf) * 512;
+}
+int conv3z_pack(const half_t* w, int N, int Cin, int bn, half_t* stream, hipStream_t s) {
+  if (Cin % 64 || (bn != 64 && bn != 128) || N % bn) return mvd_fail("conv3z_pack: unsupported shape");
+  const int nf = bn / 32;
+  const long nfrag = (long)(N / bn) * 3 * (Cin / 64) * 36 * nf;
+  HIP_CHECK_RET(hipMemsetAsync(stream + nfrag * 512, 0, (size_t)4 * 3 * nf * 1024, s));
+  hipLaunchKernelGGL(conv3x_pack_kernel, dim3((unsigned)((nfrag * 64 + 255) / 256)), dim3(256), 0, s, w, N, Cin, nf, 3, stream, nfrag);
+  HIP_CHECK_RET(hipGetLastError());
+  return 0;
+}
+int launch_conv3z(const IGemm& g, const half_t* stream, int bn, hipStream_t s) {
+  if (!conv3z_eligible(g, bn)) return mvd_fail("conv3z: shape not supported");
+  if ((long)(g.N / bn) * 3 * (g.Cin / 64) * 36 * (bn / 32) * 1024 >= 0xFFFFFF00L) return mvd_fail("conv3z: weight stream exceeds 4 GiB");
+  return bn == 64 ? launch_cz<2>(g, stream, s) : launch_cz<4>(g, stream, s);
+}
diff --git a/morphablediffusion_amd/engine.py b/morphablediffusion_amd/engine.py
--- a/morphablediffusion_amd/engine.py
+++ b/morphablediffusion_amd/engine.py
@@ -1390,7 +1390,7 @@
         return res
 
     def op_conv3d_ex(self, x, w, bias=None, stride=1, transposed=False, use_bias=True, resid=None, ldr=0, in_place=False,
-                     out_f16=False, ldc=0, a_half=True, force_splitk=0, poison=True):
+                     out_f16=False, ldc=0, a_half=True, force_splitk=0, poison=True, form=None):
         dev = self.device
         x, w = _f32(x, dev), _f32(w, dev)
         B, Cin, D, H, W = x.shape
@@ -1406,12 +1406,19 @@
             r[:, :Cout] = _f32(resid, dev).permute(0, 2, 3, 4, 1).reshape(rows, Cout)
         ldc = ldc or Cout
         out = self._guarded(rows, ldc, f32=not out_f16)
-        L.check(self.lib.mvd_op_conv3d_ex(self._ctx, L.ptr(xl), B, D, H, W, Cin, L.ptr(w), L.ptr(b), Cout, stride, bool(transposed),
-                                          bool(use_bias and b is not None), L.ptr(r), ldr or 0, bool(in_place), bool(out_f16), ldc,
-                                          bool(a_half), force_splitk, bool(poison), L.ptr(out), _stream()))
+        head = (self._ctx, L.ptr(xl), B, D, H, W, Cin, L.ptr(w), L.ptr(b), Cout, stride, bool(transposed),
+                bool(use_bias and b is not None), L.ptr(r), ldr or 0, bool(in_place), bool(out_f16), ldc, bool(a_half), force_splitk)
+        tail = (bool(poison), L.ptr(out), _stream())
+        if form is None:
+            L.check(self.lib.mvd_op_conv3d_ex(*head, *tail))
+        else:
+            L.check(self.lib.mvd_op_conv3d_form(*head, int(form), *tail))
         self._guard_intact(out, rows, Cout, "op_conv3d_ex")
         raw = out[:rows, :Cout]
         return types.SimpleNamespace(raw=raw, out=raw.float().reshape(B, *od, Cout).permute(0, 4, 1, 2, 3).contiguous())
+
+    def op_conv3d_form(self, x, w, form, **kw):
+        return self.op_conv3d_ex(x, w, form=form, **kw)
 
     def op_group_norm_ex(self, x, groups, gamma, beta, eps=1e-5, act=0, form=0, ld=0, preadd=None, pld=0, split=0, bias2=None,
                          resid=None, ldr=0, mat=False, ldm=0, ldo=0, poison=True):
```
